# DaanVrancken/HubbardTN

Measured on AMD Instinct MI355X. Metric: DMRG sweep time (s) + GS energy/site, 1-band Hubbard L=64 chi=1024, lower is better.
Workload: dtype c128; 1 GPU; one-band Hubbard chain L=64 U/t=4, half filling, fZ2xSU(2)xU(1), two-site DMRG sweep (2L-3=125 bond updates) at chi=1024 (TensorKit dim units); model=one_band, L=64, chi=1024, krylovdim=30, parallelism=sector-parallel apply x1, backend=hip

## Files before the change

hubbardtn_amd/abi.py:

```python
from __future__ import annotations

import ctypes as C
import os

import numpy as np

HERE = os.path.dirname(os.path.abspath(__file__))
LIB_PATH = os.path.join(HERE, "csrc", "libhubbardtn_hip.so")

HTN_MAX_BUFS = 8
HTN_TILE = 32
OP_N, OP_T, OP_C = 0, 1, 2
SEG_GEMM, SEG_COPY = 0, 1

TILE_DT = np.dtype([("c_off", "<i8"), ("buf_c", "<i4"), ("ldc", "<i4"), ("m", "<i4"), ("n", "<i4"),
                    ("row0", "<i4"), ("col0", "<i4"), ("seg_begin", "<i4"), ("seg_count", "<i4"),
                    ("pad0", "<i4"), ("pad1", "<i4"), ("part", "<i4"), ("nparts", "<i4"), ("ws_slot", "<i4"),
                    ("ticket", "<i4")], align=False)
BUF_WS = 7
WS_TICKET_ELEMS = 4096
SEG_DT = np.dtype([("a_off", "<i8"), ("b_off", "<i8"), ("buf_a", "<i4"), ("buf_b", "<i4"),
                   ("lda", "<i4"), ("ldb", "<i4"), ("k", "<i4"), ("op_a", "<i4"), ("op_b", "<i4"),
                   ("type", "<i4"), ("alpha_re", "<f8"), ("alpha_im", "<f8")], align=False)
SVD_DT = np.dtype([("g_off", "<i8"), ("v_off", "<i8"), ("s_off", "<i8"), ("m", "<i4"), ("n", "<i4"),
                   ("flags", "<i4"), ("pad", "<i4")], align=False)
SVD_ACCUMULATE = 1
SVD_QRCP = 2
COPY_DT = np.dtype([("dst_off", "<i8"), ("src_off", "<i8"), ("idx_off", "<i8"), ("scl_off", "<i8"),
                    ("rows", "<i4"), ("cols", "<i4"), ("ldd", "<i4"), ("lds", "<i4"), ("op", "<i4"),
                    ("gather_dim", "<i4"), ("scale_dim", "<i4"), ("inv_norm", "<i4")], align=False)
QR_DT = np.dtype([("offset", "<i8"), ("m", "<i4"), ("n", "<i4"), ("ld", "<i4"), ("pad", "<i4"), ("r_offset", "<i8"),
                  ("ldr", "<i4"), ("trans", "<i4")], align=False)
QR_PANEL, QR_CHUNK, QR_MAX_M = 16, 512, 7664
assert TILE_DT.itemsize == 64 and SEG_DT.itemsize == 64 and SVD_DT.itemsize == 40 and COPY_DT.itemsize == 64
assert QR_DT.itemsize == 40
TRDOT_DT = np.dtype([("a_off", "<i8"), ("b_off", "<i8"), ("rows", "<i4"), ("cols", "<i4"), ("lda", "<i4"), ("ldb", "<i4"),
                     ("out", "<i4"), ("pad", "<i4", (3,)), ("w_re", "<f8"), ("w_im", "<f8")], align=False)
TRDOT_SLOTS = 16
assert TRDOT_DT.itemsize == 64

SYM_SU2_U1, SYM_U1_U1, SYM_SU2 = 0, 1, 2
MAX_SITE = 4
BACKEND_CPU, BACKEND_HIP = 0, 1
SITE_OP_DT = np.dtype([("k", "<i4"), ("dN", "<i4"), ("red", "<f8", (MAX_SITE * MAX_SITE,))], align=False)
MPO_ENTRY_DT = np.dtype([("wl", "<i4"), ("wr", "<i4"), ("op", "<i4"), ("pad", "<i4"), ("coef_re", "<f8"),
                         ("coef_im", "<f8")], align=False)
SUBBLOCK_DT = np.dtype([("lN", "<i4"), ("lj", "<i4"), ("s", "<i4"), ("rN", "<i4"), ("rj", "<i4"), ("ld", "<i4"),
                        ("off", "<i8")], align=False)
SECTOR_DT = np.dtype([("N", "<i4"), ("j", "<i4"), ("count", "<i4")], align=False)
ENV_BLOCK_DT = np.dtype([("aN", "<i4"), ("aj", "<i4"), ("w", "<i4"), ("bN", "<i4"), ("bj", "<i4"), ("rows", "<i4"),
                         ("cols", "<i4"), ("pad", "<i4"), ("off", "<i8")], align=False)
BOND_STATS_DT = np.dtype([("bond", "<i4"), ("direction", "<i4"), ("n_matvec", "<i4"), ("jacobi_sweeps", "<i4"),
                          ("chi_full", "<i4"), ("multiplets", "<i4"), ("n_tiles", "<i4"), ("n_segs", "<i4"),
                          ("theta_size", "<i8"), ("apply_flops", "<i8"), ("apply_bytes", "<i8"), ("svd_flops", "<i8"),
                          ("energy", "<f8"), ("residual", "<f8"), ("trunc_weight", "<f8"), ("t_plan", "<f8"),
                          ("t_lanczos", "<f8"), ("t_svd", "<f8"), ("t_env", "<f8"), ("t_total", "<f8"),
                          ("matvec_ms", "<f8")], align=False)
assert SITE_OP_DT.itemsize == 136 and MPO_ENTRY_DT.itemsize == 32 and SUBBLOCK_DT.itemsize == 32
assert SECTOR_DT.itemsize == 12 and ENV_BLOCK_DT.itemsize == 40 and BOND_STATS_DT.itemsize == 136


class Symmetry(C.Structure):
    _fields_ = [("kind", C.c_int32), ("n_site", C.c_int32), ("site_N", C.c_int32 * MAX_SITE),
                ("site_j", C.c_int32 * MAX_SITE)]


class SiteOp(C.Structure):
    _fields_ = [("k", C.c_int32), ("dN", C.c_int32), ("red", C.c_double * (MAX_SITE * MAX_SITE))]


class TrdotItem(C.Structure):
    _fields_ = [("a_off", C.c_int64), ("b_off", C.c_int64), ("rows", C.c_int32), ("cols", C.c_int32), ("lda", C.c_int32),
                ("ldb", C.c_int32), ("out", C.c_int32), ("pad", C.c_int32 * 3), ("w_re", C.c_double), ("w_im", C.c_double)]


class CorrChannel(C.Structure):
    _fields_ = [("open", SiteOp), ("pass_", SiteOp), ("close", SiteOp), ("onsite", SiteOp), ("has_onsite", C.c_int32),
                ("pad", C.c_int32)]


class SvdOpts(C.Structure):
    _fields_ = [("split_elems", C.c_int32), ("sweeps_hint", C.c_int32), ("rank_cut", C.c_double),
                ("sweeps_used", C.POINTER(C.c_int32))]


class SweepOpts(C.Structure):
    _fields_ = [("chi_full", C.c_int32), ("weighting", C.c_int32), ("cutoff", C.c_double), ("krylovdim", C.c_int32),
                ("maxrestart", C.c_int32), ("lanczos_tol", C.c_double), ("jacobi_tol", C.c_double),
                ("jacobi_max_sweeps", C.c_int32), ("svd_split_elems", C.c_int32), ("rank_cut", C.c_double),
                ("profile", C.c_int32), ("pad", C.c_int32)]


class IdmrgOpts(C.Structure):
    _fields_ = [("sweep", SweepOpts), ("cell_sites", C.c_int32), ("window_dN", C.c_int32), ("tol", C.c_double),
                ("min_steps", C.c_int32), ("maxiter", C.c_int32), ("sweeps_per_step", C.c_int32), ("warm_start", C.c_int32)]


class IdmrgStats(C.Structure):
    _fields_ = [("step", C.c_int32), ("sweeps", C.c_int32), ("converged", C.c_int32), ("finished", C.c_int32),
                ("needs_window", C.c_int32), ("chi_full", C.c_int32), ("energy", C.c_double),
                ("energy_per_site", C.c_double), ("delta", C.c_double)]


assert C.sizeof(SiteOp) == 136 and C.sizeof(TrdotItem) == 64 and C.sizeof(CorrChannel) == 4 * 136 + 8
assert C.sizeof(SweepOpts) == 64 and C.sizeof(IdmrgOpts) == 96 and C.sizeof(IdmrgStats) == 48

EXPORTS = ["htn_last_error", "htn_abi_version", "htn_device_init", "htn_grouped_gemm_z",
           "htn_dots_scratch_elems", "htn_dots_z", "htn_axpys_z", "htn_scale_inv_sqrt_z",
           "htn_jacobi_svd_z", "htn_batched_copy_z", "htn_lanczos_scratch_elems", "htn_lanczos_z", "htn_lanczos_orth_z",
           "htn_trdots_scratch_elems", "htn_block_trdots_z"]
ENGINE_EXPORTS = ["htn_ctx_create", "htn_ctx_destroy", "htn_ctx_backend", "htn_ctx_set_timing", "htn_comm_unique_id",
                  "htn_ctx_set_comm", "htn_ctx_set_exchange", "htn_mpo_create", "htn_mpo_destroy", "htn_mps_create",
                  "htn_mps_destroy", "htn_bond_update", "htn_dmrg2_sweep", "htn_mps_theta_size", "htn_heff2_apply",
                  "htn_mps_get_theta", "htn_mps_nsites", "htn_mps_bond", "htn_mps_spectrum", "htn_mps_site_size",
                  "htn_mps_get_site", "htn_mps_env_size", "htn_mps_get_env", "htn_mps_env_blocks", "htn_mps_env_bond",
                  "htn_plan_apply_dump", "htn_mps_cache_stats", "htn_balance_tiles",
                  "htn_idmrg_create", "htn_idmrg_destroy", "htn_idmrg_boundary", "htn_idmrg_step", "htn_idmrg_window",
                  "htn_mps_set_orthogonal", "htn_mps_orthogonal_count", "htn_mps_overlap",
                  "htn_site_update", "htn_dmrg1_sweep", "htn_mps_centre", "htn_mps_site_theta_size", "htn_heff1_apply",
                  "htn_qr_blocks_z", "htn_mps_correlator"]


class GemmLaunch(C.Structure):
    _fields_ = [("bufs", C.c_void_p * HTN_MAX_BUFS), ("tiles", C.c_void_p), ("segs", C.c_void_p),
                ("n_tiles", C.c_int32), ("pad", C.c_int32)]


EXCHANGE_FN = C.CFUNCTYPE(C.c_int, C.c_void_p, C.c_int64, C.c_void_p)

_lib = None


class HtnError(RuntimeError):
    pass


def load_library(path: str | None = None):
    global _lib
    if _lib is not None and path is None:
        return _lib
    p = path or LIB_PATH
    import torch
    if not os.path.exists(p):
        raise HtnError(f"{p} not found: build it with `python -m hubbardtn_amd.build` "
                       "(hipcc --offload-arch=gfx950); there is no CPU fallback")
    lib = C.CDLL(p)
    vp, i32, i64, f64 = C.c_void_p, C.c_int32, C.c_int64, C.c_double
    lib.htn_last_error.restype = C.c_char_p
    lib.htn_abi_version.restype = C.c_int
    lib.htn_device_init.argtypes = [C.c_int, C.c_char_p, C.POINTER(C.c_int)]
    lib.htn_grouped_gemm_z.argtypes = [C.POINTER(vp), vp, i32, vp, vp]
    lib.htn_dots_scratch_elems.argtypes = [i32]
    lib.htn_dots_scratch_elems.restype = i64
    lib.htn_dots_z.argtypes = [vp, i64, i32, vp, i64, vp, vp, vp]
    lib.htn_axpys_z.argtypes = [vp, vp, i64, i32, vp, f64, i64, vp]
    lib.htn_scale_inv_sqrt_z.argtypes = [vp, vp, vp, i64, vp]
    lib.htn_jacobi_svd_z.argtypes = [vp, vp, vp, vp, vp, i32, i32, i32, f64, vp, C.POINTER(SvdOpts), vp]
    lib.htn_batched_copy_z.argtypes = [vp, vp, vp, vp, vp, i32, f64, vp]
    lib.htn_lanczos_scratch_elems.argtypes = [i32]
    lib.htn_lanczos_scratch_elems.restype = i64
    lib.htn_lanczos_z.argtypes = [C.POINTER(GemmLaunch), i32, i32, i32, vp, i64, i32, f64, i32, vp, i32,
                                  EXCHANGE_FN, vp, C.POINTER(f64), C.POINTER(i32), C.POINTER(f64), C.POINTER(f64), vp]
    lib.htn_lanczos_orth_z.argtypes = [C.POINTER(GemmLaunch), i32, i32, i32, vp, i64, i32, f64, i32, vp, i32,
                                       EXCHANGE_FN, vp, C.POINTER(f64), C.POINTER(i32), C.POINTER(f64), C.POINTER(f64),
                                       vp, i32, vp]
    lib.htn_trdots_scratch_elems.argtypes = [i32]
    lib.htn_trdots_scratch_elems.restype = i64
    lib.htn_block_trdots_z.argtypes = [vp, vp, vp, i32, vp, i32, vp, vp]
    declare_engine(lib)
    for name in EXPORTS + ENGINE_EXPORTS:
        getattr(lib, name)
    if lib.htn_abi_version() != ABI_VERSION:
        raise HtnError("ABI version mismatch")
    if path is None:
        _lib = lib
    return lib


ABI_VERSION = 2


def declare_engine(lib):
    vp, i32, i64, f64 = C.c_void_p, C.c_int32, C.c_int64, C.c_double
    lib.htn_last_error.restype = C.c_char_p
    lib.htn_abi_version.restype = C.c_int
    lib.htn_ctx_create.argtypes = [i32, i32, vp, C.POINTER(vp)]
    lib.htn_ctx_destroy.argtypes = [vp]
    lib.htn_ctx_destroy.restype = None
    lib.htn_ctx_backend.argtypes = [vp]
    lib.htn_ctx_set_timing.argtypes = [vp, i32]
    lib.htn_comm_unique_id.argtypes = [vp]
    lib.htn_ctx_set_comm.argtypes = [vp, i32, i32, vp]
    lib.htn_ctx_set_exchange.argtypes = [vp, i32, i32, EXCHANGE_FN, vp]
    lib.htn_mpo_create.argtypes = [vp, C.POINTER(Symmetry), i32, vp, i32, vp, vp, vp, vp, C.POINTER(vp)]
    lib.htn_mpo_destroy.argtypes = [vp]
    lib.htn_mpo_destroy.restype = None
    lib.htn_mps_create.argtypes = [vp, vp, i32, vp, vp, vp, vp, vp, vp, vp, vp, C.POINTER(vp)]
    lib.htn_mps_destroy.argtypes = [vp]
    lib.htn_mps_destroy.restype = None
    lib.htn_bond_update.argtypes = [vp, i32, i32, i32, i32, C.POINTER(SweepOpts), vp]
    lib.htn_dmrg2_sweep.argtypes = [vp, C.POINTER(SweepOpts), vp, C.POINTER(f64)]
    lib.htn_mps_theta_size.argtypes = [vp, i32]
    lib.htn_mps_theta_size.restype = i64
    lib.htn_heff2_apply.argtypes = [vp, i32, vp, vp]
    lib.htn_mps_get_theta.argtypes = [vp, i32, vp]
    lib.htn_mps_nsites.argtypes = [vp]
    lib.htn_mps_bond.argtypes = [vp, i32, vp]
    lib.htn_mps_spectrum.argtypes = [vp, i32, vp, vp]
    lib.htn_mps_spectrum.restype = i64
    lib.htn_mps_site_size.argtypes = [vp, i32, C.POINTER(i32)]
    lib.htn_mps_site_size.restype = i64
    lib.htn_mps_get_site.argtypes = [vp, i32, vp, vp]
    lib.htn_mps_env_size.argtypes = [vp, i32, i32]
    lib.htn_mps_env_size.restype = i64
    lib.htn_mps_get_env.argtypes = [vp, i32, i32, vp]
    lib.htn_mps_env_blocks.argtypes = [vp, i32, i32, vp]
    lib.htn_mps_env_bond.argtypes = [vp, i32, i32, vp]
    lib.htn_plan_apply_dump.argtypes = [vp, i32, i32, C.POINTER(i32), vp, C.POINTER(i32), vp, C.POINTER(i64),
                                        C.POINTER(i64)]
    lib.htn_mps_cache_stats.argtypes = [vp, C.POINTER(i64), C.POINTER(i64)]
    lib.htn_balance_tiles.argtypes = [vp, i32, i32, vp, i32, C.POINTER(i32)]
    lib.htn_idmrg_create.argtypes = [vp, vp, C.POINTER(IdmrgOpts), C.POINTER(vp)]
    lib.htn_idmrg_destroy.argtypes = [vp]
    lib.htn_idmrg_destroy.restype = None
    lib.htn_idmrg_boundary.argtypes = [vp, i32, vp]
    lib.htn_idmrg_step.argtypes = [vp, vp, vp, vp, vp, vp, vp, C.POINTER(IdmrgStats)]
    lib.htn_idmrg_window.argtypes = [vp, C.POINTER(vp)]
    lib.htn_mps_set_orthogonal.argtypes = [vp, C.POINTER(vp), i32]
    lib.htn_mps_orthogonal_count.argtypes = [vp, C.POINTER(i32)]
    lib.htn_mps_overlap.argtypes = [vp, vp, C.POINTER(f64)]
    lib.htn_site_update.argtypes = [vp, i32, i32, i32, C.POINTER(SweepOpts), vp]
    lib.htn_dmrg1_sweep.argtypes = [vp, C.POINTER(SweepOpts), vp, C.POINTER(f64)]
    lib.htn_mps_centre.argtypes = [vp]
    lib.htn_mps_site_theta_size.argtypes = [vp, i32]
    lib.htn_mps_site_theta_size.restype = i64
    lib.htn_heff1_apply.argtypes = [vp, i32, vp, vp]
    lib.htn_qr_blocks_z.argtypes = [vp, vp, vp, vp, i32, vp]
    lib.htn_mps_correlator.argtypes = [vp, C.POINTER(CorrChannel), vp, C.POINTER(f64)]
    for name in ENGINE_EXPORTS:
        getattr(lib, name)


def check(lib, rc: int, what: str):
    if rc != 0:
        raise HtnError(f"{what}: {lib.htn_last_error().decode()}")
```

hubbardtn_amd/csrc/htn_backend_hip.hip:

```cpp
#include <dlfcn.h>

#include <map>
#include <mutex>

#include "htn_common.h"
#include "htn_core.h"

namespace {

__global__ __launch_bounds__(256) void k_scale_z(double2* __restrict__ x, int64_t n, double f) {
    for (int64_t j = (int64_t)blockIdx.x * blockDim.x + threadIdx.x; j < n; j += (int64_t)gridDim.x * blockDim.x) {
        const double2 v = x[j];
        x[j] = make_double2(v.x * f, v.y * f);
    }
}

__global__ __launch_bounds__(256) void k_copy_words(uint32_t* __restrict__ dst, const uint32_t* __restrict__ src, size_t n) {
    for (size_t j = (size_t)blockIdx.x * blockDim.x + threadIdx.x; j < n; j += (size_t)gridDim.x * blockDim.x) dst[j] = src[j];
    __threadfence_system();
}

struct Rccl {
    void* lib = nullptr;
    int (*GetUniqueId)(void*) = nullptr;
    void* CommInitRank = nullptr;
    int (*CommDestroy)(void*) = nullptr;
    int (*AllReduce)(const void*, void*, size_t, int, int, void*, hipStream_t) = nullptr;
    const char* (*GetErrorString)(int) = nullptr;
    bool ok = false;
};
struct NcclId {
    char internal[128];
};
Rccl& rccl() {
    static Rccl r;
    static std::once_flag once;
    std::call_once(once, [] {
        const char* names[] = {"librccl.so.1", "librccl.so", "/opt/rocm/lib/librccl.so.1", "/opt/rocm/lib/librccl.so"};
        for (const char* n : names) {
            r.lib = dlopen(n, RTLD_NOW | RTLD_GLOBAL);
            if (r.lib) break;
        }
        if (!r.lib) return;
        r.GetUniqueId = (int (*)(void*))dlsym(r.lib, "ncclGetUniqueId");
        r.CommInitRank = dlsym(r.lib, "ncclCommInitRank");
        r.CommDestroy = (int (*)(void*))dlsym(r.lib, "ncclCommDestroy");
        r.AllReduce = (int (*)(const void*, void*, size_t, int, int, void*, hipStream_t))dlsym(r.lib, "ncclAllReduce");
        r.GetErrorString = (const char* (*)(int))dlsym(r.lib, "ncclGetErrorString");
        r.ok = r.GetUniqueId && r.CommInitRank && r.CommDestroy && r.AllReduce;
    });
    return r;
}
typedef int (*nccl_init_fn)(void**, int, NcclId, int);

struct HipBackend : htn::Backend {
    int device = 0;
    hipStream_t st = nullptr;
    bool own_stream = false;
    std::multimap<size_t, void*> free_list;
    bool fork_open = false;
    std::map<void*, size_t> live;
    size_t pooled = 0;
    void* lan_scratch = nullptr;
    int64_t lan_scratch_elems = 0;
    void* trd_scratch = nullptr;
    int64_t trd_scratch_elems = 0;
    void* comm = nullptr;
    char* stage = nullptr;
    size_t stage_cap = (size_t)32 << 20, stage_pos = 0;
    char* land = nullptr;
    char* land_dev = nullptr;
    size_t land_cap = (size_t)4 << 20;

    ~HipBackend() override {
        (void)hipSetDevice(device);
        if (st) (void)hipStreamSynchronize(st);
        htn_krylov_release_stream(st);
        htn_svd_release_stream(st);
        if (comm && rccl().ok) rccl().CommDestroy(comm);
        for (auto& kv : free_list) (void)hipFree(kv.second);
        for (auto& kv : live) (void)hipFree(kv.first);
        if (lan_scratch) (void)hipFree(lan_scratch);
        if (trd_scratch) (void)hipFree(trd_scratch);
        if (stage) (void)hipHostFree(stage);
        if (land) (void)hipHostFree(land);
        if (own_stream && st) (void)hipStreamDestroy(st);
    }
    int kind() const override { return HTN_BACKEND_HIP; }
    int activate() override {
        HIP_TRY(hipSetDevice(device));
        return 0;
    }

    void* poisoned(void* p, size_t bytes) {
        if (p && htn_debug_poison() && hipMemsetAsync(p, 0xFF, bytes, st) != hipSuccess) {
            (void)hipGetLastError();
            htn::set_error("HTN_DEBUG_POISON: hipMemsetAsync failed");
            live.erase(p);
            (void)hipFree(p);
            return nullptr;
        }
        return p;
    }
    void* alloc(size_t bytes) override {
        if (fork_open) {
            htn::set_error("pool invariant violated: allocation while the SVD's forked stream is open");
            return nullptr;
        }
        bytes = (bytes + 255) / 256 * 256;
        auto it = free_list.lower_bound(bytes);
        if (it != free_list.end() && it->first <= bytes + bytes / 4 + 4096) {
            void* p = it->second;
            live[p] = it->first;
            pooled -= it->first;
            free_list.erase(it);
            return poisoned(p, live[p]);
        }
        void* p = nullptr;
        const size_t want = bytes + bytes / 8;
        if (hipMalloc(&p, want) != hipSuccess) {
            (void)hipGetLastError();
            (void)hipStreamSynchronize(st);
            for (auto& kv : free_list) (void)hipFree(kv.second);
            free_list.clear();
            pooled = 0;
            if (hipMalloc(&p, bytes) != hipSuccess) {
                (void)hipGetLastError();
                return nullptr;
            }
            live[p] = bytes;
            return poisoned(p, bytes);
        }
        live[p] = want;
        return poisoned(p, want);
    }
    void release(void* p) override {
        if (fork_open) {
            htn::set_error("pool invariant violated: release while the SVD's forked stream is open");
            abort();
        }
        auto it = live.find(p);
        if (it == live.end()) return;
        const size_t sz = it->second;
        live.erase(it);
        if (pooled + sz > ((size_t)64 << 30)) {
            (void)hipStreamSynchronize(st);
            (void)hipFree(p);
            return;
        }
        free_list.insert({sz, p});
        pooled += sz;
    }
    int upload(void* dst, const void* src, size_t bytes) override {
        if (!bytes) return 0;
        if (bytes > stage_cap / 2) {
            HIP_TRY(hipMemcpyAsync(dst, src, bytes, hipMemcpyHostToDevice, st));
            HIP_TRY(hipStreamSynchronize(st));
            stage_pos = 0;
            return 0;
        }
        if (!stage) HIP_TRY(hipHostMalloc((void**)&stage, stage_cap));
        const size_t need = (bytes + 255) & ~(size_t)255;
        if (stage_pos + need > stage_cap) {
            HIP_TRY(hipStreamSynchronize(st));
            stage_pos = 0;
        }
        memcpy(stage + stage_pos, src, bytes);
        HIP_TRY(hipMemcpyAsync(dst, stage + stage_pos, bytes, hipMemcpyHostToDevice, st));
        stage_pos += need;
        return 0;
    }
    int download(void* dst, const void* src, size_t bytes) override {
        if (!bytes) return 0;
        if (bytes > land_cap) {
            HIP_TRY(hipMemcpyAsync(dst, src, bytes, hipMemcpyDeviceToHost, st));
            HIP_TRY(hipStreamSynchronize(st));
            stage_pos = 0;
            return 0;
        }
        if (!land) {
            HIP_TRY(hipHostMalloc((void**)&land, land_cap, hipHostMallocMapped | hipHostMallocCoherent));
            HIP_TRY(hipHostGetDevicePointer((void**)&land_dev, land, 0));
        }
        if (bytes <= ((size_t)256 << 10) && ((uintptr_t)src & 3) == 0) {
            const size_t words = (bytes + 3) / 4;
            hipLaunchKernelGGL(k_copy_words, dim3((unsigned)std::min<size_t>((words + 255) / 256, 64)), dim3(256), 0, st,
                               (uint32_t*)land_dev, (const uint32_t*)src, words);
            HIP_TRY(hipGetLastError());
        } else
            HIP_TRY(hipMemcpyAsync(land, src, bytes, hipMemcpyDeviceToHost, st));
        HIP_TRY(htn_stream_spin(st));
        memcpy(dst, land, bytes);
        stage_pos = 0;
        return 0;
    }
    int zero(void* p, size_t bytes) override {
        if (!bytes) return 0;
        HIP_TRY(hipMemsetAsync(p, 0, bytes, st));
        return 0;
    }
    int sync() override {
        HIP_TRY(htn_stream_spin(st));
        stage_pos = 0;
        return 0;
    }
    int grouped_gemm(const void* const* bufs, const htn_tile* tiles, int32_t n_tiles, const htn_seg* segs) override {
        return htn_grouped_gemm_z(bufs, tiles, n_tiles, segs, st);
    }
    int lanczos(const htn_gemm_launch* stages, int n_stages, int x_slot, int y_slot, void* V, int64_t n, int krylovdim,
                double tol, int max_restart, int zero_y, htn_exchange2_fn exchange, void* user, double* eig, int* n_matvec,
                double* residual, double* matvec_ms) override {
        if (ensure_lan_scratch(htn_lanczos_scratch_elems(krylovdim))) return 1;
        int32_t nmv = 0;
        const int rc = htn_lanczos_z(stages, n_stages, x_slot, y_slot, V, n, krylovdim, tol, max_restart, lan_scratch, zero_y,
                                     exchange, user, eig, &nmv, residual, matvec_ms, st);
        *n_matvec = nmv;
        return rc;
    }
    int ensure_lan_scratch(int64_t need) {
        if (need > lan_scratch_elems) {
            if (lan_scratch) HIP_TRY(hipFree(lan_scratch));
            HIP_TRY(hipMalloc(&lan_scratch, sizeof(double2) * need));
            if (htn_debug_poison()) HIP_TRY(hipMemsetAsync(lan_scratch, 0xFF, sizeof(double2) * need, st));
            lan_scratch_elems = need;
        }
        return 0;
    }
    int lanczos_orth(const htn_gemm_launch* stages, int n_stages, int x_slot, int y_slot, void* V, int64_t n, int krylovdim,
                     double tol, int max_restart, int zero_y, htn_exchange2_fn exchange, void* user, const void* Q, int n_frozen,
                     double* eig, int* n_matvec, double* residual, double* matvec_ms) override {
        if (ensure_lan_scratch(htn_lanczos_scratch_elems(krylovdim + n_frozen))) return 1;
        int32_t nmv = 0;
        const int rc = htn_lanczos_orth_z(stages, n_stages, x_slot, y_slot, V, n, krylovdim, tol, max_restart, lan_scratch, zero_y,
                                          exchange, user, eig, &nmv, residual, matvec_ms, Q, n_frozen, st);
        *n_matvec = nmv;
        return rc;
    }
    int orthonormalise_rows(void* Pv, int64_t n, int nvec, double drop_tol, int* kept) override {
        if (nvec > 32) return htn::set_error("orthonormalise_rows: more than 32 rows");
        if (ensure_lan_scratch(htn_dots_scratch_elems(32) + 64)) return 1;
        double2* P = (double2*)Pv;
        double2* part = (double2*)lan_scratch;
        double2* coef = part + htn_dots_scratch_elems(32);
        double2* nrm = coef + 32;
        int k = 0;
        for (int r = 0; r < nvec; ++r) {
            double2* dst = P + (int64_t)k * n;
            if (r != k) HIP_TRY(hipMemcpyAsync(dst, P + (int64_t)r * n, sizeof(double2) * n, hipMemcpyDeviceToDevice, st));
            if (htn_dots_z(dst, n, 1, dst, n, nrm, part, st)) return 1;
            for (int pass = 0; pass < 2 && k > 0; ++pass) {
                if (htn_dots_z(P, n, k, dst, n, coef, part, st)) return 1;
                if (htn_axpys_z(dst, P, n, k, coef, -1.0, n, st)) return 1;
            }
            if (htn_dots_z(dst, n, 1, dst, n, nrm + 1, part, st)) return 1;
            double h[4];
            if (download(h, nrm, sizeof(h))) return 1;
            const double n0 = h[0], n1 = h[2];
            if (!(n0 > 0.0) || !(n1 > drop_tol * drop_tol * n0)) continue;
            if (htn_scale_inv_sqrt_z(dst, dst, nrm + 1, n, st)) return 1;
            ++k;
        }
        *kept = k;
        return 0;
    }
    int jacobi_svd(void* G, void* Vj, double* S, const htn_svd_block* desc_dev, const htn_svd_block* desc_host, int n_blocks,
                   int max_m, int max_sweeps, double tol, int32_t* info_dev, const htn_svd_opts* opts) override {
        fork_open = true;
        const int rc = htn_jacobi_svd_z(G, Vj, S, desc_dev, desc_host, n_blocks, max_m, max_sweeps, tol, info_dev, opts, st);
        fork_open = false;
        return rc;
    }
    int qr_blocks(void* A, void* R, const htn_qr_block* desc_dev, const htn_qr_block* desc_host, int n_blocks) override {
        return htn_qr_blocks_z(A, R, desc_dev, desc_host, n_blocks, st);
    }
    int block_trdots(const void* A, const void* B, const htn_trdot_item* items_dev, const htn_trdot_item* items_host, int n_items,
                     void* out, int n_out) override {
        (void)items_host;
        const int64_t need = htn_trdots_scratch_elems(n_items);
        if (need > trd_scratch_elems) {
            if (trd_scratch) HIP_TRY(hipFree(trd_scratch));
            trd_scratch = nullptr, trd_scratch_elems = 0;
            HIP_TRY(hipMalloc(&trd_scratch, sizeof(double2) * 2 * need));
            trd_scratch_elems = 2 * need;
            if (htn_debug_poison()) HIP_TRY(hipMemsetAsync(trd_scratch, 0xFF, sizeof(double2) * trd_scratch_elems, st));
        }
        return htn_block_trdots_z(A, B, items_dev, n_items, out, n_out, trd_scratch, st);
    }
    int batched_copy(void* dst, const void* src, const int32_t* idx, const double* scl, const htn_copy_item* items, int n_items,
                     double gscale) override {
        return htn_batched_copy_z(dst, src, idx, scl, items, n_items, gscale, st);
    }
    int scale(void* x, int64_t n, double f) override {
        if (n <= 0) return 0;
        const int grid = (int)std::min<int64_t>((n + 255) / 256, 2048);
        hipLaunchKernelGGL(k_scale_z, dim3(grid), dim3(256), 0, st, (double2*)x, n, f);
        HIP_TRY(hipGetLastError());
        return 0;
    }
    int set_comm(int rank, int world, const void* id) override {
        Rccl& r = rccl();
        if (!r.ok) return htn::set_error("htn_ctx_set_comm: librccl.so could not be loaded");
        if (comm) {
            r.CommDestroy(comm);
            comm = nullptr;
        }
        NcclId uid;
        memcpy(uid.internal, id, sizeof(uid.internal));
        const int rc = ((nccl_init_fn)r.CommInitRank)(&comm, world, uid, rank);
        if (rc != 0) return htn::set_error("ncclCommInitRank: %s", r.GetErrorString ? r.GetErrorString(rc) : "error");
        return 0;
    }
    bool has_comm() const override { return comm != nullptr; }
    int allreduce(void* y, int64_t n) override {
        if (!comm) return htn::set_error("allreduce: no communicator (htn_ctx_set_comm)");
        const int rc = rccl().AllReduce(y, y, (size_t)(2 * n), 8, 0, comm, st);
        if (rc != 0) return htn::set_error("ncclAllReduce: %s", rccl().GetErrorString ? rccl().GetErrorString(rc) : "error");
        return 0;
    }
};

}

char* htn_err_buf() { return htn::err_buf(); }

namespace htn {
Backend* make_backend(int backend, int device, void* stream) {
    if (backend != HTN_BACKEND_HIP) {
        set_error("libhubbardtn_hip.so has no CPU backend (backend %d requested): there is no CPU fallback", backend);
        return nullptr;
    }
    char name[256];
    int cus = 0;
    if (htn_device_init(device, name, &cus)) return nullptr;
    auto* b = new HipBackend();
    b->device = device;
    if (stream) b->st = (hipStream_t)stream;
    else {
        if (hipStreamCreateWithFlags(&b->st, hipStreamNonBlocking) != hipSuccess) {
            set_error("hipStreamCreate failed");
            delete b;
            return nullptr;
        }
        b->own_stream = true;
    }
    return b;
}
}

extern "C" int htn_comm_unique_id(void* id_host) {
    Rccl& r = rccl();
    if (!r.ok) return htn::set_error("htn_comm_unique_id: librccl.so could not be loaded");
    const int rc = r.GetUniqueId(id_host);
    if (rc != 0) return htn::set_error("ncclGetUniqueId: %s", r.GetErrorString ? r.GetErrorString(rc) : "error");
    return 0;
}
```

hubbardtn_amd/csrc/htn_common.h:

```cpp
#pragma once
#include <hip/hip_runtime.h>
#include <stdint.h>
#include <stdio.h>
#include <stdlib.h>
#include <string.h>

#include <map>
#include <memory>
#include <mutex>
#include <utility>

#include "hubbardtn_hip.h"

char* htn_err_buf();

static inline int htn_fail(const char* what, hipError_t e) {
    snprintf(htn_err_buf(), 512, "%s: %s", what, hipGetErrorString(e));
    return 1;
}
static inline int htn_fail_msg(const char* what) {
    snprintf(htn_err_buf(), 512, "%s", what);
    return 1;
}
#define fail htn_fail
#define fail_msg htn_fail_msg
#define HIP_TRY(x)                                       \
    do {                                                 \
        hipError_t _e = (x);                             \
        if (_e != hipSuccess) return htn_fail(#x, _e);   \
    } while (0)

typedef double d4 __attribute__((ext_vector_type(4)));

static inline hipError_t htn_event_spin(hipEvent_t ev) {
    hipError_t e;
    while ((e = hipEventQuery(ev)) == hipErrorNotReady) __builtin_ia32_pause();
    return e;
}
static inline hipError_t htn_stream_spin(hipStream_t st) {
    static thread_local hipEvent_t evs[64] = {};
    int dev = 0;
    hipError_t e = hipGetDevice(&dev);
    if (e != hipSuccess) return e;
    if (dev < 0 || dev >= 64) return hipStreamSynchronize(st);
    if (!evs[dev] && (e = hipEventCreateWithFlags(&evs[dev], hipEventDisableTiming)) != hipSuccess) return e;
    if ((e = hipEventRecord(evs[dev], st)) != hipSuccess) return e;
    return htn_event_spin(evs[dev]);
}


static inline bool htn_env_flag(const char* name) {
    const char* v = getenv(name);
    return v && v[0] && v[0] != '0';
}
static inline bool htn_debug_poison() {
    static const bool on = htn_env_flag("HTN_DEBUG_POISON");
    return on;
}
static inline bool htn_debug_event_waits() {
    static const bool on = htn_env_flag("HTN_DEBUG_EVENT_WAITS");
    return on;
}

struct LanRecord {
    unsigned long long w[4];
};
__host__ __device__ __forceinline__ unsigned long long lan_rotl(unsigned long long x, int r) { return (x << r) | (x >> (64 - r)); }
__host__ __device__ __forceinline__ unsigned long long lan_check(unsigned long long w0, unsigned long long w1, unsigned long long w2,
                                                                 unsigned long long serial) {
    return serial ^ lan_rotl(w0, 13) ^ lan_rotl(w1, 29) ^ lan_rotl(w2, 47) ^ 0x9E3779B97F4A7C15ull;
}
#define HTN_DOT_BLOCKS 256
struct HtnGemmPublish {
    const double* norm_partial;
    const double2* c1;
    const double2* c2;
    LanRecord* rec_out;
    unsigned long long serial;
};
int htn_grouped_gemm_launch(const void* const* bufs_host, const htn_tile* tiles, int32_t n_tiles, const htn_seg* segs,
                            const HtnGemmPublish* pub, hipStream_t stream);

enum HtnBufKind {
    HTN_BUF_DEVICE,
    HTN_BUF_PINNED,
    HTN_BUF_MAPPED
};
struct HtnBuf {
    const HtnBufKind kind;
    const bool poison;
    void* p = nullptr;
    void* dev = nullptr;
    size_t cap = 0;
    explicit HtnBuf(HtnBufKind k, bool poison_new = true) : kind(k), poison(poison_new) {}
    HtnBuf(const HtnBuf&) = delete;
    ~HtnBuf() { (void)release(); }
    hipError_t release() {
        const hipError_t e = !p ? hipSuccess : (kind == HTN_BUF_DEVICE ? hipFree(p) : hipHostFree(p));
        p = dev = nullptr, cap = 0;
        return e;
    }
    int reserve(size_t bytes) {
        if (bytes <= cap) return 0;
        HIP_TRY(release());
        const size_t want = bytes * 2;
        if (kind == HTN_BUF_DEVICE) {
            HIP_TRY(hipMalloc(&p, want));
            dev = p;
            if (poison && htn_debug_poison()) HIP_TRY(hipMemset(p, 0xFF, want));
        } else if (kind == HTN_BUF_PINNED) {
            HIP_TRY(hipHostMalloc(&p, want, hipHostMallocDefault));
        } else {
            HIP_TRY(hipHostMalloc(&p, want, hipHostMallocMapped | hipHostMallocCoherent));
            HIP_TRY(hipHostGetDevicePointer(&dev, p, 0));
        }
        cap = want;
        return 0;
    }
};

template <class T>
class HtnStreamRegistry {
    std::mutex mu;
    std::map<std::pair<int, hipStream_t>, std::unique_ptr<T>> entries;

public:
    template <class Init>
    int get(hipStream_t st, T** out, Init init) {
        int dev = 0;
        HIP_TRY(hipGetDevice(&dev));
        std::lock_guard<std::mutex> lk(mu);
        auto it = entries.find({dev, st});
        if (it == entries.end()) {
            auto r = std::make_unique<T>();
            r->device = dev;
            if (init(*r)) return 1;
            it = entries.emplace(std::make_pair(dev, st), std::move(r)).first;
        }
        *out = it->second.get();
        return 0;
    }
    void release(hipStream_t st) {
        int dev = 0;
        if (hipGetDevice(&dev) != hipSuccess) return;
        std::lock_guard<std::mutex> lk(mu);
        entries.erase({dev, st});
    }
};
void htn_krylov_release_stream(hipStream_t st);
void htn_svd_release_stream(hipStream_t st);

template <int CTRL>
__device__ __forceinline__ double dpp_f64(double v) {
    const int lo = __builtin_amdgcn_update_dpp(0, __double2loint(v), CTRL, 0xF, 0xF, true);
    const int hi = __builtin_amdgcn_update_dpp(0, __double2hiint(v), CTRL, 0xF, 0xF, true);
    return __hiloint2double(hi, lo);
}

__device__ __forceinline__ double row_sum16(double v) {
    v += dpp_f64<0xB1>(v);
    v += dpp_f64<0x4E>(v);
    v += dpp_f64<0x141>(v);
    v += dpp_f64<0x140>(v);
    return v;
}

template <int L>
__device__ __forceinline__ double lane_bcast(double v) {
    const int lo = __builtin_amdgcn_readlane(__double2loint(v), L);
    const int hi = __builtin_amdgcn_readlane(__double2hiint(v), L);
    return __hiloint2double(hi, lo);
}

__device__ __forceinline__ double wave_sum(double v) {
    v = row_sum16(v);
    const double a = lane_bcast<0>(v) + lane_bcast<16>(v);
    const double b = lane_bcast<32>(v) + lane_bcast<48>(v);
    return a + b;
}

template <int CTRL>
__device__ __forceinline__ unsigned long long dpp_u64(unsigned long long v) {
    const unsigned lo = (unsigned)__builtin_amdgcn_update_dpp(0, (int)(unsigned)v, CTRL, 0xF, 0xF, true);
    const unsigned hi = (unsigned)__builtin_amdgcn_update_dpp(0, (int)(unsigned)(v >> 32), CTRL, 0xF, 0xF, true);
    return ((unsigned long long)hi << 32) | lo;
}
__device__ __forceinline__ unsigned long long umax64(unsigned long long a, unsigned long long b) { return a > b ? a : b; }
__device__ __forceinline__ unsigned long long row_max16_u64(unsigned long long v) {
    v = umax64(v, dpp_u64<0xB1>(v));
    v = umax64(v, dpp_u64<0x4E>(v));
    v = umax64(v, dpp_u64<0x141>(v));
    v = umax64(v, dpp_u64<0x140>(v));
    return v;
}
template <int L>
__device__ __forceinline__ unsigned long long lane_bcast_u64(unsigned long long v) {
    const unsigned lo = (unsigned)__builtin_amdgcn_readlane((int)(unsigned)v, L);
    const unsigned hi = (unsigned)__builtin_amdgcn_readlane((int)(unsigned)(v >> 32), L);
    return ((unsigned long long)hi << 32) | lo;
}
__device__ __forceinline__ unsigned long long wave_max_u64(unsigned long long v) {
    v = row_max16_u64(v);
    return umax64(umax64(lane_bcast_u64<0>(v), lane_bcast_u64<16>(v)),
                  umax64(lane_bcast_u64<32>(v), lane_bcast_u64<48>(v)));
}

__device__ __forceinline__ double fast_rcp(double a) {
    double x = __builtin_amdgcn_rcp(a);
    x = fma(fma(-a, x, 1.0), x, x);
    x = fma(fma(-a, x, 1.0), x, x);
    return x;
}
__device__ __forceinline__ double fast_rsq(double a) {
    double y = __builtin_amdgcn_rsq(a);
    const double h = 0.5 * a;
    y = y * fma(-h * y, y, 1.5);
    y = y * fma(-h * y, y, 1.5);
    return y;
}
```

hubbardtn_amd/csrc/htn_core.h:

```cpp
#pragma once
#include <stdint.h>
#include <string.h>

#include <array>
#include <complex>
#include <memory>
#include <string>
#include <unordered_map>
#include <utility>
#include <vector>

#include "hubbardtn_hip.h"

namespace htn {

typedef std::complex<double> cplx;

enum { BUF_X = 0, BUF_Y, BUF_L, BUF_R, BUF_Z, BUF_S1, BUF_S2, BUF_AUX };

struct Sec {
    int32_t N, j;
};
inline bool operator<(const Sec& a, const Sec& b) { return a.N < b.N || (a.N == b.N && a.j < b.j); }
inline bool operator==(const Sec& a, const Sec& b) { return a.N == b.N && a.j == b.j; }
inline bool operator!=(const Sec& a, const Sec& b) { return !(a == b); }
inline uint64_t skey(Sec s) { return ((uint64_t)(uint32_t)s.N << 32) | (uint32_t)s.j; }

struct Sym {
    int kind = HTN_SYM_SU2_U1;
    int n_site = 3;
    Sec site[HTN_MAX_SITE] = {{0, 0}, {1, 1}, {2, 0}, {0, 0}};
    bool su2() const { return kind != HTN_SYM_U1_U1; }
    int wrapN(int N) const { return kind == HTN_SYM_SU2 ? (N & 1) : N; }
    int qdim(Sec c) const { return su2() ? c.j + 1 : 1; }
    int jeff(int j) const { return su2() ? j : 0; }
    bool triangle(int a, int b, int c) const;
    bool connects(Sec ket, int dN, int k, Sec bra) const { return bra.N == wrapN(ket.N + dN) && triangle(ket.j, k, bra.j); }
    void fuse(Sec sec, int s, std::vector<Sec>& out) const;
    void split(Sec sec, int s, std::vector<Sec>& out) const;
};

double wigner6j(int j1, int j2, int j3, int j4, int j5, int j6);
double wigner9j(int j1, int j2, int j3, int j4, int j5, int j6, int j7, int j8, int j9);
double coef_left(int jbp, int k, int jb, int jsp, int js, int kop, int jap, int kp, int ja);
double coef_right(int jcp, int k, int jc, int jsp, int js, int kop, int jbp, int kp, int jb);
double coef_apply(int ja, int jap, int k, int js1, int js1p, int kop1, int km, int jc, int jcp, int js2, int js2p,
                  int kop2, int kp, int jb, int jbp);

typedef std::array<int32_t, 12> Key;
struct KeyHash {
    size_t operator()(const Key& k) const {
        uint64_t h = 1469598103934665603ull;
        for (int32_t v : k) {
            h ^= (uint32_t)v;
            h *= 1099511628211ull;
        }
        return (size_t)h;
    }
};
typedef std::unordered_map<Key, int, KeyHash> KeyMap;
inline Key mk(int32_t a = -9, int32_t b = -9, int32_t c = -9, int32_t d = -9, int32_t e = -9, int32_t f = -9, int32_t g = -9,
              int32_t h = -9, int32_t i = -9, int32_t j = -9, int32_t k = -9, int32_t l = -9) {
    return Key{a, b, c, d, e, f, g, h, i, j, k, l};
}

struct Bond {
    std::vector<Sec> secs;
    std::vector<int32_t> dims;
    std::unordered_map<uint64_t, int> index;
    std::string key;
    std::string seckey;
    Bond() {}
    explicit Bond(std::vector<std::pair<Sec, int>> items);
    int find(Sec s) const {
        auto it = index.find(skey(s));
        return it == index.end() ? -1 : it->second;
    }
    bool has(Sec s) const { return index.count(skey(s)) != 0; }
    int dim(Sec s) const {
        const int i = find(s);
        return i < 0 ? 0 : dims[i];
    }
    int64_t dim_full(const Sym& sym) const;
    int multiplets() const;
};
typedef std::shared_ptr<const Bond> BondP;

struct BlockRec {
    int64_t off;
    int32_t m, n, ld;
};
struct Grp {
    Sec sec;
    int s;
};

struct SiteLayout {
    char kind;
    BondP bl, br;
    std::vector<Key> bkeys;
    std::vector<BlockRec> blocks;
    KeyMap bidx;
    struct Mat {
        Sec c;
        int64_t off;
        int32_t rows, cols;
        std::vector<Grp> groups;
    };
    std::vector<Mat> mats;
    std::unordered_map<uint64_t, int> midx;
    int64_t size = 0;
    int block(Sec l, int s, Sec r) const {
        auto it = bidx.find(mk(l.N, l.j, s, r.N, r.j));
        return it == bidx.end() ? -1 : it->second;
    }
    int mat(Sec c) const {
        auto it = midx.find(skey(c));
        return it == midx.end() ? -1 : it->second;
    }
};
typedef std::shared_ptr<const SiteLayout> SiteLayoutP;
SiteLayoutP build_site_layout(const Sym& sym, char kind, BondP bl, BondP br);

struct ThetaLayout {
    BondP bl, br;
    struct Mat {
        Sec c;
        int64_t off;
        int32_t rows, cols;
        std::vector<Grp> rows_g, cols_g;
        std::vector<int32_t> roffs, coffs;
    };
    std::vector<Mat> mats;
    std::unordered_map<uint64_t, int> midx;
    std::vector<Key> bkeys;
    std::vector<BlockRec> blocks;
    KeyMap bidx;
    int64_t size = 0;
    int block(Sec a, int s1, Sec c, int s2, Sec b) const {
        auto it = bidx.find(mk(a.N, a.j, s1, c.N, c.j, s2, b.N, b.j));
        return it == bidx.end() ? -1 : it->second;
    }
};
typedef std::shared_ptr<const ThetaLayout> ThetaLayoutP;
ThetaLayoutP build_theta_layout(const Sym& sym, BondP bl, BondP br);

struct Lvl {
    int32_t dN, k;
};
struct EnvLayout {
    char side;
    BondP bond;
    std::vector<Lvl> levels;
    int ident;
    std::vector<Key> bkeys;
    struct Blk {
        int64_t off;
        int32_t m, n;
    };
    std::vector<Blk> blocks;
    KeyMap bidx;
    std::unordered_map<Key, std::vector<Sec>, KeyHash> by_ket;
    int64_t size = 0;
    int block(Sec x, int w, Sec y) const {
        auto it = bidx.find(mk(x.N, x.j, w, y.N, y.j));
        return it == bidx.end() ? -1 : it->second;
    }
    const std::vector<Sec>* kets(int w, Sec ket) const {
        auto it = by_ket.find(mk(w, ket.N, ket.j));
        return it == by_ket.end() ? nullptr : &it->second;
    }
};
typedef std::shared_ptr<const EnvLayout> EnvLayoutP;
EnvLayoutP build_env_layout(const Sym& sym, char side, BondP bond, const std::vector<Lvl>& levels);

struct MpoEntry {
    int32_t wl, wr, op;
    cplx coef;
};
struct MpoSite {
    std::vector<Lvl> left, right;
    std::vector<MpoEntry> entries;
    std::string key;
};
struct SiteOp {
    int k, dN;
    double red[HTN_MAX_SITE][HTN_MAX_SITE];
};
struct Mpo {
    Sym sym;
    std::vector<SiteOp> ops;
    std::vector<MpoSite> sites;
};

struct Tasks {
    std::vector<htn_tile> tiles;
    int32_t ntiles = 0;
    std::vector<htn_seg> segs;
    int32_t nsegs = 0;
    int64_t flops = 0;
    std::vector<int64_t> group_bounds;
};

int balance_tiles(Tasks& t, int n_cus);

struct ApplyPlan {
    Tasks tz, ty;
    bool has_z = false;
    int64_t zsize = 0;
    int64_t nterms = 0;
};
void plan_apply(const Mpo& mpo, const ThetaLayout& tl, const EnvLayout& Ll, const EnvLayout& Rl, const MpoSite& W1,
                const MpoSite& W2, ApplyPlan& out);
void plan_apply1(const Mpo& mpo, const SiteLayout& lay, const EnvLayout& Ll, const EnvLayout& Rl, const MpoSite& W, ApplyPlan& out);
void plan_gauge1(const SiteLayout& cen, const SiteLayout& nb, std::vector<htn_qr_block>& desc, int64_t& rsize, Tasks& out);
void plan_theta(const char* mode, const SiteLayout& lay1, const SiteLayout& lay2, const ThetaLayout& tl, Tasks& out);
struct EnvPlan {
    Tasks t1, t2;
    int64_t zsize = 0;
};
void plan_left_env(const Mpo& mpo, const EnvLayout& Ll, const SiteLayout& lay, const MpoSite& W, const EnvLayout& Lnew,
                   EnvPlan& out);
void plan_right_env(const Mpo& mpo, const EnvLayout& Rl, const SiteLayout& lay, const MpoSite& W, const EnvLayout& Rnew,
                    EnvPlan& out);

struct OvlLayout {
    BondP rows, cols;
    std::vector<Sec> secs;
    std::vector<int64_t> off;
    std::vector<int32_t> m, n;
    std::unordered_map<uint64_t, int> index;
    int64_t size = 0;
    int find(Sec s) const {
        auto it = index.find(skey(s));
        return it == index.end() ? -1 : it->second;
    }
};
typedef std::shared_ptr<const OvlLayout> OvlLayoutP;
OvlLayoutP build_ovl_layout(BondP rows, BondP cols);
struct OvlPlan {
    Tasks t1, t2;
    int64_t zsize = 0;
};
void plan_ovl_left(const OvlLayout& Ol, const SiteLayout& bra, const SiteLayout& ket, const OvlLayout& Onew, OvlPlan& out);
void plan_ovl_right(const OvlLayout& Or, const SiteLayout& bra, const SiteLayout& ket, const OvlLayout& Onew, OvlPlan& out);
void plan_ovl_project(const OvlLayout& Ol, const OvlLayout& Or, const SiteLayout& k1, const SiteLayout& k2, const ThetaLayout& tl,
                      OvlPlan& out);

struct SvdPlan {
    std::vector<htn_svd_block> desc;
    std::vector<htn_copy_item> stage;
    std::vector<Sec> mids;
    std::vector<char> transposed, accumulate;
    int64_t g_size = 0, v_size = 0, s_size = 0;
    int32_t max_m = 0;
    int64_t flops = 0;
    bool any_accumulate = false;
};
int plan_svd(const ThetaLayout& tl, bool right, SvdPlan& out);

void truncate(const std::vector<double>& vals, const std::vector<int>& lens, const std::vector<int>& qdims, int chi_full,
              double cutoff, int weighting, std::vector<int>& counts, double& trunc_weight, double& kept_norm);

struct FinalizePlan {
    std::vector<htn_copy_item> iso_g, cen_g, iso_v;
    Tasks cen;
    bool has_cen = false;
    int64_t n_idx = 0;
};
void plan_finalize(const ThetaLayout& tl, const SvdPlan& sp, const std::vector<int>& keep, const SiteLayout& layA,
                   const SiteLayout& layB, bool right, int64_t offA, int64_t offB, FinalizePlan& out);

struct Backend {
    virtual ~Backend() {}
    virtual int kind() const = 0;
    virtual int activate() { return 0; }
    virtual void* alloc(size_t bytes) = 0;
    virtual void release(void* p) = 0;
    virtual int upload(void* dst, const void* src_host, size_t bytes) = 0;
    virtual int download(void* dst_host, const void* src, size_t bytes) = 0;
    virtual int zero(void* p, size_t bytes) = 0;
    virtual int sync() = 0;
    virtual int grouped_gemm(const void* const* bufs, const htn_tile* tiles, int32_t n_tiles, const htn_seg* segs) = 0;
    virtual int lanczos(const htn_gemm_launch* stages, int n_stages, int x_slot, int y_slot, void* V, int64_t n,
                        int krylovdim, double tol, int max_restart, int zero_y, htn_exchange2_fn exchange, void* user,
                        double* eig, int* n_matvec, double* residual, double* matvec_ms) = 0;
    virtual int lanczos_orth(const htn_gemm_launch* stages, int n_stages, int x_slot, int y_slot, void* V, int64_t n,
                             int krylovdim, double tol, int max_restart, int zero_y, htn_exchange2_fn exchange, void* user,
                             const void* Q, int n_frozen, double* eig, int* n_matvec, double* residual, double* matvec_ms);
    virtual int orthonormalise_rows(void* P, int64_t n, int nvec, double drop_tol, int* kept);
    virtual int qr_blocks(void* A, void* R, const htn_qr_block* desc_dev, const htn_qr_block* desc_host, int n_blocks);
    virtual int block_trdots(const void* A, const void* B, const htn_trdot_item* items_dev, const htn_trdot_item* items_host,
                             int n_items, void* out, int n_out);
    virtual int jacobi_svd(void* G, void* Vj, double* S, const htn_svd_block* desc_dev, const htn_svd_block* desc_host,
                           int n_blocks, int max_m, int max_sweeps, double tol, int32_t* info_dev,
                           const htn_svd_opts* opts) = 0;
    virtual int batched_copy(void* dst, const void* src, const int32_t* idx, const double* scl,
                             const htn_copy_item* items_dev, int n_items, double gscale) = 0;
    virtual int scale(void* x, int64_t n, double f) = 0;
    virtual int set_comm(int rank, int world, const void* id) { return 1; }
    virtual bool has_comm() const { return false; }
    virtual int allreduce(void* y, int64_t n) { return 1; }
    bool timing = false;
};

void qr_blocks_host(cplx* A, cplx* R, const htn_qr_block* desc, int n_blocks);

int set_error(const char* fmt, ...);
char* err_buf();

}
```

hubbardtn_amd/csrc/htn_engine.cpp:

```cpp
#include <math.h>
#include <stdio.h>
#include <stdlib.h>

#include <algorithm>
#include <atomic>
#include <chrono>
#include <map>

#include "htn_core.h"

namespace htn {
Backend* make_backend(int backend, int device, void* stream);
}
using namespace htn;

namespace {
void tridiag_lowest_host(const std::vector<double>& alpha, const std::vector<double>& beta, double* eig, std::vector<double>& vec) {
    const int k = (int)alpha.size();
    auto count = [&](double x) {
        int cnt = 0;
        double d = 1.0;
        for (int i = 0; i < k; ++i) {
            d = (alpha[i] - x) - (i ? beta[i - 1] * beta[i - 1] / d : 0.0);
            if (d == 0.0) d = 1e-300;
// ... 597 lines not shown
        (left ? plan_left_env : plan_right_env)(*mpo, *elay[from], lay, W, *e->lay, p);
        return compile2(e, p);
    });
    if (!c) return 1;
    DView z = zalloc(c->zsize, false), out = zalloc(c->lay->size, false);
    if (!z.base || !out.base) return set_error("device allocation failed (%s environment)", left ? "left" : "right");
    if (gemm(c->d1, {{left ? BUF_L : BUF_R, ebuf[from].ptr()}, {BUF_S1, site_buf[i].ptr()}, {BUF_Z, z.ptr()}})) return 1;
    if (gemm(c->d2, {{BUF_S1, site_buf[i].ptr()}, {BUF_Z, z.ptr()}, {BUF_Y, out.ptr()}})) return 1;
    elay[to] = c->lay;
    ebuf[to] = out;
    return 0;
}

int htn_mps::ovl_boundary(const htn_mps* ket, int b, OvlLayoutP* outl, DView* out) {
    OvlLayoutP lay = b == 0 ? build_ovl_layout(bonds[0], ket->bonds[0]) : build_ovl_layout(ket->bonds[L], bonds[L]);
    if (lay->size != 1) return set_error("overlap: the end bonds of the two states are not one common sector of dimension 1");
    DView v = zalloc(1, false);
    const cplx one(1.0, 0.0);
    if (!v.base || be->upload(v.ptr(), &one, sizeof(one))) return set_error("overlap: device allocation failed");
    *outl = lay;
    *out = v;
    return 0;
}

int htn_mps::ovl_step(char side, const htn_mps* ket, int i, const OvlLayoutP& inl, const DView& in, OvlLayoutP* outl, DView* out) {
    const bool left = side == 'L';
    const SiteLayout &lb = *site_lay[i], &lk = *ket->site_lay[i];
    auto c = cached<OvlC>(std::string(left ? "ovlL" : "ovlR") + lb.kind + lk.kind + bonds[i]->key + "|" + bonds[i + 1]->key + "|" +
                              ket->bonds[i]->key + "|" + ket->bonds[i + 1]->key,
                          [&]() -> std::shared_ptr<OvlC> {
                              auto e = std::make_shared<OvlC>();
                              e->lay = left ? build_ovl_layout(bonds[i + 1], ket->bonds[i + 1]) : build_ovl_layout(ket->bonds[i], bonds[i]);
                              OvlPlan p;
                              (left ? plan_ovl_left : plan_ovl_right)(*inl, lb, lk, *e->lay, p);
                              return compile2(e, p);
                          });
    if (!c) return 1;
    DView z = zalloc(c->zsize, false), o = zalloc(c->lay->size, true);
    if (!z.base || !o.base) return set_error("device allocation failed (overlap environment)");
    if (gemm(c->d1, {{left ? BUF_L : BUF_R, in.ptr()}, {BUF_S2, ket->site_buf[i].ptr()}, {BUF_Z, z.ptr()}})) return 1;
    if (gemm(c->d2, {{BUF_S1, site_buf[i].ptr()}, {BUF_Z, z.ptr()}, {BUF_Y, o.ptr()}})) return 1;
    *outl = c->lay;
    *out = o;
    return 0;
}

int htn_mps::ovl_project(const OrthState& os, int i, const ThetaLayout& tl, cplx* dst) {
    const htn_mps* ket = os.phi;
    const SiteLayout &k1 = *ket->site_lay[i], &k2 = *ket->site_lay[i + 1];
    auto c = cached<OvlC>(std::string("ovlP") + k1.kind + k2.kind + bonds[i]->key + "|" + bonds[i + 2]->key + "|" + ket->bonds[i]->key + "|" +
                              ket->bonds[i + 1]->key + "|" + ket->bonds[i + 2]->key,
                          [&]() -> std::shared_ptr<OvlC> {
                              OvlPlan p;
                              plan_ovl_project(*os.Llay[i], *os.Rlay[i + 2], k1, k2, tl, p);
                              return compile2(std::make_shared<OvlC>(), p);
                          });
    if (!c) return 1;
    DView z = zalloc(c->zsize, false);
    if (!z.base) return set_error("device allocation failed (projector row)");
    if (gemm(c->d1, {{BUF_L, os.Lbuf[i].ptr()}, {BUF_R, os.Rbuf[i + 2].ptr()}, {BUF_S1, ket->site_buf[i].ptr()},
                     {BUF_S2, ket->site_buf[i + 1].ptr()}, {BUF_Z, z.ptr()}}))
        return 1;
    return gemm(c->d2, {{BUF_Z, z.ptr()}, {BUF_Y, dst}});
}

void htn_mps::orth_detach() {
    for (auto& os : orth) htn_mps_destroy(os.phi);
    orth.clear();
    orth_dropped = 0;
}

int htn_mps::orth_attach(htn_mps* const* others, int n) {
    std::vector<OrthState> fresh((size_t)n);
    for (int k = 0; k < n; ++k) {
        OrthState& os = fresh[k];
        os.phi = others[k];
        os.Llay.resize(L + 1);
        os.Rlay.resize(L + 1);
        os.Lbuf.resize(L + 1);
        os.Rbuf.resize(L + 1);
        if (ovl_boundary(os.phi, 0, &os.Llay[0], &os.Lbuf[0]) || ovl_boundary(os.phi, L, &os.Rlay[L], &os.Rbuf[L])) return 1;
        for (int i = 0; i < L; ++i)
            if (ovl_step('L', os.phi, i, os.Llay[i], os.Lbuf[i], &os.Llay[i + 1], &os.Lbuf[i + 1])) return 1;
        for (int i = L - 1; i >= 0; --i)
            if (ovl_step('R', os.phi, i, os.Rlay[i + 1], os.Rbuf[i + 1], &os.Rlay[i], &os.Rbuf[i])) return 1;
    }
    if (be->sync()) return 1;
    for (int k = 0; k < n; ++k) ++others[k]->refs;
    orth_detach();
    orth.swap(fresh);
    return 0;
}

std::shared_ptr<ApplyC> htn_mps::compile_apply(ApplyPlan& p, bool deal_y) {
    auto a = std::make_shared<ApplyC>();
    a->has_z = p.has_z;
    a->zsize = p.zsize;
    a->flops = p.ty.flops + (p.has_z ? p.tz.flops : 0);
    a->ntiles = p.ty.ntiles + (p.has_z ? p.tz.ntiles : 0);
    a->nsegs = p.ty.nsegs + (p.has_z ? p.tz.nsegs : 0);
    if (deal_y && ctx->world > 1) {
        std::vector<htn_tile> sel;
        for (int t = ctx->rank; t < p.ty.ntiles; t += ctx->world) sel.push_back(p.ty.tiles[t]);
        p.ty.ntiles = (int32_t)sel.size();
        if (sel.empty()) sel.push_back(p.ty.tiles[0]);
        p.ty.tiles.swap(sel);
    }
    if (p.has_z && upload_tasks(p.tz, a->dz)) return nullptr;
    if (upload_tasks(p.ty, a->dy)) return nullptr;
    return a;
}

std::shared_ptr<ApplyC> htn_mps::make_apply(int i, const ThetaLayout& tl) {
    return cached<ApplyC>(ikey("apply", i) + bonds[i]->key + "|" + bonds[i + 2]->key, [&]() -> std::shared_ptr<ApplyC> {
        ApplyPlan p;
        plan_apply(*mpo, tl, *Llay[i], *Rlay[i + 2], mpo->sites[i], mpo->sites[i + 1], p);
        return compile_apply(p, true);
    });
}
std::shared_ptr<ApplyC> htn_mps::make_apply1(int i, const SiteLayout& lay) {
    return cached<ApplyC>(ikey("apply1", i) + lay.kind + bonds[i]->key + "|" + bonds[i + 1]->key, [&]() -> std::shared_ptr<ApplyC> {
        ApplyPlan p;
        plan_apply1(*mpo, lay, *Llay[i], *Rlay[i + 1], mpo->sites[i], p);
        return compile_apply(p, false);
    });
}

int htn_mps::apply_stages(const ApplyC& ap, const DView& L, const DView& R, const DView& z, htn_gemm_launch* stages) {
    if (ensure_ws(std::max(ap.dy.ws_slots, ap.has_z ? ap.dz.ws_slots : 0))) return -1;
    memset(stages, 0, 2 * sizeof(htn_gemm_launch));
    stages[0].bufs[HTN_BUF_WS] = stages[1].bufs[HTN_BUF_WS] = ws.ptr();
    int ns = 0;
    if (ap.has_z) {
        stages[ns].bufs[BUF_L] = L.ptr();
        stages[ns].bufs[BUF_Z] = z.ptr();
        stages[ns].tiles = ap.dz.tiles, stages[ns].segs = ap.dz.segs, stages[ns].n_tiles = ap.dz.ntiles;
        ++ns;
    }
    stages[ns].bufs[BUF_L] = L.ptr();
    stages[ns].bufs[BUF_R] = R.ptr();
    stages[ns].bufs[BUF_Z] = z.ptr();
    stages[ns].tiles = ap.dy.tiles, stages[ns].segs = ap.dy.segs, stages[ns].n_tiles = ap.dy.ntiles;
    return ns + 1;
}

int htn_mps::theta_into(int i, const ThetaLayout& tl, cplx* dst) {
    const SiteLayout &l1 = *site_lay[i], &l2 = *site_lay[i + 1];
    const char mode[3] = {l1.kind, l2.kind, 0};
    if (strcmp(mode, "RR") && strcmp(mode, "LL") && strcmp(mode, "LR")) return set_error("theta: centre is not on sites (%d, %d)", i, i + 1);
    auto d = cached<DevTasks>(std::string("theta") + mode + bonds[i]->key + "|" + bonds[i + 1]->key + "|" + bonds[i + 2]->key,
                              [&]() -> std::shared_ptr<DevTasks> {
                                  Tasks t;
                                  plan_theta(mode, l1, l2, tl, t);
                                  auto dt = std::make_shared<DevTasks>();
                                  if (upload_tasks(t, *dt)) return nullptr;
                                  return dt;
                              });
    if (!d) return 1;
    return gemm(*d, {{BUF_S1, site_buf[i].ptr()}, {BUF_S2, site_buf[i + 1].ptr()}, {BUF_Y, dst}});
}

static int exchange_tramp(void* y, int64_t n, void* user) {
    htn_ctx* ctx = (htn_ctx*)user;
    if (ctx->exch) return ctx->exch(y, n, ctx->exch_user);
    return ctx->be->allreduce(y, n);
}

int htn_mps::apply_once(const ApplyC& ap, const DView& L, const DView& R, int64_t n, const void* x_host, void* y_host, bool exchange) {
    DView x = zalloc(n, false), y = zalloc(n, true), z = zalloc(ap.zsize, false);
    if (!x.base || !y.base || !z.base) return set_error("device allocation failed");
    if (be->upload(x.ptr(), x_host, sizeof(cplx) * n)) return 1;
    if (ap.has_z && gemm(ap.dz, {{BUF_X, x.ptr()}, {BUF_L, L.ptr()}, {BUF_Z, z.ptr()}})) return 1;
    if (gemm(ap.dy, {{BUF_X, x.ptr()}, {BUF_Y, y.ptr()}, {BUF_L, L.ptr()}, {BUF_R, R.ptr()}, {BUF_Z, z.ptr()}})) return 1;
    if (exchange && exchange_tramp(y.ptr(), n, ctx)) return set_error("htn_heff2_apply: exchange failed");
    return be->download(y_host, y.ptr(), sizeof(cplx) * n);
}

void htn_mps::fill_stats(htn_bond_stats* st, int bond, int direction, const Solve& sol, int64_t env_elems, int jacobi_sweeps,
                         int64_t svd_flops, double trunc_weight, const StageClock& clk) {
    memset(st, 0, sizeof(*st));
    st->bond = bond, st->direction = direction;
    st->n_matvec = sol.nmv, st->jacobi_sweeps = jacobi_sweeps;
    st->chi_full = (int32_t)bonds[bond]->dim_full(mpo->sym), st->multiplets = bonds[bond]->multiplets();
    st->n_tiles = sol.ap->ntiles, st->n_segs = sol.ap->nsegs;
    st->theta_size = sol.n;
    st->apply_flops = sol.ap->flops, st->apply_bytes = 16 * (2 * sol.n + env_elems), st->svd_flops = svd_flops;
    st->energy = sol.E, st->residual = sol.res, st->trunc_weight = trunc_weight;
    st->t_plan = clk.plan, st->t_lanczos = clk.lanczos, st->t_env = clk.env;
    st->t_total = now() - clk.t0;
    st->t_svd = clk.svd >= 0.0 ? clk.svd : st->t_total - clk.plan - clk.lanczos - clk.env;
    st->matvec_ms = sol.mv_ms > 0.0 ? sol.mv_ms : 0.0;
}

int htn_mps::bond_solve(int i, bool optimise, const htn_sweep_opts& o, StageClock& clk, BondWork& w) {
    w.tl = theta_layout(bonds[i], bonds[i + 2]);
    const ThetaLayout& tl = *w.tl;
    Solve& s = w.sol;
    const int64_t n = s.n = tl.size;
    const int kd = o.krylovdim;
    if (n <= 0) return set_error("htn_bond_update: empty two-site tensor on bond %d", i);
    w.V = zalloc((int64_t)(kd + 2) * n, false);
    if (!w.V.base) return set_error("device allocation of the Krylov basis failed (%lld elements)", (long long)((kd + 2) * n));
    if (theta_into(i, tl, w.V.ptr())) return 1;
    s.ap = make_apply(i, tl);
    if (!s.ap) return 1;
    w.z = zalloc(s.ap->zsize, false);
    htn_gemm_launch stages[2];
    const int ns = apply_stages(*s.ap, Lbuf[i], Rbuf[i + 2], w.z, stages);
    if (ns < 0) return 1;
    clk.plan = clk.lap();
    const bool shard = ctx->shard;
    int n_frozen = 0;
    if (!orth.empty() && optimise) {
        const int na = (int)orth.size();
        if (kd + na > 31)
            return set_error("htn_bond_update: krylovdim + attached states = %d + %d > 31 (row limit of the projected Lanczos step)", kd, na);
        w.Qb = zalloc((int64_t)na * n, false);
        if (!w.Qb.base) return set_error("device allocation of the projector rows failed");
        for (int k = 0; k < na; ++k)
            if (ovl_project(orth[k], i, tl, w.Qb.ptr() + (int64_t)k * n)) return 1;
        if (be->orthonormalise_rows(w.Qb.ptr(), n, na, 1e-12, &n_frozen)) return 1;
        orth_dropped = na - n_frozen;
    }
    if (n_frozen > 0) {
        if (be->lanczos_orth(stages, ns, BUF_X, BUF_Y, w.V.ptr(), n, kd, o.lanczos_tol, o.maxrestart, shard ? 1 : 0,
                             shard ? exchange_tramp : nullptr, ctx, w.Qb.ptr(), n_frozen, &s.E, &s.nmv, &s.res,
                             be->timing ? &s.mv_ms : nullptr))
            return 1;
    } else if (be->lanczos(stages, ns, BUF_X, BUF_Y, w.V.ptr(), n, kd, optimise ? o.lanczos_tol : 1e300, o.maxrestart, shard ? 1 : 0,
                           shard ? exchange_tramp : nullptr, ctx, &s.E, &s.nmv, &s.res, be->timing ? &s.mv_ms : nullptr))
        return 1;
    clk.lanczos = clk.lap();
    return 0;
}

std::shared_ptr<SvdC> htn_mps::make_svd(int i, const ThetaLayout& tl, bool right) {
    return cached<SvdC>(std::string(right ? "svdR" : "svdL") + bonds[i]->key + "|" + bonds[i + 2]->key, [&]() -> std::shared_ptr<SvdC> {
        auto s = std::make_shared<SvdC>();
        if (plan_svd(tl, right, s->sp)) return nullptr;
        if (!(s->stage = upload_vec(be, s->sp.stage)) || !(s->desc = upload_vec(be, s->sp.desc))) return nullptr;
        if (ctx->world > 1) {
            const int nbk = (int)s->sp.mids.size();
            std::vector<int> ord(nbk);
            for (int b = 0; b < nbk; ++b) ord[b] = b;
            auto cost = [&](int b) { return (double)s->sp.desc[b].m * s->sp.desc[b].n * s->sp.desc[b].n; };
            std::stable_sort(ord.begin(), ord.end(), [&](int a, int b) { return cost(a) > cost(b); });
            std::vector<double> load(ctx->world, 0.0);
            std::vector<htn_copy_item> st_own;
            for (int b : ord) {
                int r = 0;
                for (int q = 1; q < ctx->world; ++q)
                    if (load[q] < load[r]) r = q;
                load[r] += cost(b);
                if (r == ctx->rank) {
                    s->own_desc.push_back(s->sp.desc[b]);
                    st_own.push_back(s->sp.stage[b]);
                }
            }
            s->n_own = (int)s->own_desc.size();
            if (s->n_own && (!(s->own_stage = upload_vec(be, st_own)) || !(s->own_desc_dev = upload_vec(be, s->own_desc)))) return nullptr;
        }
        return s;
    });
}

int htn_mps::bond_svd(int i, bool right, const htn_sweep_opts& o, BondWork& w) {
    w.sc = make_svd(i, *w.tl, right);
    if (!w.sc) return 1;
    const SvdC& sc = *w.sc;
    const SvdPlan& sp = sc.sp;
    const int nb = (int)sp.mids.size();
    w.G = zalloc(sp.g_size, false), w.Vj = zalloc(sp.v_size, false);
    w.s_elems = ((size_t)std::max<int64_t>(sp.s_size, 1) + 1) & ~(size_t)1;
    const size_t s_elems = w.s_elems, i_elems = (size_t)std::max(nb, 1);
    const size_t s_bytes = sizeof(double) * s_elems + sizeof(int32_t) * i_elems;
    w.S = dalloc(s_bytes);
    if (!w.G.base || !w.Vj.base || !w.S) return set_error("device allocation failed (SVD workspace)");
    int32_t* info_dev = (int32_t*)((double*)w.S->p + s_elems);
    const bool svd_shard = ctx->world > 1 && ctx->shard;
    const DBufP& stage = svd_shard ? sc.own_stage : sc.stage;
    const DBufP& desc_dev = svd_shard ? sc.own_desc_dev : sc.desc;
    const htn_svd_block* desc_host = svd_shard ? sc.own_desc.data() : sp.desc.data();
    const int n_run = svd_shard ? sc.n_own : nb;
    const bool run = n_run > 0 || !svd_shard;
    if (svd_shard) {
        if (be->zero(w.G.ptr(), sizeof(cplx) * (size_t)std::max<int64_t>(sp.g_size, 1))) return 1;
        if (be->zero(w.S->p, s_bytes)) return 1;
        if (sp.any_accumulate && be->zero(w.Vj.ptr(), sizeof(cplx) * (size_t)std::max<int64_t>(sp.v_size, 1))) return 1;
    }
    if (run && be->batched_copy(w.G.ptr(), w.V.ptr(), nullptr, nullptr, (const htn_copy_item*)stage->p, n_run, 1.0)) return 1;
    int32_t jac_used = 0;
    htn_svd_opts so = {o.svd_split_elems, 0, 0.0, &jac_used};
    {
        auto h = sweeps_hint.find(i + 1);
        if (h != sweeps_hint.end()) so.sweeps_hint = h->second;
    }
    if (o.rank_cut > 0.0) {
        double cut = 0.0;
        auto h = cut_hint.find(i + 1);
        if (h != cut_hint.end() && h->second.first.first == o.chi_full && h->second.first.second == o.cutoff)
            cut = o.rank_cut * h->second.second;
        so.rank_cut = std::max(cut, o.rank_cut * o.cutoff);
    }
    if (run && be->jacobi_svd(w.G.ptr(), w.Vj.ptr(), (double*)w.S->p, (const htn_svd_block*)desc_dev->p, desc_host, n_run, sp.max_m,
                              o.jacobi_max_sweeps, o.jacobi_tol, info_dev, &so))
        return 1;
    if (svd_shard) {
        if (exchange_tramp(w.G.ptr(), std::max<int64_t>(sp.g_size, 1), ctx)) return set_error("sharded SVD: exchange of the blocks failed");
        if (exchange_tramp(w.S->p, (int64_t)(s_elems / 2), ctx)) return set_error("sharded SVD: exchange of the singular values failed");
        if (sp.any_accumulate && exchange_tramp(w.Vj.ptr(), std::max<int64_t>(sp.v_size, 1), ctx)) return 1;
    }
    if (jac_used > 0) sweeps_hint[i + 1] = jac_used;
    w.tA = now();
    w.s_host.resize(s_elems + (i_elems + 1) / 2);
    if (be->download(w.s_host.data(), w.S->p, s_bytes)) return 1;
    w.tB = now();
    const int32_t* info_h = (const int32_t*)(w.s_host.data() + s_elems);
    for (int b = 0; b < n_run; ++b) {
        if (info_h[b] < 0) return set_error("Jacobi SVD did not converge (bond %d, block %d, %d sweeps)", i + 1, b, -info_h[b]);
        w.jac_sweeps = std::max(w.jac_sweeps, (int)info_h[b]);
    }
    return 0;
}

int htn_mps::bond_truncate(int i, const htn_sweep_opts& o, BondWork& w) {
    const SvdPlan& sp = w.sc->sp;
    const int nb = (int)sp.mids.size();
    w.lens.resize(nb), w.qd.resize(nb), w.order.resize(nb);
    w.vals.reserve((size_t)sp.s_size);
    std::vector<std::pair<double, int>> tmp;
    for (int b = 0; b < nb; ++b) {
        const int len = sp.desc[b].n;
        const double* sv = w.s_host.data() + sp.desc[b].s_off;
        w.lens[b] = len;
        w.qd[b] = mpo->sym.qdim(sp.mids[b]);
        tmp.resize(len);
        for (int k = 0; k < len; ++k) tmp[k] = {sv[k], k};
        std::sort(tmp.begin(), tmp.end(), [](const std::pair<double, int>& a, const std::pair<double, int>& c) {
            return a.first != c.first ? a.first > c.first : a.second < c.second;
        });
        w.order[b].resize(len);
        for (int k = 0; k < len; ++k) {
            w.order[b][k] = tmp[k].second;
            w.vals.push_back(tmp[k].first);
        }
    }
    truncate(w.vals, w.lens, w.qd, o.chi_full, o.cutoff, o.weighting, w.counts, w.tw, w.nrm);
    std::vector<std::pair<Sec, int>> mid_items;
    int64_t kept_tot = 0, positive = 0;
    for (int b = 0; b < nb; ++b) {
        if (w.counts[b] > 0) mid_items.push_back({sp.mids[b], w.counts[b]});
        kept_tot += w.counts[b];
    }
    for (double v : w.vals) positive += v > 0.0;
    if (kept_tot == 0 || !(w.nrm > 0.0)) return set_error("htn_bond_update: nothing kept by the truncation on bond %d", i + 1);
    w.mid = std::make_shared<Bond>(mid_items);
    w.tC = now();
    if (o.chi_full > 0 && w.tw > 0.0 && kept_tot < positive) {
        double smin = 1e300;
        size_t p = 0;
        for (int b = 0; b < nb; ++b) {
            if (w.counts[b] > 0) smin = std::min(smin, w.vals[p + w.counts[b] - 1]);
            p += w.lens[b];
        }
        cut_hint[i + 1] = {{o.chi_full, o.cutoff}, smin};
    } else
        cut_hint.erase(i + 1);
    return 0;
}

int htn_mps::bond_finalise(int i, bool right, BondWork& w) {
    const ThetaLayout& tl = *w.tl;
    const SvdPlan& sp = w.sc->sp;
    const std::vector<int>& counts = w.counts;
    const BondP bl = bonds[i], br = bonds[i + 2], mid = w.mid;
    std::string ckey((const char*)counts.data(), sizeof(int) * counts.size());
    auto fc = cached<FinC>(std::string(right ? "finR" : "finL") + bl->key + "|" + br->key + "|" + ckey, [&]() -> std::shared_ptr<FinC> {
        auto f = std::make_shared<FinC>();
        f->layA = site_layout('L', bl, mid);
        f->layB = site_layout('R', mid, br);
        FinalizePlan fp;
        plan_finalize(tl, sp, counts, *f->layA, *f->layB, right, 0, f->layA->size, fp);
        f->n_ig = (int)fp.iso_g.size(), f->n_cg = (int)fp.cen_g.size(), f->n_iv = (int)fp.iso_v.size();
        if (f->n_ig + f->n_cg + f->n_iv) {
            std::vector<htn_copy_item> all;
            all.insert(all.end(), fp.iso_g.begin(), fp.iso_g.end());
            all.insert(all.end(), fp.cen_g.begin(), fp.cen_g.end());
            all.insert(all.end(), fp.iso_v.begin(), fp.iso_v.end());
            if (!(f->items = upload_vec(be, all))) return nullptr;
            f->ig = (const htn_copy_item*)f->items->p;
            f->cg = f->ig + f->n_ig;
            f->iv = f->cg + f->n_cg;
        }
        f->has_cen = fp.has_cen;
        if (fp.has_cen && upload_tasks(fp.cen, f->cen)) return nullptr;
        return f;
    });
    if (!fc) return 1;
    w.tD = now();
    idx_host.clear();
    for (size_t b = 0; b < counts.size(); ++b)
        for (int k = 0; k < counts[b]; ++k) idx_host.push_back(w.order[b][k]);
    w.idx = upload_vec(be, idx_host);
    const int64_t sizeA = fc->layA->size, sizeB = fc->layB->size;
    DView out = zalloc(sizeA + sizeB, true);
    if (!w.idx || !out.base) return set_error("device allocation failed (site tensors)");
    const int32_t* idxp = (const int32_t*)w.idx->p;
    const double* Sp = (const double*)w.S->p;
    cplx* x = w.V.ptr();
    const int64_t n = tl.size;
    if (fc->n_ig && be->batched_copy(out.ptr(), w.G.ptr(), idxp, Sp, fc->ig, fc->n_ig, 1.0)) return 1;
    if (fc->n_cg && be->batched_copy(out.ptr(), w.G.ptr(), idxp, Sp, fc->cg, fc->n_cg, 1.0 / w.nrm)) return 1;
    if (fc->n_iv && be->batched_copy(out.ptr(), w.Vj.ptr(), idxp, Sp, fc->iv, fc->n_iv, 1.0)) return 1;
    if (fc->has_cen) {
        if (be->scale(x, n, 1.0 / w.nrm)) return 1;
        if (gemm(fc->cen, {{BUF_X, x}, {BUF_S1, out.ptr()}, {BUF_Y, out.ptr()}})) return 1;
    }
    bonds[i + 1] = mid;
    site_lay[i] = fc->layA;
    site_buf[i] = DView{out.base, out.off};
    site_lay[i + 1] = fc->layB;
    site_buf[i + 1] = DView{out.base, out.off + sizeA};
    return 0;
}

int htn_mps::bond_advance(int i, bool right) {
    if (right ? left_env(i) : right_env(i + 1)) return 1;
    for (auto& os : orth)
        if (right ? ovl_step('L', os.phi, i, os.Llay[i], os.Lbuf[i], &os.Llay[i + 1], &os.Lbuf[i + 1])
                  : ovl_step('R', os.phi, i + 1, os.Rlay[i + 2], os.Rbuf[i + 2], &os.Rlay[i + 1], &os.Rbuf[i + 1]))
            return 1;
    return 0;
}

void htn_mps::bond_spectrum(int i, const BondWork& w) {
    const SvdPlan& sp = w.sc->sp;
    Spectrum spec;
    size_t p = 0;
    for (size_t b = 0; b < w.counts.size(); ++b) {
        if (w.counts[b] > 0) {
            spec.secs.push_back(sp.mids[b]);
            std::vector<double> v(w.counts[b]);
            const double f = 1.0 / w.nrm / sqrt((double)w.qd[b]);
            for (int k = 0; k < w.counts[b]; ++k) v[k] = w.vals[p + k] * f;
            spec.vals.push_back(std::move(v));
        }
        p += w.lens[b];
    }
    spectra[i + 1] = std::move(spec);
}

int htn_mps::update_bond(int i, int direction, bool right, bool optimise, const htn_sweep_opts& o, htn_bond_stats* st) {
    if (i < 0 || i + 1 >= L) return set_error("htn_bond_update: bond index %d out of range", i);
    StageClock clk(be, o.profile);
    BondWork w;
    if (bond_solve(i, optimise, o, clk, w)) return 1;
    const double t_svd0 = clk.last;
    if (bond_svd(i, right, o, w)) return 1;
    if (bond_truncate(i, o, w)) return 1;
    if (bond_finalise(i, right, w)) return 1;
    static const bool dbg_timers = getenv("HTN_DEBUG_HOST_TIMERS") != nullptr;
    if (dbg_timers)
        fprintf(stderr, "bond %d: svd call %.1f us, download %.1f, sort+truncate %.1f, finalize plan %.1f, enqueue %.1f  misses %lld hits %lld nvals %zu\n", i + 1,
                (w.tA - t_svd0) * 1e6, (w.tB - w.tA) * 1e6, (w.tC - w.tB) * 1e6, (w.tD - w.tC) * 1e6, (now() - w.tD) * 1e6, (long long)misses, (long long)hits, w.vals.size());
    clk.svd = clk.lap();
    if (bond_advance(i, right)) return 1;
    clk.env = clk.lap();
    energy = w.sol.E;
    centre = right ? i + 1 : i;
    bond_spectrum(i, w);
    if (st) fill_stats(st, i + 1, direction, w.sol, Llay[i]->size + Rlay[i + 2]->size, w.jac_sweeps, w.sc->sp.flops, w.tw, clk);
    return 0;
}

int htn_mps::sweep(const htn_sweep_opts& o, htn_bond_stats* st, double* E) {
    int k = 0;
    for (int i = 0; i < L - 1; ++i, ++k)
        if (update_bond(i, +1, i < L - 2, true, o, st ? st + k : nullptr)) return 1;
    for (int i = L - 3; i >= 0; --i, ++k)
        if (update_bond(i, -1, false, true, o, st ? st + k : nullptr)) return 1;
    if (E) *E = energy;
    return 0;
}

int htn_mps::relay(const SiteLayout& from, const cplx* src, const SiteLayout& to, cplx* dst) {
    auto rc = cached<RelayC>(std::string("relay") + from.kind + to.kind + from.bl->key + "|" + from.br->key, [&]() -> std::shared_ptr<RelayC> {
        std::vector<htn_copy_item> items;
        for (size_t q = 0; q < to.blocks.size(); ++q) {
            const Key& k = to.bkeys[q];
            const int sq = from.block({k[0], k[1]}, k[2], {k[3], k[4]});
            if (sq < 0) continue;
            const BlockRec &D = to.blocks[q], &S = from.blocks[sq];
            items.push_back(copy_item(D.off, D.ld, S.off, S.ld, D.m, D.n));
        }
        auto r = std::make_shared<RelayC>();
        r->n = (int)items.size();
        if (!(r->items = upload_vec(be, items))) return nullptr;
        return r;
    });
    if (!rc) return 1;
    return rc->n ? be->batched_copy(dst, src, nullptr, nullptr, (const htn_copy_item*)rc->items->p, rc->n, 1.0) : 0;
}

static int site1_checks(const htn_mps* m, int i, const char* who) {
    if (i < 0 || i >= m->L) return set_error("%s: site %d out of range", who, i);
    if (m->centre != i) return set_error("%s: the centre is on site %d, not on site %d", who, m->centre, i);
    if (!m->orth.empty()) return set_error("%s: one-site updates of a state with attached orthogonal states are not supported", who);
    if (m->ctx->world > 1 || m->ctx->shard || m->be->has_comm())
        return set_error("%s: one-site updates on a context with a communicator are not supported", who);
    if (!m->Llay[i] || !m->Rlay[i + 1] || m->Llay[i]->bond->key != m->bonds[i]->key || m->Rlay[i + 1]->bond->key != m->bonds[i + 1]->key)
        return set_error("%s: the environments of site %d were built on other bond tables: run a two-site sweep first", who, i);
    return 0;
}

int htn_mps::update_site(int i, int direction, bool optimise, const htn_sweep_opts& o, htn_bond_stats* st) {
    if (site1_checks(this, i, "htn_site_update")) return 1;
    if (direction < -1 || direction > 1) return set_error("htn_site_update: direction %d (must be -1, 0 or +1)", direction);
    if ((direction > 0 && i + 1 >= L) || (direction < 0 && i == 0))
        return set_error("htn_site_update: site %d has no neighbour in direction %d", i, direction);
    StageClock clk(be, o.profile);
    const SiteLayoutP cur = site_lay[i];
    const SiteLayoutP lay = direction == 0 ? cur : site_layout(direction > 0 ? 'L' : 'R', bonds[i], bonds[i + 1]);
    Solve s;
    const int64_t n = s.n = lay->size;
    if (n <= 0) return set_error("htn_site_update: empty site tensor on site %d", i);
    for (const auto& M : lay->mats)
        if (direction != 0 && (lay->kind == 'L' ? M.rows < M.cols : M.cols < M.rows))
            return set_error("htn_site_update: sector (%d, %d) of site %d is a %d x %d block, its bond is wider than the rest of the "
                             "site supports: run a two-site sweep first", M.c.N, M.c.j, i, M.rows, M.cols);
    if (direction != 0 && site_lay[i + direction]->kind != (direction > 0 ? 'R' : 'L'))
        return set_error("htn_site_update: site %d is not in %s layout", i + direction, direction > 0 ? "right" : "left");
    const int kd = o.krylovdim;
    DView V = zalloc((int64_t)(kd + 2) * n, false);
    if (!V.base) return set_error("device allocation of the Krylov basis failed (%lld elements)", (long long)((kd + 2) * n));
    if (relay(*cur, site_buf[i].ptr(), *lay, V.ptr())) return 1;
    s.ap = make_apply1(i, *lay);
    if (!s.ap) return 1;
    DView z = zalloc(s.ap->zsize, false);
    if (!z.base) return set_error("device allocation failed (one-site apply)");
    htn_gemm_launch stages[2];
    const int ns = apply_stages(*s.ap, Lbuf[i], Rbuf[i + 1], z, stages);
    if (ns < 0) return 1;
    clk.plan = clk.lap();
    if (be->lanczos(stages, ns, BUF_X, BUF_Y, V.ptr(), n, kd, optimise ? o.lanczos_tol : 1e300, o.maxrestart, 0, nullptr, ctx, &s.E, &s.nmv,
                    &s.res, be->timing ? &s.mv_ms : nullptr))
        return 1;
    clk.lanczos = clk.lap();
    DView out = zalloc(n, false);
    if (!out.base) return set_error("device allocation failed (site tensor)");
    if (relay(*lay, V.ptr(), *lay, out.ptr())) return 1;
    const int crossed = direction > 0 ? i + 1 : i;
    if (direction != 0) {
        const int j = i + direction;
        const SiteLayoutP nl = site_lay[j];
        auto gc = cached<Gauge1C>(std::string(direction > 0 ? "gauge1R" : "gauge1L") + lay->bl->key + "|" + lay->br->key + "|" +
                                      (direction > 0 ? nl->br->key : nl->bl->key),
                                  [&]() -> std::shared_ptr<Gauge1C> {
                                      auto g = std::make_shared<Gauge1C>();
                                      Tasks t;
                                      plan_gauge1(*lay, *nl, g->desc, g->rsize, t);
                                      if (!(g->desc_dev = upload_vec(be, g->desc)) || upload_tasks(t, g->absorb)) return nullptr;
                                      return g;
                                  });
        if (!gc) return 1;
        DView Rf = zalloc(gc->rsize, false), nb_out = zalloc(nl->size, false);
        if (!Rf.base || !nb_out.base) return set_error("device allocation failed (gauge move)");
        if (be->qr_blocks(out.ptr(), Rf.ptr(), (const htn_qr_block*)gc->desc_dev->p, gc->desc.data(), (int)gc->desc.size())) return 1;
        if (gemm(gc->absorb, {{BUF_S1, Rf.ptr()}, {BUF_S2, site_buf[j].ptr()}, {BUF_Y, nb_out.ptr()}})) return 1;
        site_lay[i] = lay;
        site_buf[i] = out;
        site_buf[j] = nb_out;
        centre = j;
        clk.lap();
        if (direction > 0 ? left_env(i) : right_env(i)) return 1;
        clk.env = clk.lap();
    } else {
        site_lay[i] = lay;
        site_buf[i] = out;
    }
    energy = s.E;
    if (st) fill_stats(st, crossed, direction, s, Llay[i]->size + Rlay[i + 1]->size, 0, 0, 0.0, clk);
    return 0;
}

int htn_mps::sweep1(const htn_sweep_opts& o, htn_bond_stats* st, double* E) {
    if (L < 2) return set_error("htn_dmrg1_sweep: a chain of %d site(s) has no bond to sweep over", L);
    if (centre != 0) return set_error("htn_dmrg1_sweep: the centre is on site %d, not on site 0", centre);
    int k = 0;
    for (int i = 0; i < L - 1; ++i, ++k)
        if (update_site(i, +1, true, o, st ? st + k : nullptr)) return 1;
    for (int i = L - 1; i >= 1; --i, ++k)
        if (update_site(i, -1, true, o, st ? st + k : nullptr)) return 1;
    if (E) *E = energy;
    return 0;
}

int htn_mps::correlator(const htn_corr_channel& ch, cplx* out_host, double* norm_host) {
    const Sym& sym = mpo->sym;
    const char* who = "htn_mps_correlator";
    if (ctx->world > 1 || ctx->shard || ctx->exch || be->has_comm())
        return set_error("%s: not available on a context with a communicator or an exchange hook", who);
    if (ch.open.dN + ch.close.dN != 0 || (sym.su2() ? ch.open.k != ch.close.k : ch.open.k + ch.close.k != 0))
        return set_error("%s: the charges of open (dN %d, k %d) and close (dN %d, k %d) do not add up to zero", who, ch.open.dN, ch.open.k,
                         ch.close.dN, ch.close.k);
    if (ch.pass.dN != 0 || ch.pass.k != 0) return set_error("%s: the pass operator carries a charge (dN %d, k %d)", who, ch.pass.dN, ch.pass.k);
    if (ch.has_onsite && (ch.onsite.dN != 0 || ch.onsite.k != 0))
        return set_error("%s: the onsite operator carries a charge (dN %d, k %d)", who, ch.onsite.dN, ch.onsite.k);
    if (Llay[0]->size != 0 || Rlay[L]->size != 0 || bonds[0]->multiplets() != 1 || bonds[L]->multiplets() != 1)
        return set_error("%s: needs a finite chain with open ends (end bonds of one sector, dimension 1)", who);

    Mpo pm;
    pm.sym = sym;
    auto add_op = [&](const htn_site_op& o) {
        SiteOp r;
        r.k = o.k, r.dN = o.dN;
        for (int a = 0; a < HTN_MAX_SITE; ++a)
            for (int b = 0; b < HTN_MAX_SITE; ++b) r.red[a][b] = o.red[a * HTN_MAX_SITE + b];
        pm.ops.push_back(r);
// ... 1173 lines not shown
```

hubbardtn_amd/csrc/htn_krylov.hip:

```cpp
#include <math.h>

#include <chrono>
#include <vector>

#include "htn_common.h"

#define DOT_BLOCKS HTN_DOT_BLOCKS
#define DOT_THREADS 256
#define DOT_CHUNK 32

#define HTN_CH_DISPATCH(nvec, per, LAUNCH)          \
    do {                                            \
        if ((nvec) <= 4) LAUNCH(4, 256);            \
        else if ((nvec) <= 8) LAUNCH(8, 256);       \
        else if ((nvec) <= 12) LAUNCH(12, 256);     \
        else if ((nvec) <= 16) LAUNCH(16, 256);     \
        else if ((nvec) <= 20) LAUNCH(20, 256);     \
        else if ((nvec) <= 24) LAUNCH(24, 256);     \
        else if ((nvec) <= 28) LAUNCH(28, 256);     \
        else LAUNCH(32, 256);                       \
    } while (0)
static inline int64_t dot_slice(int64_t n) { return (n + DOT_BLOCKS - 1) / DOT_BLOCKS; }

template <bool FZ>
// ... 73 lines not shown
    HTN_CH_DISPATCH(nvec, dot_slice(n), HTN_DP);
#undef HTN_DP
}
static void launch_dots_partial_fz(const double2* V, int64_t ldv, int nvec, const double2* w, int64_t n, double2* partial,
                                   const double2* Q, int nf, int upd0, hipStream_t st) {
#define HTN_DP(CHV, THV)                                                                                                    \
    hipLaunchKernelGGL((k_dots_partial<CHV, THV, true>), dim3(DOT_BLOCKS), dim3(THV), 0, st, V, ldv, nvec, w, n, partial, Q, \
                       nf, upd0)
    HTN_CH_DISPATCH(nvec, dot_slice(n), HTN_DP);
#undef HTN_DP
}

__global__ void k_dots_reduce(const double2* __restrict__ partial, int nvec, double2* __restrict__ out) {
    const int i = blockIdx.x;
    const double2 r = reduce_partials(partial + (int64_t)i * DOT_BLOCKS, threadIdx.x);
    if (threadIdx.x == 0) out[i] = r;
}

template <int CH, int TH, bool FZ>
__global__ __launch_bounds__(TH) void k_axpy_norm(double2* __restrict__ w, const double2* __restrict__ V,
                                                           int64_t ldv, int nvec,
                                                           const double2* __restrict__ partial,
                                                           double2* __restrict__ c_out, int c_index, double sign,
                                                           int64_t n, double* __restrict__ norm_partial,
                                                           const double2* __restrict__ Q, int nf) {
    __shared__ double cs[64][2];
    __shared__ double red[TH / 64];
    const int tid = threadIdx.x, lane = tid & 63, wave = tid >> 6;
    for (int i = wave; i < nvec; i += TH / 64) {
        const double2 r = reduce_partials(partial + (int64_t)i * DOT_BLOCKS, lane);
        if (lane == 0) {
            cs[i][0] = r.x;
            cs[i][1] = r.y;
            if (blockIdx.x == 0 && i == c_index) *c_out = r;
        }
    }
    if (tid >= nvec && tid < 64) cs[tid][0] = cs[tid][1] = 0.0;
    __syncthreads();
    const int64_t per = (n + DOT_BLOCKS - 1) / DOT_BLOCKS;
    const int64_t lo = (int64_t)blockIdx.x * per;
    const int64_t hi = lo + per < n ? lo + per : n;
    double nn = 0.0;
    for (int64_t j = lo + tid; j < hi; j += TH) {
        double2 v[CH];
#pragma unroll
        for (int c = 0; c < CH; ++c) {
            const int i = c < nvec ? c : nvec - 1;
            v[c] = lan_row<FZ>(V, Q, ldv, nf, i)[j];
        }
        double2 x = w[j];
        double sr = 0.0, si = 0.0;
#pragma unroll
        for (int c = 0; c < CH; ++c) {
            sr += cs[c][0] * v[c].x - cs[c][1] * v[c].y;
            si += cs[c][0] * v[c].y + cs[c][1] * v[c].x;
        }
        x.x += sign * sr;
        x.y += sign * si;
        w[j] = x;
        nn += x.x * x.x + x.y * x.y;
    }
    nn = wave_sum(nn);
    if (lane == 0) red[wave] = nn;
    __syncthreads();
    if (tid == 0) {
        double t = 0.0;
#pragma unroll
        for (int q = 0; q < TH / 64; ++q) t += red[q];
        norm_partial[blockIdx.x] = t;
    }
}

static void launch_axpy_norm(double2* w, const double2* V, int64_t ldv, int nvec, const double2* partial, double2* c_out, int c_index,
                             double sign, int64_t n, double* norm_partial, hipStream_t st) {
#define HTN_AN(CHV, THV)                                                                                                    \
    hipLaunchKernelGGL((k_axpy_norm<CHV, THV, false>), dim3(DOT_BLOCKS), dim3(THV), 0, st, w, V, ldv, nvec, partial, c_out, \
                       c_index, sign, n, norm_partial, (const double2*)nullptr, 0)
    HTN_CH_DISPATCH(nvec, dot_slice(n), HTN_AN);
#undef HTN_AN
}
static void launch_axpy_norm_fz(double2* w, const double2* V, int64_t ldv, int nvec, const double2* partial, double2* c_out,
                                int c_index, double sign, int64_t n, double* norm_partial, const double2* Q, int nf,
                                hipStream_t st) {
#define HTN_AN(CHV, THV)                                                                                                   \
    hipLaunchKernelGGL((k_axpy_norm<CHV, THV, true>), dim3(DOT_BLOCKS), dim3(THV), 0, st, w, V, ldv, nvec, partial, c_out, \
                       c_index, sign, n, norm_partial, Q, nf)
    HTN_CH_DISPATCH(nvec, dot_slice(n), HTN_AN);
#undef HTN_AN
}

template <int CH, int TH, bool FZ>
__global__ __launch_bounds__(TH) void k_axpy_dots(double2* __restrict__ w, double2* __restrict__ V,
                                                           int64_t ldv, int nvec,
                                                           const double2* __restrict__ partial_in,
                                                           double2* __restrict__ c_out, int c_index, double sign,
                                                           int64_t n, double2* __restrict__ partial_out,
                                                           const double* __restrict__ norm_prev, int upd0,
                                                           const double2* __restrict__ Q, int nf) {
    __shared__ double cs[64][2];
    __shared__ double red[TH / 64][CH][2];
    __shared__ double s_scale;
    const int tid = threadIdx.x, lane = tid & 63, wave = tid >> 6;
    const int last = nvec - 1;
    if (tid < 64) {
        double t = 1.0;
        if (norm_prev) {
            t = 0.0;
#pragma unroll
            for (int b = 0; b < DOT_BLOCKS / 64; ++b) t += norm_prev[tid + 64 * b];
            t = wave_sum(t);
            t = t > 0.0 ? 1.0 / sqrt(t) : 0.0;
        }
        if (tid == 0) s_scale = t;
    }
    __syncthreads();
    const double s = s_scale;
    const int skip = FZ ? upd0 - nf : upd0;
    for (int p = (FZ ? 0 : upd0) + wave; p < (FZ ? nvec - skip : nvec); p += TH / 64) {
        const int i = FZ && p >= nf ? p + skip : p;
        double2 r = reduce_partials(partial_in + (int64_t)(FZ ? p : i - upd0) * DOT_BLOCKS, lane);
        const bool raw_row = norm_prev && i == last;
        const double f = raw_row ? s * s : s;
        r.x *= f;
        r.y *= f;
        if (lane == 0) {
            cs[i][0] = raw_row ? r.x * s : r.x;
            cs[i][1] = raw_row ? r.y * s : r.y;
            if (blockIdx.x == 0 && i == c_index) *c_out = r;
        }
    }
    if ((tid >= nvec || (tid < upd0 && !(FZ && tid < nf))) && tid < 64) cs[tid][0] = cs[tid][1] = 0.0;
    __syncthreads();
    const bool fix = norm_prev != nullptr;
    double2* const vlast = V + (int64_t)(FZ ? last - nf : last) * ldv;
    const int64_t per = (n + DOT_BLOCKS - 1) / DOT_BLOCKS;
    const int64_t lo = (int64_t)blockIdx.x * per;
    const int64_t hi = lo + per < n ? lo + per : n;
    double ar[CH], ai[CH];
#pragma unroll
    for (int c = 0; c < CH; ++c) ar[c] = ai[c] = 0.0;
    for (int64_t j = lo + tid; j < hi; j += TH) {
        double2 v[CH];
#pragma unroll
        for (int c = 0; c < CH; ++c) {
            const int i = c < nvec ? c : nvec - 1;
            v[c] = lan_row<FZ>(V, Q, ldv, nf, i)[j];
        }
        if (fix) {
            const double2 vl = vlast[j];
            vlast[j] = make_double2(vl.x * s, vl.y * s);
        }
        double sr = 0.0, si = 0.0;
#pragma unroll
        for (int c = 0; c < CH; ++c) {
            sr += cs[c][0] * v[c].x - cs[c][1] * v[c].y;
            si += cs[c][0] * v[c].y + cs[c][1] * v[c].x;
        }
        double2 x = w[j];
        x.x = fma(x.x, s, sign * sr);
        x.y = fma(x.y, s, sign * si);
        w[j] = x;
#pragma unroll
        for (int c = 0; c < CH; ++c) {
            ar[c] += v[c].x * x.x + v[c].y * x.y;
            ai[c] += v[c].x * x.y - v[c].y * x.x;
        }
    }
#pragma unroll
    for (int c = 0; c < CH; ++c) {
        const double r = wave_sum(ar[c]);
        const double m = wave_sum(ai[c]);
        if (lane == 0) {
            red[wave][c][0] = r;
            red[wave][c][1] = m;
        }
    }
    __syncthreads();
    if (tid < CH && tid < nvec) {
        double r = 0.0, m = 0.0;
#pragma unroll
        for (int q = 0; q < TH / 64; ++q) {
            r += red[q][tid][0];
            m += red[q][tid][1];
        }
        if (fix && tid == last) {
            r *= s;
            m *= s;
        }
        partial_out[(int64_t)tid * DOT_BLOCKS + blockIdx.x] = make_double2(r, m);
    }
}

static void launch_axpy_dots(double2* w, double2* V, int64_t ldv, int nvec, const double2* partial_in, double2* c_out,
                             int c_index, double sign, int64_t n, double2* partial_out, const double* norm_prev, int upd0,
                             hipStream_t st) {
#define HTN_AD(CHV, THV)                                                                                                  \
    hipLaunchKernelGGL((k_axpy_dots<CHV, THV, false>), dim3(DOT_BLOCKS), dim3(THV), 0, st, w, V, ldv, nvec, partial_in, c_out, \
                       c_index, sign, n, partial_out, norm_prev, upd0, (const double2*)nullptr, 0)
    HTN_CH_DISPATCH(nvec, dot_slice(n), HTN_AD);
#undef HTN_AD
}
static void launch_axpy_dots_fz(double2* w, double2* V, int64_t ldv, int nvec, const double2* partial_in, double2* c_out,
                                int c_index, double sign, int64_t n, double2* partial_out, const double* norm_prev, int upd0,
                                const double2* Q, int nf, hipStream_t st) {
#define HTN_AD(CHV, THV)                                                                                                 \
    hipLaunchKernelGGL((k_axpy_dots<CHV, THV, true>), dim3(DOT_BLOCKS), dim3(THV), 0, st, w, V, ldv, nvec, partial_in, c_out, \
                       c_index, sign, n, partial_out, norm_prev, upd0, Q, nf)
    HTN_CH_DISPATCH(nvec, dot_slice(n), HTN_AD);
#undef HTN_AD
}

__global__ __launch_bounds__(DOT_THREADS) void k_scale_by_norm(double2* __restrict__ dst, const double2* __restrict__ src,
                                                               const double* __restrict__ norm_partial, int64_t n,
                                                               LanRecord* __restrict__ rec_out,
                                                               const double2* __restrict__ c1, const double2* __restrict__ c2,
                                                               unsigned long long serial) {
    __shared__ double s_inv;
    const int tid = threadIdx.x;
    if (tid < 64) {
        double t = 0.0;
#pragma unroll
        for (int b = 0; b < DOT_BLOCKS / 64; ++b) t += norm_partial[tid + 64 * b];
        t = wave_sum(t);
        if (tid == 0) {
            s_inv = t > 0.0 ? 1.0 / sqrt(t) : 0.0;
            if (blockIdx.x == 0 && rec_out) {
                const unsigned long long w0 = (unsigned long long)__double_as_longlong(c1[0].x);
                const unsigned long long w1 = (unsigned long long)__double_as_longlong(c2[0].x);
                const unsigned long long w2 = (unsigned long long)__double_as_longlong(t);
                ulonglong2* out = (ulonglong2*)rec_out;
                out[0] = make_ulonglong2(w0, w1);
                out[1] = make_ulonglong2(w2, lan_check(w0, w1, w2, serial));
                __threadfence_system();
            }
        }
    }
    __syncthreads();
    const double s = s_inv;
    for (int64_t j = (int64_t)blockIdx.x * DOT_THREADS + tid; j < n; j += (int64_t)gridDim.x * DOT_THREADS) {
        const double2 v = src[j];
        dst[j] = make_double2(v.x * s, v.y * s);
    }
}

__global__ __launch_bounds__(64) void k_publish_record(const double* __restrict__ norm_partial, const double2* __restrict__ c1,
                                                       const double2* __restrict__ c2, LanRecord* __restrict__ rec_out,
                                                       unsigned long long serial) {
    const int tid = threadIdx.x;
    double t = 0.0;
#pragma unroll
    for (int b = 0; b < DOT_BLOCKS / 64; ++b) t += norm_partial[tid + 64 * b];
    t = wave_sum(t);
    if (tid == 0) {
        const unsigned long long w0 = (unsigned long long)__double_as_longlong(c1[0].x);
        const unsigned long long w1 = (unsigned long long)__double_as_longlong(c2[0].x);
        const unsigned long long w2 = (unsigned long long)__double_as_longlong(t);
        ulonglong2* out = (ulonglong2*)rec_out;
        out[0] = make_ulonglong2(w0, w1);
        out[1] = make_ulonglong2(w2, lan_check(w0, w1, w2, serial));
        __threadfence_system();
    }
}

__global__ __launch_bounds__(DOT_THREADS) void k_norm_partial(const double2* __restrict__ w, int64_t n,
                                                              double* __restrict__ norm_partial) {
    __shared__ double red[DOT_THREADS / 64];
    const int tid = threadIdx.x;
    const int64_t per = (n + DOT_BLOCKS - 1) / DOT_BLOCKS;
    const int64_t lo = (int64_t)blockIdx.x * per;
    const int64_t hi = lo + per < n ? lo + per : n;
    double nn = 0.0;
    for (int64_t j = lo + tid; j < hi; j += DOT_THREADS) {
        const double2 x = w[j];
        nn += x.x * x.x + x.y * x.y;
    }
    nn = wave_sum(nn);
    if ((tid & 63) == 0) red[tid >> 6] = nn;
    __syncthreads();
    if (tid == 0) {
        double t = 0.0;
        for (int q = 0; q < DOT_THREADS / 64; ++q) t += red[q];
        norm_partial[blockIdx.x] = t;
    }
}

__global__ __launch_bounds__(256) void k_axpys(double2* __restrict__ w, const double2* __restrict__ V,
                                               int64_t ldv, int nvec, const double2* __restrict__ coef,
                                               double sign, int64_t n) {
    for (int64_t j = (int64_t)blockIdx.x * blockDim.x + threadIdx.x; j < n; j += (int64_t)gridDim.x * blockDim.x) {
        double sr = 0.0, si = 0.0;
        for (int i = 0; i < nvec; ++i) {
            const double2 c = coef[i];
            const double2 v = V[(int64_t)i * ldv + j];
            sr += c.x * v.x - c.y * v.y;
            si += c.x * v.y + c.y * v.x;
        }
        double2 x = w[j];
        x.x += sign * sr;
        x.y += sign * si;
        w[j] = x;
    }
}

__global__ __launch_bounds__(256) void k_scale_inv_sqrt(double2* __restrict__ dst, const double2* __restrict__ src,
                                                        const double2* __restrict__ nrm2, int64_t n) {
    const double s = 1.0 / sqrt(nrm2[0].x);
    for (int64_t j = (int64_t)blockIdx.x * blockDim.x + threadIdx.x; j < n; j += (int64_t)gridDim.x * blockDim.x) {
        const double2 v = src[j];
        dst[j] = make_double2(v.x * s, v.y * s);
    }
}

static inline int grid_for(int64_t n) {
    int64_t b = (n + 255) / 256;
    return (int)(b > 1024 ? 1024 : (b < 1 ? 1 : b));
}

extern "C" int64_t htn_dots_scratch_elems(int32_t nvec) { return (int64_t)nvec * DOT_BLOCKS; }

extern "C" int htn_dots_z(const void* V, int64_t ldv, int32_t nvec, const void* w, int64_t n, void* out,
                          void* scratch, void* stream) {
    if (nvec <= 0) return 0;
    if (nvec > 64) return fail_msg("htn_dots_z: nvec > 64");
    launch_dots_partial((const double2*)V, ldv, nvec, (const double2*)w, n, (double2*)scratch, (hipStream_t)stream);
    hipLaunchKernelGGL(k_dots_reduce, dim3(nvec), dim3(64), 0, (hipStream_t)stream, (const double2*)scratch,
                       nvec, (double2*)out);
    HIP_TRY(hipGetLastError());
    return 0;
}

extern "C" int htn_axpys_z(void* w, const void* V, int64_t ldv, int32_t nvec, const void* coef, double sign,
                           int64_t n, void* stream) {
    if (nvec <= 0 || n <= 0) return 0;
    hipLaunchKernelGGL(k_axpys, dim3(grid_for(n)), dim3(256), 0, (hipStream_t)stream, (double2*)w, (const double2*)V,
                       ldv, nvec, (const double2*)coef, sign, n);
    HIP_TRY(hipGetLastError());
    return 0;
}

extern "C" int htn_scale_inv_sqrt_z(void* dst, const void* src, const void* nrm2, int64_t n, void* stream) {
    if (n <= 0) return 0;
    hipLaunchKernelGGL(k_scale_inv_sqrt, dim3(grid_for(n)), dim3(256), 0, (hipStream_t)stream, (double2*)dst,
                       (const double2*)src, (const double2*)nrm2, n);
    HIP_TRY(hipGetLastError());
    return 0;
}

static int sturm_count(const std::vector<double>& a, const std::vector<double>& b, double x) {
    int cnt = 0;
    double d = 1.0;
    const int k = (int)a.size();
    for (int i = 0; i < k; ++i) {
        const double off = i ? b[i - 1] * b[i - 1] : 0.0;
        d = (a[i] - x) - (i ? off / d : 0.0);
        if (d == 0.0) d = 1e-300;
        if (d < 0.0) ++cnt;
    }
    return cnt;
}

static void tridiag_lowest(const std::vector<double>& alpha, const std::vector<double>& beta, double* eig,
                           std::vector<double>& vec) {
    const int k = (int)alpha.size();
    double lo = alpha[0], hi = alpha[0];
    for (int i = 0; i < k; ++i) {
        const double r = (i ? fabs(beta[i - 1]) : 0.0) + (i + 1 < k ? fabs(beta[i]) : 0.0);
        lo = fmin(lo, alpha[i] - r);
        hi = fmax(hi, alpha[i] + r);
    }
    const double scale = fmax(fabs(lo), fabs(hi)) + 1e-300;
    hi = hi + 1e-12 * scale;
    for (int it = 0; it < 200 && hi - lo > 4e-16 * scale; ++it) {
        const double mid = 0.5 * (lo + hi);
        if (sturm_count(alpha, beta, mid) >= 1) hi = mid;
        else lo = mid;
    }
    const double lam = 0.5 * (lo + hi);
    *eig = lam;
    vec.assign(k, 1.0 / sqrt((double)k));
    if (k == 1) {
        vec[0] = 1.0;
        return;
    }
    const double mu = lam - 1e-10 * scale;
    std::vector<double> d(k), l(k), z(k);
    d[0] = alpha[0] - mu;
    for (int i = 1; i < k; ++i) {
        l[i] = beta[i - 1] / d[i - 1];
        d[i] = (alpha[i] - mu) - l[i] * beta[i - 1];
        if (d[i] == 0.0) d[i] = 1e-300;
    }
    for (int i = 0; i < k; ++i) vec[i] = (i & 1) ? -0.7 : 1.0;
    for (int iter = 0; iter < 4; ++iter) {
        z[0] = vec[0];
        for (int i = 1; i < k; ++i) z[i] = vec[i] - l[i] * z[i - 1];
        z[k - 1] /= d[k - 1];
        for (int i = k - 2; i >= 0; --i) z[i] = z[i] / d[i] - l[i + 1] * z[i + 1];
        double nn = 0.0;
        for (int i = 0; i < k; ++i) nn += z[i] * z[i];
        nn = 1.0 / sqrt(nn);
        for (int i = 0; i < k; ++i) vec[i] = z[i] * nn;
    }
    if (vec[0] < 0.0)
        for (int i = 0; i < k; ++i) vec[i] = -vec[i];
}

extern "C" int64_t htn_lanczos_scratch_elems(int32_t krylovdim) {
    return 2 * (int64_t)(krylovdim + 1) * DOT_BLOCKS + 3 * (krylovdim + 1) + DOT_BLOCKS + 8;
}

#define LAN_SLOTS 64
namespace {
struct LanRes {
    int device = -1;
    LanRecord* h_rec = nullptr;
    LanRecord* d_rec = nullptr;
    double2* h_y = nullptr;
    hipEvent_t ev_done[LAN_SLOTS], ev_mv0[LAN_SLOTS], ev_mv1[LAN_SLOTS];
    bool have_events = false;
    unsigned long long serial = 0;
    unsigned sample = 0;
    ~LanRes() {
        if (device >= 0) (void)hipSetDevice(device);
        if (h_rec) (void)hipHostFree(h_rec);
        if (h_y) (void)hipHostFree(h_y);
        if (have_events)
            for (int i = 0; i < LAN_SLOTS; ++i) {
                (void)hipEventDestroy(ev_done[i]);
                (void)hipEventDestroy(ev_mv0[i]);
                (void)hipEventDestroy(ev_mv1[i]);
            }
    }
};
HtnStreamRegistry<LanRes> g_lan_res;

int lan_res_get(hipStream_t st, LanRes** out) {
    return g_lan_res.get(st, out, [](LanRes& r) -> int {
        HIP_TRY(hipHostMalloc((void**)&r.h_rec, sizeof(LanRecord) * LAN_SLOTS, hipHostMallocMapped | hipHostMallocCoherent));
        memset(r.h_rec, 0, sizeof(LanRecord) * LAN_SLOTS);
        HIP_TRY(hipHostGetDevicePointer((void**)&r.d_rec, r.h_rec, 0));
        HIP_TRY(hipHostMalloc((void**)&r.h_y, sizeof(double2) * LAN_SLOTS, hipHostMallocDefault));
        for (int i = 0; i < LAN_SLOTS; ++i) {
            HIP_TRY(hipEventCreateWithFlags(&r.ev_done[i], hipEventDisableTiming));
            HIP_TRY(hipEventCreate(&r.ev_mv0[i]));
            HIP_TRY(hipEventCreate(&r.ev_mv1[i]));
        }
        r.have_events = true;
        return 0;
    });
}
}

void htn_krylov_release_stream(hipStream_t st) { g_lan_res.release(st); }

static int lanczos_run(const htn_gemm_launch* stages, int32_t n_stages, int32_t x_slot, int32_t y_slot,
                       void* Vv, int64_t n, int32_t krylovdim, double tol, int32_t max_restart,
                       void* scratch, int32_t zero_y, htn_exchange2_fn exchange, void* user,
                       double* eig_host, int32_t* n_matvec_host, double* residual_host,
                       double* matvec_ms_host, void* stream_v, const double2* Q, int nf) {
    hipStream_t st = (hipStream_t)stream_v;
    const int kd = krylovdim;
    const int kt = kd + nf;
    double2* V = (double2*)Vv;
    double2* partial = (double2*)scratch;
    double2* partial2 = partial + (int64_t)(kt + 1) * DOT_BLOCKS;
    double2* c1 = partial2 + (int64_t)(kt + 1) * DOT_BLOCKS;
    double2* c2 = c1 + (kt + 1);
    double2* ycoef = c2 + (kt + 1);
    double* norm_partial = (double*)(ycoef + (kt + 1));

    LanRes* R = nullptr;
    if (lan_res_get(st, &R)) return 1;
    const bool event_waits = htn_debug_event_waits();
    static const bool full_first_pass = htn_env_flag("HTN_LANCZOS_FULL_FIRST_PASS");

    bool timed_step[LAN_SLOTS] = {false};
    unsigned long long step_serial[LAN_SLOTS] = {0};
    auto matvec = [&](double2* x, double2* y, const HtnGemmPublish* pub) -> int {
        if (zero_y) HIP_TRY(hipMemsetAsync(y, 0, sizeof(double2) * n, st));
        bool published = pub == nullptr;
        for (int s = 0; s < n_stages; ++s) {
            const void* bufs[HTN_MAX_BUFS];
            for (int b = 0; b < HTN_MAX_BUFS; ++b) bufs[b] = stages[s].bufs[b];
            bufs[x_slot] = x;
            bufs[y_slot] = y;
            const bool here = !published && stages[s].n_tiles > 0;
            if (htn_grouped_gemm_launch(bufs, stages[s].tiles, stages[s].n_tiles, stages[s].segs, here ? pub : nullptr, st)) return 1;
            published |= here;
        }
        if (!published)
            hipLaunchKernelGGL(k_publish_record, dim3(1), dim3(64), 0, st, pub->norm_partial, pub->c1, pub->c2, pub->rec_out, pub->serial);
        if (exchange && exchange(y, n, user)) return fail_msg("htn_lanczos_z: the exchange hook reported a failure");
        return 0;
    };
    auto enqueue_step = [&](int j, bool first) -> int {
        double2* vj = V + (int64_t)j * n;
        double2* w = V + (int64_t)(j + 1) * n;
        const bool timed = matvec_ms_host && (R->sample % 8) == 0;
        timed_step[j] = timed;
        ++R->sample;
        step_serial[j] = ++R->serial;
        HtnGemmPublish pub = {nullptr, nullptr, nullptr, nullptr, 0ull};
        if (!first) pub = {norm_partial, (const double2*)(c1 + (j - 1)), (const double2*)(c2 + (j - 1)), R->d_rec + (j - 1), step_serial[j - 1]};
        if (timed) HIP_TRY(hipEventRecord(R->ev_mv0[j], st));
        if (matvec(vj, w, first ? nullptr : &pub)) return 1;
        if (timed) HIP_TRY(hipEventRecord(R->ev_mv1[j], st));
        if (!first && event_waits) HIP_TRY(hipEventRecord(R->ev_done[j - 1], st));
        const int upd0 = full_first_pass || j < 2 ? 0 : j - 1;
        if (nf == 0) {
            launch_dots_partial(V + (int64_t)upd0 * n, n, j + 1 - upd0, w, n, partial, st);
            launch_axpy_dots(w, V, n, j + 1, partial, c1 + j, j, -1.0, n, partial2, first ? (const double*)nullptr : norm_partial, upd0, st);
            launch_axpy_norm(w, V, n, j + 1, partial2, c2 + j, j, -1.0, n, norm_partial, st);
        } else {
            launch_dots_partial_fz(V, n, nf + j + 1 - upd0, w, n, partial, Q, nf, upd0, st);
            launch_axpy_dots_fz(w, V, n, nf + j + 1, partial, c1 + j, nf + j, -1.0, n, partial2,
                                first ? (const double*)nullptr : norm_partial, nf + upd0, Q, nf, st);
            launch_axpy_norm_fz(w, V, n, nf + j + 1, partial2, c2 + j, nf + j, -1.0, n, norm_partial, Q, nf, st);
        }
        if (j == kd - 1) {
            hipLaunchKernelGGL(k_publish_record, dim3(1), dim3(64), 0, st, (const double*)norm_partial, (const double2*)(c1 + j),
                               (const double2*)(c2 + j), R->d_rec + j, step_serial[j]);
            if (event_waits) HIP_TRY(hipEventRecord(R->ev_done[j], st));
        }
        return 0;
    };
    auto read_record = [&](int j, double* a1, double* a2, double* nn) -> bool {
        const volatile unsigned long long* p = R->h_rec[j].w;
        const unsigned long long w0 = p[0], w1 = p[1], w2 = p[2], w3 = p[3];
        if (w3 != lan_check(w0, w1, w2, step_serial[j])) return false;
        memcpy(a1, &w0, 8);
        memcpy(a2, &w1, 8);
        memcpy(nn, &w2, 8);
        return true;
    };
    auto wait_step = [&](int j, double* a1, double* a2, double* nn) -> int {
        if (event_waits) {
            HIP_TRY(hipEventSynchronize(R->ev_done[j]));
            if (!read_record(j, a1, a2, nn)) return fail_msg("htn_lanczos_z: the step's event completed but its record does not validate");
            return 0;
        }
        for (unsigned spins = 1;; ++spins) {
            if (read_record(j, a1, a2, nn)) return 0;
            __builtin_ia32_pause();
            if ((spins & 0xffff) == 0) {
                const hipError_t q = hipStreamQuery(st);
                if (q == hipSuccess)
                    return read_record(j, a1, a2, nn) ? 0 : fail_msg("htn_lanczos_z: the stream drained without producing the step's record");
                if (q != hipErrorNotReady) return fail("hipStreamQuery", q);
            }
        }
    };

    auto project_out = [&](double2* w) {
        for (int pass = 0; pass < 2; ++pass) {
            launch_dots_partial(Q, n, nf, w, n, partial, st);
            launch_axpy_norm(w, Q, n, nf, partial, c1, -1, -1.0, n, norm_partial, st);
        }
    };
    if (nf > 0) project_out(V);
    else
    hipLaunchKernelGGL(k_norm_partial, dim3(DOT_BLOCKS), dim3(DOT_THREADS), 0, st, V, n, norm_partial);
    hipLaunchKernelGGL(k_scale_by_norm, dim3(grid_for(n)), dim3(DOT_THREADS), 0, st, V, V, norm_partial, n,
                       (LanRecord*)nullptr, (const double2*)nullptr, (const double2*)nullptr, 0ull);
    double mv_ms = 0.0;
    int nmv = 0, n_timed = 0;
    static const bool dbg_timers = getenv("HTN_DEBUG_HOST_TIMERS") != nullptr;
    auto now_us = [] { return std::chrono::duration<double, std::micro>(std::chrono::steady_clock::now().time_since_epoch()).count(); };
    double t_enq = 0.0, t_wait = 0.0, t_host = 0.0;
    const double t_begin = now_us();
    double theta = 0.0, res = 0.0, beta = 0.0, amax = 0.0;
    std::vector<double> y;
    for (int restart = 0; restart <= max_restart; ++restart) {
        std::vector<double> alphas, betas;
        double tq = now_us();
        if (enqueue_step(0, true)) return 1;
        t_enq += now_us() - tq;
        ++nmv;
        for (int j = 0; j < kd; ++j) {
            if (j + 1 < kd) {
                tq = now_us();
                if (enqueue_step(j + 1, false)) return 1;
                t_enq += now_us() - tq;
                ++nmv;
            }
            double a1 = 0.0, a2 = 0.0, nn = 0.0;
            tq = now_us();
            if (wait_step(j, &a1, &a2, &nn)) return 1;
            t_wait += now_us() - tq;
            tq = now_us();
            if (timed_step[j]) {
                float ms = 0.f;
                HIP_TRY(htn_event_spin(R->ev_mv1[j]));
                HIP_TRY(hipEventElapsedTime(&ms, R->ev_mv0[j], R->ev_mv1[j]));
                mv_ms += ms;
                ++n_timed;
            }
            const double alpha = a1 + a2;
            if (!(alpha == alpha) || !(nn == nn)) return fail_msg("htn_lanczos_z: NaN in the tridiagonal coefficients (operator or start vector not finite)");
            beta = sqrt(nn > 0.0 ? nn : 0.0);
            alphas.push_back(alpha);
            tridiag_lowest(alphas, betas, &theta, y);
            res = fabs(beta * y.back());
            amax = std::max(amax, std::max(fabs(alpha), beta));
            t_host += now_us() - tq;
            if (res < tol || beta < 1e-14 * std::max(amax, 1e-300) || j == kd - 1) break;
            betas.push_back(beta);
        }
        HIP_TRY(htn_stream_spin(st));
        const int k = (int)y.size();
        for (int i = 0; i < k; ++i) R->h_y[i] = make_double2(y[i], 0.0);
        HIP_TRY(hipMemcpyAsync(ycoef, R->h_y, sizeof(double2) * k, hipMemcpyHostToDevice, st));
        double2* xrow = V + (int64_t)(kd + 1) * n;
        HIP_TRY(hipMemsetAsync(xrow, 0, sizeof(double2) * n, st));
        hipLaunchKernelGGL(k_axpys, dim3(grid_for(n)), dim3(256), 0, st, xrow, V, n, k, ycoef, 1.0, n);
        if (nf > 0) project_out(xrow);
        else
        hipLaunchKernelGGL(k_norm_partial, dim3(DOT_BLOCKS), dim3(DOT_THREADS), 0, st, xrow, n, norm_partial);
        hipLaunchKernelGGL(k_scale_by_norm, dim3(grid_for(n)), dim3(DOT_THREADS), 0, st, V, xrow, norm_partial, n,
                           (LanRecord*)nullptr, (const double2*)nullptr, (const double2*)nullptr, 0ull);
        HIP_TRY(htn_stream_spin(st));
        if (res < tol || beta < 1e-14 * std::max(amax, 1e-300)) break;
    }
    HIP_TRY(hipGetLastError());
    if (dbg_timers)
        fprintf(stderr, "lanczos n=%lld: %d matvecs in %.1f us: enqueue %.1f, waiting for records %.1f, tridiagonal %.1f\n", (long long)n, nmv,
                now_us() - t_begin, t_enq, t_wait, t_host);
    *eig_host = theta;
    *n_matvec_host = nmv;
    *residual_host = res;
    if (matvec_ms_host) *matvec_ms_host = n_timed ? mv_ms * nmv / n_timed : -1.0;
    return 0;
}

extern "C" int htn_lanczos_z(const htn_gemm_launch* stages, int32_t n_stages, int32_t x_slot, int32_t y_slot,
                             void* Vv, int64_t n, int32_t krylovdim, double tol, int32_t max_restart,
                             void* scratch, int32_t zero_y, htn_exchange2_fn exchange, void* user,
                             double* eig_host, int32_t* n_matvec_host, double* residual_host,
                             double* matvec_ms_host, void* stream_v) {
    if (krylovdim < 2 || krylovdim + 1 > DOT_CHUNK) return fail_msg("htn_lanczos_z: krylovdim must be in 2..31");
    return lanczos_run(stages, n_stages, x_slot, y_slot, Vv, n, krylovdim, tol, max_restart, scratch, zero_y, exchange, user,
                       eig_host, n_matvec_host, residual_host, matvec_ms_host, stream_v, nullptr, 0);
}

extern "C" int htn_lanczos_orth_z(const htn_gemm_launch* stages, int32_t n_stages, int32_t x_slot, int32_t y_slot,
                                  void* Vv, int64_t n, int32_t krylovdim, double tol, int32_t max_restart,
                                  void* scratch, int32_t zero_y, htn_exchange2_fn exchange, void* user,
                                  double* eig_host, int32_t* n_matvec_host, double* residual_host,
                                  double* matvec_ms_host, const void* Q, int32_t n_frozen, void* stream_v) {
    if (n_frozen < 0 || (n_frozen > 0 && !Q)) return fail_msg("htn_lanczos_orth_z: n_frozen rows need a device pointer Q");
    if (krylovdim < 2 || krylovdim + n_frozen + 1 > DOT_CHUNK)
        return fail_msg("htn_lanczos_orth_z: krylovdim >= 2 and krylovdim + n_frozen <= 31 required");
    return lanczos_run(stages, n_stages, x_slot, y_slot, Vv, n, krylovdim, tol, max_restart, scratch, zero_y, exchange, user,
                       eig_host, n_matvec_host, residual_host, matvec_ms_host, stream_v, (const double2*)Q, n_frozen);
}
```

hubbardtn_amd/csrc/htn_svd.hip:

```cpp
#include <algorithm>
#include <utility>
#include <vector>

#include "htn_common.h"

#define JAC_THREADS 1024
#define JAC_MAXEL 8

template <int GS>
__device__ __forceinline__ double group_sum(double v) {
    v = row_sum16(v);
    if (GS == 16) return v;
    const double a = lane_bcast<0>(v) + lane_bcast<16>(v);
    const double b = lane_bcast<32>(v) + lane_bcast<48>(v);
    if (GS == 32) return (threadIdx.x & 32) ? b : a;
    return a + b;
}

template <int GS>
__device__ __forceinline__ double jacobi_pair(double2* ga, double2* gb, double2* __restrict__ va,
                                              double2* __restrict__ vb, int m, int n, int sub, double tol,
                                              bool accumulate, double zero2) {
    double2 a[JAC_MAXEL], b[JAC_MAXEL];
    double aa = 0.0, bb = 0.0, gr = 0.0, gi = 0.0;
// ... 2090 lines not shown
#else
#define RING_T(var)
#define RING_ACC(slot, a, b)
#endif
struct RingArgs {
    double2* Vj;
    double2* G;
    double* S;
    const htn_svd_block* desc;
    const int* large_ids;
    const RingItem* items;
    const int* perm;
    const double* zero2;
    double2* mbox;
    unsigned* sync;
    int arrive_off, fail_off, conv_off;
    int xcc_off;
    int max_sweeps;
    int two_partner;
    int staged_send;
    double tol;
    int* info;
    int* sweeps_out;
};

template <int GS, int E>
__device__ __forceinline__ void ring_run(const RingArgs A, const RingItem it, const htn_svd_block D, double2* lds, int* s_top, int* s_bot,
                         unsigned long long* s_rbits, int* s_ok, double* s_bnorm, int* s_local, unsigned* s_arr) {
    constexpr int mp = GS * E;
    const int tid = threadIdx.x, lane = tid & 63, wave = tid >> 6;
    const int P = it.P, k = it.k, w = it.w, n = it.n, m = D.m;
    double2* __restrict__ X = A.Vj + D.v_off;
    const int slot_elems = w * mp;
    double2* bufT = lds;
    double2* bufB = lds + slot_elems;
    unsigned* flags = A.sync;
    unsigned* fail = A.sync + A.fail_off;
    const double zero2 = A.zero2[it.li];
    const double tol2 = A.tol * A.tol, thr = fmax(tol2, 0.1 * A.tol);
    auto ncols = [&](int q) {
        const int c = n - q * w;
        return c < 0 ? 0 : (c > w ? w : c);
    };
    if (tid < P) {
        s_top[tid] = 2 * tid;
        s_bot[tid] = 2 * tid + 1;
    }
    if (tid == 0) {
        *s_ok = 1;
        s_arr[0] = s_arr[1] = 0u;
        int local = 0;
        if (P > 1 && A.xcc_off >= 0) {
            unsigned xcc;
            asm volatile("s_getreg_b32 %0, hwreg(HW_REG_XCC_ID)" : "=s"(xcc));
            xcc = (xcc & 0xfu) + 1u;
            unsigned* xw = A.sync + A.xcc_off + it.g0;
            __hip_atomic_store(xw + k, xcc, __ATOMIC_RELAXED, __HIP_MEMORY_SCOPE_AGENT);
            local = 1;
            for (int q = 0; q < P && local >= 0; ++q) {
                if (!ring_wait_ge(xw + q, 1u, fail)) local = -1;
                else if (__hip_atomic_load(xw + q, __ATOMIC_RELAXED, __HIP_MEMORY_SCOPE_AGENT) != xcc) local = local > 0 ? 0 : local;
            }
            if (local < 0) *s_ok = 0;
        }
        *s_local = local > 0 ? 1 : 0;
    }
    __syncthreads();
    const bool local = *s_local != 0;
    {
        const int gsx = m <= 16 * JAC_MAXEL ? 16 : (m <= 32 * JAC_MAXEL ? 32 : 64);
        const int ldx = gsx * ((m + gsx - 1) / gsx);
        for (int side = 0; side < 2; ++side) {
            const int q = side ? s_bot[k] : s_top[k];
            double2* buf = side ? bufB : bufT;
            const int cnt = ncols(q) * mp;
            for (int idx = tid; idx < cnt; idx += RING_THREADS) {
                const int c = idx / mp, i = idx - c * mp;
                buf[idx] = i < m ? X[(int64_t)(q * w + c) * ldx + i] : make_double2(0.0, 0.0);
            }
        }
    }
    __syncthreads();
#ifdef HTN_RING_PROF
    long long prof[16] = {0, 0, 0, 0, 0, 0, 0, 0, 0, 0, 0, 0, 0, 0, 0, 0};
    const long long prof_t0 = wall_clock64();
    long long prof_c0;
    asm volatile("s_memtime %0\n\ts_waitcnt lgkmcnt(0)" : "=s"(prof_c0)::"memory");
#endif
    long long* split = nullptr;
#ifdef HTN_RING_STEP_PROF
    split = prof + 8;
#endif
    int sweeps = 0;
    bool done = n < 2, ok = *s_ok != 0;
    const int rounds = 2 * P - 1;
    const bool direct = A.staged_send == 0;
    double* const s_bscale = s_bnorm + RING_THREADS / 16;
    double* const s_tnorm = s_bnorm + 2 * (RING_THREADS / 16);
    while (!done && ok && sweeps < A.max_sweeps) {
        double ratio = 0.0;
        for (int r = 0; r < rounds && ok; ++r) {
            const unsigned epoch = (unsigned)(sweeps * rounds + r + 1);
            const int par = (int)(epoch & 1u);
            const int nt = ncols(s_top[k]), nb = ncols(s_bot[k]);
            RING_T(p0);
            double2* box = A.mbox + it.mbox;
            double2* const to_t = box + (int64_t)(((k + 1) * 2 + 0) * 2 + par) * slot_elems;
            double2* const to_b = k == 0 ? box + (int64_t)((1 * 2 + 0) * 2 + par) * slot_elems
                                         : box + (int64_t)(((k - 1) * 2 + 1) * 2 + par) * slot_elems;
            const bool send_t = k > 0 && k < P - 1;
            const bool have_t = direct && r > 0 && k > 0, have_b = direct && r > 0 && k < P - 1;
            const bool reg_send = direct && !(GS == 16 && A.two_partner) && P > 1 && nt > 0 && nb > 0;
            RingOut out;
            out.slot_t = __builtin_amdgcn_make_buffer_rsrc((void*)to_t, 0, (reg_send && send_t) ? nt * mp * 16 : 0, 0x00020000);
            out.slot_b = __builtin_amdgcn_make_buffer_rsrc((void*)to_b, 0, reg_send ? nb * mp * 16 : 0, 0x00020000);
            out.send_t = send_t, out.keep_t = !send_t, out.local = local;
            double rr = 0.0;
            if (reg_send) rr = ring_cross<GS, E, false, true>(bufT, bufB, nt, nb, tid, tol2, zero2, s_bnorm, s_bscale, s_tnorm, have_t, have_b, out, split);
            else if (GS == 16 && A.two_partner) {
                if constexpr (GS == 16)
                    rr = ring_cross<GS, E, true, false>(bufT, bufB, nt, nb, tid, tol2, zero2, s_bnorm, s_bscale, s_tnorm, have_t, have_b, out, split);
            } else rr = ring_cross<GS, E, false, false>(bufT, bufB, nt, nb, tid, tol2, zero2, s_bnorm, s_bscale, s_tnorm, have_t, have_b, out, split);
            ratio = rr > ratio ? rr : ratio;
            RING_T(p1);
            RING_ACC(0, p0, p1);
            if (P < 2) continue;
            if (!reg_send) {
                if (send_t) ring_send(bufT, to_t, nt * mp, tid, local);
                ring_send(bufB, to_b, nb * mp, tid, local);
            }
            const int in_top = k == 0 ? s_top[0] : (k == 1 ? s_bot[0] : s_top[k - 1]);
            const int in_bot = k < P - 1 ? s_bot[k + 1] : s_top[P - 1];
            asm volatile("s_waitcnt vmcnt(0)" ::: "memory");
            __syncthreads();
            RING_T(p2);
            RING_ACC(1, p1, p2);
            const int half = k == 0 ? 1 : (k == P - 1 ? 0 : wave >> 2);
            const bool both = k > 0 && k < P - 1;
            if (tid == 0) {
                if (k == 0) ring_flag(flags + (it.g0 + 1) * 2 + 0, epoch, local);
                else {
                    if (k < P - 1) ring_flag(flags + (it.g0 + k + 1) * 2 + 0, epoch, local);
                    ring_flag(flags + (it.g0 + k - 1) * 2 + 1, epoch, local);
                }
                const int t_last = s_top[P - 1], b0 = s_bot[0];
                for (int q = P - 1; q >= 2; --q) s_top[q] = s_top[q - 1];
                s_top[1] = b0;
                for (int q = 0; q + 1 < P; ++q) s_bot[q] = s_bot[q + 1];
                s_bot[P - 1] = t_last;
                if (!direct) {
                    bool good = true;
                    if (k > 0) good = ring_wait_ge(flags + (it.g0 + k) * 2 + 0, epoch, fail);
                    if (good && k < P - 1) good = ring_wait_ge(flags + (it.g0 + k) * 2 + 1, epoch, fail);
                    if (!good) *s_ok = 0;
                }
            }
            if (k == P - 1) {
                double2* t = bufT;
                bufT = bufB;
                bufB = t;
            }
            if (!direct) {
                __syncthreads();
                RING_T(p3);
                RING_ACC(2, p2, p3);
                ok = *s_ok != 0;
                if (ok) {
                    const double2* mine = box + (int64_t)(k * 4) * slot_elems;
                    if (k > 0) ring_recv(bufT, mine + (int64_t)(0 * 2 + par) * slot_elems, ncols(s_top[k]) * mp, tid);
                    if (k < P - 1) ring_recv(bufB, mine + (int64_t)(1 * 2 + par) * slot_elems, ncols(s_bot[k]) * mp, tid);
                }
                __syncthreads();
                RING_T(p4);
                RING_ACC(3, p3, p4);
            } else {
                if (tid == (both ? half * (RING_THREADS / 2) : 0)) {
                    const bool good = ring_wait_ge(flags + (it.g0 + k) * 2 + half, epoch, fail);
                    if (!good) *s_ok = 0;
                    __hip_atomic_store(s_arr + half, good ? epoch : ~0u, __ATOMIC_RELEASE, __HIP_MEMORY_SCOPE_WORKGROUP);
                }
                unsigned seen;
                while ((seen = __hip_atomic_load(s_arr + half, __ATOMIC_ACQUIRE, __HIP_MEMORY_SCOPE_WORKGROUP)) < epoch)
                    __builtin_amdgcn_s_sleep(1);
                RING_T(p3);
                RING_ACC(2, p2, p3);
                if (seen != ~0u) {
                    const double2* mine = box + (int64_t)(k * 4 + half * 2 + par) * slot_elems;
                    const int ngt = RING_THREADS / GS, ng = both ? ngt / 2 : ngt, grp = tid / GS;
                    ring_recv_cols<GS, E>(half ? bufB : bufT, mine, ncols(half ? in_bot : in_top), both ? grp % ng : grp, ng, tid % GS,
                                          half ? s_bnorm : s_tnorm, half ? s_bscale : nullptr);
                }
                __syncthreads();
                RING_T(p4);
                RING_ACC(3, p3, p4);
                ok = *s_ok != 0;
            }
        }
        if (!ok) break;
        RING_T(p5);
        {
            const double rr = ring_intra<GS, E>(bufT, ncols(s_top[k]), bufB, ncols(s_bot[k]), tid, tol2, zero2);
            ratio = rr > ratio ? rr : ratio;
        }
        RING_T(p6);
        RING_ACC(4, p5, p6);
        if (tid == 0) *s_rbits = 0ull;
        __syncthreads();
        {
            const unsigned long long key = wave_max_u64((unsigned long long)__double_as_longlong(ratio));
            if (lane == 0 && key) atomicMax(s_rbits, key);
        }
        __syncthreads();
        if (tid == 0) {
            unsigned long long* conv = (unsigned long long*)(A.sync + A.conv_off) + (int64_t)it.li * A.max_sweeps + sweeps;
            unsigned* arrive = A.sync + A.arrive_off + it.li * A.max_sweeps + sweeps;
            unsigned long long mx = *s_rbits;
            if (P > 1) {
                const unsigned long long old = __hip_atomic_fetch_max(conv, mx, __ATOMIC_RELAXED, __HIP_MEMORY_SCOPE_AGENT);
                asm volatile("s_waitcnt vmcnt(0)" ::: "memory");
                (void)old;
                __hip_atomic_fetch_add(arrive, 1u, __ATOMIC_RELAXED, __HIP_MEMORY_SCOPE_AGENT);
                if (ring_wait_ge(arrive, (unsigned)P, fail)) mx = __hip_atomic_load(conv, __ATOMIC_RELAXED, __HIP_MEMORY_SCOPE_AGENT);
                else *s_ok = 0;
            }
            *s_rbits = mx;
        }
        __syncthreads();
        ok = *s_ok != 0;
        ++sweeps;
        done = __longlong_as_double((long long)*s_rbits) <= thr;
        __syncthreads();
        RING_T(p7);
        RING_ACC(5, p6, p7);
    }
#ifdef HTN_RING_PROF
    if (tid == 0 && blockIdx.x < 256) {
        prof[6] = wall_clock64() - prof_t0;
        prof[7] = (local ? 1000000 : 0) + sweeps * 1000 + P;
        long long prof_c1;
        asm volatile("s_memtime %0\n\ts_waitcnt lgkmcnt(0)" : "=s"(prof_c1)::"memory");
        prof[15] = prof_c1 - prof_c0;
        for (int q = 0; q < 16; ++q) g_ring_prof[blockIdx.x * 16 + q] = prof[q];
    }
#endif
    double2* __restrict__ g = A.G + D.g_off;
    const int* __restrict__ pc = A.perm + it.li * 64 * JAC_MAXEL;
    for (int side = 0; side < 2; ++side) {
        const double2* buf = side ? bufB : bufT;
        const int q = side ? s_bot[k] : s_top[k];
        const int nc = ncols(q);
        for (int c = wave; c < nc; c += RING_THREADS / 64) {
            const int col = q * w + c;
            double sn = 0.0;
            for (int i = lane; i < m; i += 64) {
                const double2 x = buf[c * mp + i];
                sn += x.x * x.x + x.y * x.y;
                g[(int64_t)col * m + pc[i]] = x;
            }
            sn = wave_sum(sn);
            if (lane == 0) A.S[D.s_off + col] = sqrt(sn);
        }
    }
    for (int col = n + k * (RING_THREADS / 64) + wave; col < D.n; col += P * (RING_THREADS / 64)) {
        for (int i = lane; i < m; i += 64) g[(int64_t)col * m + i] = make_double2(0.0, 0.0);
        if (lane == 0) A.S[D.s_off + col] = 0.0;
    }
    if (k == 0 && tid == 0) {
        A.info[A.large_ids[it.li]] = (done && ok) ? sweeps : -(sweeps > 0 ? sweeps : 1);
        A.sweeps_out[it.li] = ok ? sweeps + ((local || P == 1) ? 1000 : 0) : 0;
        __threadfence_system();
    }
}

__global__ __launch_bounds__(RING_THREADS) void k_jacobi_ring(RingArgs A) {
    extern __shared__ double2 g_lds[];
    __shared__ int s_top[RING_MAX_P], s_bot[RING_MAX_P];
    __shared__ unsigned long long s_rbits;
    __shared__ int s_ok, s_local;
    __shared__ double s_bnorm[3 * (RING_THREADS / 16)];
    __shared__ unsigned s_arr[2];
    const RingItem it = A.items[blockIdx.x];
    if (it.P <= 0) return;
    const htn_svd_block D = A.desc[A.large_ids[it.li]];
    const int m = D.m;
    const int gs = ring_gs(m), E = ring_e(m);
#define RING_CASE(GSV, EV) \
    case EV: ring_run<GSV, EV>(A, it, D, g_lds, s_top, s_bot, &s_rbits, &s_ok, s_bnorm, &s_local, s_arr); break;
    if (gs == 16) {
        switch (E) {
            RING_CASE(16, 1) RING_CASE(16, 2) RING_CASE(16, 3) RING_CASE(16, 4) RING_CASE(16, 5) RING_CASE(16, 6) RING_CASE(16, 7)
            RING_CASE(16, 8) RING_CASE(16, 9) RING_CASE(16, 10) RING_CASE(16, 11) RING_CASE(16, 12) RING_CASE(16, 13)
            RING_CASE(16, 14) RING_CASE(16, 15)
            default: ring_run<16, 16>(A, it, D, g_lds, s_top, s_bot, &s_rbits, &s_ok, s_bnorm, &s_local, s_arr);
        }
    } else {
        switch (E) {
            RING_CASE(64, 5) RING_CASE(64, 6) RING_CASE(64, 7)
            default: ring_run<64, 8>(A, it, D, g_lds, s_top, s_bot, &s_rbits, &s_ok, s_bnorm, &s_local, s_arr);
        }
    }
#undef RING_CASE
}

struct JacScratch {
    int device = -1;
    int cu_count = 0;
    int xcd_local = 0;
    HtnBuf dev{HTN_BUF_DEVICE};
    HtnBuf pinned{HTN_BUF_PINNED};
    HtnBuf flags{HTN_BUF_MAPPED};
    HtnBuf ring_sync{HTN_BUF_DEVICE, false};
    HtnBuf ring_items{HTN_BUF_DEVICE, false};
    HtnBuf ring_items_h{HTN_BUF_PINNED};
    HtnBuf ring_mbox{HTN_BUF_DEVICE};
    HtnBuf qr_box{HTN_BUF_DEVICE};
    HtnBuf tall_dev{HTN_BUF_DEVICE};
    HtnBuf tall_pin{HTN_BUF_PINNED};
    HtnBuf tall_flags{HTN_BUF_MAPPED};
    hipStream_t aux = nullptr;
    hipEvent_t ev_fork = nullptr, ev_join = nullptr, ev_sweep[2] = {nullptr, nullptr};
    ~JacScratch() {
        if (device >= 0) (void)hipSetDevice(device);
        if (aux) {
            (void)hipStreamSynchronize(aux);
            (void)hipStreamDestroy(aux);
        }
        for (hipEvent_t ev : {ev_fork, ev_join, ev_sweep[0], ev_sweep[1]})
            if (ev) (void)hipEventDestroy(ev);
    }
};
static HtnStreamRegistry<JacScratch> g_js_res;

void htn_svd_release_stream(hipStream_t st) { g_js_res.release(st); }

static int js_get(hipStream_t st, JacScratch** out) {
    return g_js_res.get(st, out, [](JacScratch& js) -> int {
        HIP_TRY(hipDeviceGetAttribute(&js.cu_count, hipDeviceAttributeMultiprocessorCount, js.device));
        HIP_TRY(hipStreamCreateWithFlags(&js.aux, hipStreamNonBlocking));
        HIP_TRY(hipEventCreateWithFlags(&js.ev_fork, hipEventDisableTiming));
        HIP_TRY(hipEventCreateWithFlags(&js.ev_join, hipEventDisableTiming));
        HIP_TRY(hipEventCreateWithFlags(&js.ev_sweep[0], hipEventDisableTiming));
        HIP_TRY(hipEventCreateWithFlags(&js.ev_sweep[1], hipEventDisableTiming));
        return 0;
    });
}

struct JacTournament {
    std::vector<JacPairItem> items;
    std::vector<size_t> off;
    int n_rounds() const { return (int)off.size() - 1; }
    unsigned round_size(int r) const { return (unsigned)(off[r + 1] - off[r]); }
};
static JacTournament jacobi_tournament(const int* n_cols, int n_blk) {
    const int w = JAC_PANEL;
    std::vector<std::vector<JacPairItem>> rounds;
    std::vector<JacPairItem> intra;
    for (int li = 0; li < n_blk; ++li) {
        const int n = n_cols[li];
        if (n < 1) continue;
        const int nb = (n + w - 1) / w;
        const int nbp = nb + (nb & 1);
        if ((int)rounds.size() < nbp - 1) rounds.resize(nbp - 1);
        for (int r = 0; r < nbp - 1; ++r)
            for (int p = 0; p < nbp / 2; ++p) {
                int a = p == 0 ? nbp - 1 : (r + p) % (nbp - 1);
                int c = p == 0 ? r : (r + nbp - 1 - p) % (nbp - 1);
                if (a >= nb || c >= nb) continue;
                if (a > c) std::swap(a, c);
                JacPairItem it = {li, a * w, std::min(w, n - a * w), c * w, std::min(w, n - c * w), {0, 0, 0}};
                rounds[r].push_back(it);
            }
        for (int a = 0; a < nb; a += 2) {
            const int c = a + 1;
            JacPairItem it = {li, a * w, std::min(w, n - a * w), c < nb ? c * w : 0,
                              c < nb ? std::min(w, n - c * w) : 0, {1, 0, 0}};
            intra.push_back(it);
        }
    }
    rounds.push_back(intra);
    JacTournament T;
    for (auto& rl : rounds) {
        T.off.push_back(T.items.size());
        T.items.insert(T.items.end(), rl.begin(), rl.end());
    }
    T.off.push_back(T.items.size());
    return T;
}
static int upload_tournament(const JacTournament& T, JacPairItem* h_items, JacPairItem* d_items, hipStream_t st) {
    if (T.items.empty()) return 0;
    memcpy(h_items, T.items.data(), sizeof(JacPairItem) * T.items.size());
    HIP_TRY(hipMemcpyAsync(d_items, h_items, sizeof(JacPairItem) * T.items.size(), hipMemcpyHostToDevice, st));
    return 0;
}

template <class Enqueue>
static int jacobi_sweep_pipeline(int max_sweeps, int hint, hipEvent_t* ev_sweep, const volatile int* h_active,
                                 hipStream_t st, Enqueue enqueue) {
    hipError_t err = hipSuccess;
    int enq = 0, used = 0;
    auto enqueue_next = [&]() {
        enqueue(enq);
        err = hipEventRecord(ev_sweep[enq & 1], st);
        ++enq;
    };
    if (max_sweeps > 0) enqueue_next();
    for (int sweep = 0; sweep < max_sweeps && err == hipSuccess; ++sweep) {
        const bool expect_last = hint > 0 && sweep + 1 >= hint;
        if (sweep + 1 < max_sweeps && !expect_last && enq == sweep + 1) enqueue_next();
        if (err == hipSuccess) err = htn_event_spin(ev_sweep[sweep & 1]);
        if (err != hipSuccess) break;
        used = sweep + 1;
        if (h_active[sweep] == 0) break;
        if (sweep + 1 < max_sweeps && enq == sweep + 1) enqueue_next();
    }
    return err == hipSuccess ? used : -htn_fail("jacobi_sweep_pipeline", err);
}

struct JacCall {
    double2 *G, *Vj;
    double* S;
    const htn_svd_block *desc, *desc_host;
    int n_blocks, max_sweeps;
    double tol, cut2;
    int split;
    int32_t* info_dev;
    hipStream_t st;
    std::vector<int> large;
    std::vector<int> n_eff;
    int nl() const { return (int)large.size(); }
};
static int jac_padded_rows(int m) {
    const int gsx = m <= 16 * JAC_MAXEL ? 16 : (m <= 32 * JAC_MAXEL ? 32 : 64);
    return gsx * ((m + gsx - 1) / gsx);
}
static const int JAC_LDS_ELEMS = 9216;

static int jac_set_kernel_attributes() {
    static std::mutex attr_mu;
    static bool attr_set[64] = {};
    int dev = 0;
    HIP_TRY(hipGetDevice(&dev));
    std::lock_guard<std::mutex> lk(attr_mu);
    if (dev >= 0 && dev < 64 && !attr_set[dev]) {
        HIP_TRY(hipFuncSetAttribute((const void*)k_jacobi_svd, hipFuncAttributeMaxDynamicSharedMemorySize,
                                    JAC_LDS_ELEMS * (int)sizeof(double2)));
        HIP_TRY(hipFuncSetAttribute((const void*)k_qr_large, hipFuncAttributeMaxDynamicSharedMemorySize,
                                    16 * (64 * JAC_MAXEL + 1) * (int)sizeof(double2)));
        HIP_TRY(hipFuncSetAttribute((const void*)k_jacobi_pairs_gram, hipFuncAttributeMaxDynamicSharedMemorySize,
                                    (16 * (64 * JAC_MAXEL + 1) + JG_GU_ELEMS) * (int)sizeof(double2)));
        HIP_TRY(hipFuncSetAttribute((const void*)k_jacobi_ring, hipFuncAttributeMaxDynamicSharedMemorySize,
                                    2 * RING_PANEL_ELEMS * (int)sizeof(double2)));
        attr_set[dev] = true;
    }
    return 0;
}

static std::vector<int> classify_large(const htn_svd_block* desc_host, int n_blocks, int split) {
    const int large_min = split > 0 ? std::min(split, JAC_LDS_ELEMS) : JAC_LDS_ELEMS;
    std::vector<int> large;
    if (desc_host)
        for (int b = 0; b < n_blocks; ++b) {
            const htn_svd_block& D = desc_host[b];
            if (!(D.flags & HTN_SVD_QRCP) || D.n < 2) continue;
            if ((int64_t)jac_padded_rows(D.m) * D.n > large_min) large.push_back(b);
        }
    return large;
}

struct JacCoreBufs {
    int *d_ids, *d_slot, *d_perm;
    double* d_zero;
    unsigned long long* d_ratio;
    int *d_done, *d_sw;
    unsigned* d_qsync;
    JacPairItem* d_items;
    JacPairItem* h_items;
    int *h_ids, *h_slot;
    volatile int *h_active, *h_rank, *h_ring_sw;
    int *d_active, *d_rank, *d_ring_sw;
};
static int carve_core_scratch(JacScratch& js, int nl, int n_blocks, int max_sweeps, size_t n_items_max, JacCoreBufs* B) {
    const size_t off_ids = 0, off_slot = off_ids + sizeof(int) * nl, off_perm = off_slot + sizeof(int) * n_blocks;
    const size_t off_zero = off_perm + sizeof(int) * nl * 64 * JAC_MAXEL;
    const size_t off_ratio = (off_zero + sizeof(double) * nl + 7) / 8 * 8, off_done = off_ratio + 8 * nl;
    const size_t off_sw = off_done + sizeof(int) * nl, off_qsync = off_sw + sizeof(int) * nl;
    const size_t off_items = (off_qsync + sizeof(unsigned) * (QR_SYNC_WORDS * (size_t)nl + 8) + 31) / 32 * 32;
    if (js.dev.reserve(off_items + sizeof(JacPairItem) * n_items_max)) return 1;
    if (js.pinned.reserve(sizeof(JacPairItem) * n_items_max + 4 * (size_t)(nl + n_blocks) + 128)) return 1;
    if (js.flags.reserve(sizeof(int) * ((size_t)(max_sweeps + 1) + 2 * (size_t)nl + 16))) return 1;
    char* d = (char*)js.dev.p;
    B->d_ids = (int*)(d + off_ids);
    B->d_slot = (int*)(d + off_slot);
    B->d_perm = (int*)(d + off_perm);
    B->d_zero = (double*)(d + off_zero);
    B->d_ratio = (unsigned long long*)(d + off_ratio);
    B->d_done = (int*)(d + off_done);
    B->d_sw = (int*)(d + off_sw);
    B->d_qsync = (unsigned*)(d + off_qsync);
    B->d_items = (JacPairItem*)(d + off_items);
    char* h = (char*)js.pinned.p;
    B->h_items = (JacPairItem*)h;
    B->h_ids = (int*)(h + sizeof(JacPairItem) * n_items_max);
    B->h_slot = B->h_ids + nl;
    B->h_active = (volatile int*)js.flags.p;
    B->h_rank = B->h_active + (max_sweeps + 1);
    B->h_ring_sw = B->h_rank + nl;
    B->d_active = (int*)js.flags.dev;
    B->d_rank = B->d_active + (max_sweeps + 1);
    B->d_ring_sw = B->d_rank + nl;
    return 0;
}

struct RingPlan {
    std::vector<RingItem> items;
    std::vector<std::pair<int, int>> batches;
    int wgs = 0;
    int64_t mbox_elems = 0;
};
static bool plan_ring(const JacCall& c, int n_xcd, int ring_cap, RingPlan* plan) {
    *plan = RingPlan();
    struct Blk {
        int li, P, w, mp;
    };
    std::vector<Blk> blks;
    for (int li = 0; li < c.nl(); ++li) {
        const htn_svd_block& D = c.desc_host[c.large[li]];
        const int gsx = ring_gs(D.m);
        const int mp = gsx * ring_e(D.m);
        int wcap = std::min(RING_THREADS / gsx, RING_PANEL_ELEMS / mp);
        if (gsx == 16 && wcap > 16 && wcap < 32) wcap = 16;
        if (c.split > 0) wcap = std::min(wcap, 3);
        const int n = std::max(c.n_eff[li], 1);
        const int P = std::max(1, (n + 2 * wcap - 1) / (2 * wcap));
        if (wcap < 1 || P > RING_MAX_P || P > ring_cap) return false;
        blks.push_back({li, P, (n + 2 * P - 1) / (2 * P), mp});
    }
    std::stable_sort(blks.begin(), blks.end(), [](const Blk& a, const Blk& b) { return a.P > b.P; });
    std::vector<char> placed(blks.size(), 0);
    size_t left = blks.size();
    int nx = n_xcd;
    for (const Blk& B : blks)
        if (B.P > ring_cap / nx) nx = 1;
    const int lane_cap = ring_cap / nx;
    while (left) {
        const int first = (int)plan->items.size();
        std::vector<int> lane_used((size_t)nx, 0);
        struct Put {
            int q, x, s0;
        };
        std::vector<Put> puts;
        for (size_t q = 0; q < blks.size(); ++q) {
            if (placed[q]) continue;
            int x = 0;
            for (int y = 1; y < nx; ++y)
                if (lane_used[y] < lane_used[x]) x = y;
            if (lane_used[x] + blks[q].P > lane_cap) continue;
            puts.push_back({(int)q, x, lane_used[x]});
            lane_used[x] += blks[q].P;
            placed[q] = 1;
            --left;
        }
        int depth = 0;
        for (int y = 0; y < nx; ++y) depth = std::max(depth, lane_used[y]);
        const int grid = depth * nx;
        plan->items.resize((size_t)first + grid, RingItem{0, 0, 0, 0, 0, 0, 0});
        for (const Put& pt : puts) {
            const Blk& B = blks[pt.q];
            for (int k = 0; k < B.P; ++k)
                plan->items[(size_t)first + (size_t)(pt.s0 + k) * nx + pt.x] = {B.li, k, B.P, B.w, c.n_eff[B.li], plan->wgs,
                                                                                 plan->mbox_elems};
            plan->mbox_elems += (int64_t)B.P * 4 * B.w * B.mp;
            plan->wgs += B.P;
        }
        plan->batches.push_back({first, grid});
    }
    return true;
}

static int launch_qr_large(const JacCall& c, JacScratch& js, const JacCoreBufs& B, int n_xcd) {
    const int nl = c.nl();
    int max_m0 = 0, min_m0 = 1 << 30, max_n0 = 0;
    for (int b : c.large) {
        max_m0 = std::max(max_m0, (int)c.desc_host[b].pad);
        min_m0 = std::min(min_m0, (int)c.desc_host[b].pad);
        max_n0 = std::max(max_n0, (int)c.desc_host[b].m);
    }
    const size_t qr_panel_elems = (size_t)16 * (((max_m0 + 15) & ~15) + 1);
    const bool coop = ((min_m0 + 15) & ~15) <= 256 && qr_panel_elems * sizeof(double2) + 65536 + 30720 <= 163840;
    const size_t qr_lds = qr_panel_elems * sizeof(double2) + (coop ? 65536 : 0);
    static const bool qr_single = htn_env_flag("HTN_QR_SINGLE");
    static const int env_nw = getenv("HTN_QR_NW") ? atoi(getenv("HTN_QR_NW")) : 0;
    int NW = qr_single ? 1 : ((max_n0 >= 160 || js.xcd_local) ? 4 : 1);
    if (env_nw > 0 && !qr_single) NW = std::min(env_nw, 4);
    const int cus = std::max(1, std::min(js.cu_count > 0 ? js.cu_count : 256, 256));
    const int qnx = (NW > 1 && n_xcd > 1) ? n_xcd : 1;
    const int nl_pad = (nl + qnx - 1) / qnx * qnx;
    NW = std::max(1, std::min(NW, cus / std::max(nl_pad, 1)));
    if (NW > 1 && js.qr_box.reserve((size_t)nl * QR_BOX_BYTES)) return 1;
    const int qgrid_nx = NW > 1 ? qnx : 1;
    hipLaunchKernelGGL(k_qr_large, dim3((NW > 1 ? nl_pad : nl) * NW), dim3(JAC_THREADS), qr_lds, c.st, c.G, c.Vj, c.desc, B.d_ids,
                       B.d_perm, B.d_zero, c.cut2, B.d_rank, NW, (char*)js.qr_box.p, B.d_qsync, nl, qgrid_nx,
                       coop ? (int)qr_panel_elems : 0);
    return 0;
}

static int run_ring(const JacCall& c, JacScratch& js, const JacCoreBufs& B, const RingPlan& plan, int n_xcd, bool two_partner,
                    bool staged_send, int32_t* sweeps_used) {
    const int nl = c.nl(), n_wg = plan.wgs, n_items = (int)plan.items.size();
    const int arrive_off = 2 * n_wg, fail_off = arrive_off + nl * c.max_sweeps, xcc_off = fail_off + 1;
    const int conv_off = (xcc_off + n_wg + 3) & ~3;
    const size_t sync_bytes = ((size_t)conv_off * 4 + (size_t)nl * c.max_sweeps * 8 + 15) & ~(size_t)15;
    if (js.ring_sync.reserve(sync_bytes)) return 1;
    if (js.ring_mbox.reserve(sizeof(double2) * (size_t)std::max<int64_t>(plan.mbox_elems, 1))) return 1;
    if (js.ring_items.reserve(sizeof(RingItem) * n_items) || js.ring_items_h.reserve(sizeof(RingItem) * n_items)) return 1;
    memcpy(js.ring_items_h.p, plan.items.data(), sizeof(RingItem) * n_items);
    for (int li = 0; li < nl; ++li) B.h_ring_sw[li] = 0;
    HIP_TRY(hipMemcpyAsync(js.ring_items.p, js.ring_items_h.p, sizeof(RingItem) * n_items, hipMemcpyHostToDevice, c.st));
    HIP_TRY(hipMemsetAsync(js.ring_sync.p, 0, sync_bytes, c.st));
    RingArgs ra;
    ra.Vj = c.Vj, ra.G = c.G, ra.S = c.S, ra.desc = c.desc, ra.large_ids = B.d_ids;
    ra.perm = B.d_perm, ra.zero2 = B.d_zero, ra.mbox = (double2*)js.ring_mbox.p, ra.sync = (unsigned*)js.ring_sync.p;
    ra.arrive_off = arrive_off, ra.fail_off = fail_off, ra.conv_off = conv_off, ra.max_sweeps = c.max_sweeps, ra.tol = c.tol;
    ra.xcc_off = xcc_off;
    ra.two_partner = two_partner ? 1 : 0;
    ra.staged_send = staged_send ? 1 : 0;
    ra.info = c.info_dev, ra.sweeps_out = B.d_ring_sw;
    for (auto& bt : plan.batches) {
        ra.items = (const RingItem*)js.ring_items.p + bt.first;
        hipLaunchKernelGGL(k_jacobi_ring, dim3((unsigned)bt.second), dim3(RING_THREADS), 2 * RING_PANEL_ELEMS * sizeof(double2),
                           c.st, ra);
    }
    HIP_TRY(hipGetLastError());
    HIP_TRY(hipStreamWaitEvent(c.st, js.ev_join, 0));
    HIP_TRY(htn_stream_spin(c.st));
    int used = 0;
    for (int li = 0; li < nl; ++li) {
        if (B.h_rank[li] < 0) return fail_msg("htn_jacobi_svd_z: a hand-off of the multi-workgroup QR timed out");
        if (B.h_ring_sw[li] <= 0 && c.n_eff[li] >= 2)
            return fail_msg("htn_jacobi_svd_z: a hand-off of the ring Jacobi kernel timed out");
        used = std::max(used, (int)B.h_ring_sw[li] % 1000);
    }
    int all_local = n_xcd > 1 ? 1 : 0;
    for (int li = 0; li < nl; ++li)
        if (c.n_eff[li] >= 2 && B.h_ring_sw[li] < 1000) all_local = 0;
    js.xcd_local = all_local;
    if (sweeps_used) *sweeps_used = used;
    return 0;
}

static int run_pair_visits(const JacCall& c, JacScratch& js, const JacCoreBufs& B, const JacTournament& T, int hint,
                           int32_t* sweeps_used) {
    const int nl = c.nl();
    int max_mp = 0;
    for (int b : c.large) max_mp = std::max(max_mp, jac_padded_rows(c.desc_host[b].m));
    const size_t gram_lds_bytes = (size_t)(16 * (max_mp + 1) + JG_GU_ELEMS) * sizeof(double2);
    const double thr = std::max(c.tol * c.tol, 0.1 * c.tol);
    const int used = jacobi_sweep_pipeline(c.max_sweeps, hint, js.ev_sweep, B.h_active, c.st, [&](int sweep) {
        for (int r = 0; r < T.n_rounds(); ++r)
            if (T.round_size(r))
                hipLaunchKernelGGL(k_jacobi_pairs_gram, dim3(T.round_size(r)), dim3(256), gram_lds_bytes, c.st, c.Vj, c.desc,
                                   B.d_ids, B.d_items + T.off[r], B.d_zero, B.d_ratio, B.d_done, c.tol, 1);
        hipLaunchKernelGGL(k_jacobi_check, dim3(1), dim3(64), 0, c.st, B.d_ratio, B.d_done, B.d_sw, nl, thr, B.d_active + sweep);
    });
    if (used < 0) return 1;
    if (sweeps_used) *sweeps_used = used;
    HIP_TRY(hipStreamWaitEvent(c.st, js.ev_join, 0));
    hipLaunchKernelGGL(k_jacobi_finish, dim3(nl), dim3(JAC_THREADS), 0, c.st, c.G, (const double2*)c.Vj, c.S, c.desc, B.d_ids,
                       B.d_perm, B.d_sw, B.d_done, c.info_dev);
    HIP_TRY(hipGetLastError());
    HIP_TRY(htn_stream_spin(c.st));
    return 0;
}

static int jacobi_svd_core(void* G, void* Vj, double* S, const htn_svd_block* desc, const htn_svd_block* desc_host,
                           int32_t n_blocks, int32_t max_m_host, int32_t max_sweeps, double tol, int32_t* info_dev,
                           const htn_svd_opts* opts, void* stream, const int* skip_dev, const unsigned char* skip_host) {
    if (n_blocks <= 0) return 0;
    if (max_m_host > 64 * JAC_MAXEL) return fail_msg("htn_jacobi_svd_z: block taller than 512 rows");
    const double rank_cut = opts && opts->rank_cut > 0.0 ? opts->rank_cut : 0.0;
    JacCall c = {(double2*)G, (double2*)Vj, S, desc, desc_host, n_blocks, max_sweeps, tol, rank_cut * rank_cut,
                 opts && opts->split_elems > 0 ? opts->split_elems : 0, info_dev, (hipStream_t)stream, {}, {}};
    int32_t* sweeps_used = opts ? opts->sweeps_used : nullptr;
    if (jac_set_kernel_attributes()) return 1;
    c.large = classify_large(desc_host, n_blocks, c.split);
    if (sweeps_used) *sweeps_used = 0;
    if (c.large.empty()) {
        hipLaunchKernelGGL(k_jacobi_svd, dim3(n_blocks), dim3(JAC_THREADS), JAC_LDS_ELEMS * sizeof(double2), c.st, c.G, c.Vj, S,
                           desc, max_sweeps, tol, info_dev, JAC_LDS_ELEMS, skip_dev, c.cut2);
        HIP_TRY(hipGetLastError());
        return 0;
    }
    const int nl = c.nl();
    size_t n_items_max = 0;
    for (int b : c.large) {
        const int nb = (desc_host[b].n + JAC_PANEL - 1) / JAC_PANEL, nbp = nb + (nb & 1);
        n_items_max += (size_t)(nbp - 1) * (nbp / 2) + (nb + 1) / 2;
        c.n_eff.push_back(desc_host[b].n);
    }
    JacScratch* jsp = nullptr;
    JacCoreBufs B;
    if (js_get(c.st, &jsp) || carve_core_scratch(*jsp, nl, n_blocks, max_sweeps, n_items_max, &B)) return 1;
    JacScratch& js = *jsp;
    for (int b = 0; b < n_blocks; ++b) B.h_slot[b] = skip_host && skip_host[b] ? nl : -1;
    for (int li = 0; li < nl; ++li) B.h_slot[c.large[li]] = li;
    for (int li = 0; li < nl; ++li) B.h_ids[li] = c.large[li];
    for (int k = 0; k <= max_sweeps; ++k) B.h_active[k] = 1;
    HIP_TRY(hipMemcpyAsync(B.d_ids, B.h_ids, sizeof(int) * (nl + n_blocks), hipMemcpyHostToDevice, c.st));
    HIP_TRY(hipMemsetAsync(B.d_ratio, 0, 16 * (size_t)nl + sizeof(unsigned) * (QR_SYNC_WORDS * (size_t)nl + 8), c.st));
    static const bool force_pairs = htn_env_flag("HTN_SVD_PAIRS");
    static const bool no_xcd = htn_env_flag("HTN_RING_NO_XCD");
    static const bool ring_staged = htn_env_flag("HTN_RING_STAGED_SEND");
    const bool ring_two_partner = htn_env_flag("HTN_RING_TWO_PARTNER");
    const int n_xcd = (!no_xcd && js.cu_count > 0 && js.cu_count % 8 == 0) ? 8 : 1;
    const int ring_cap = std::max(1, std::min(js.cu_count > 0 ? js.cu_count : 256, 256));
    RingPlan plan;
    JacTournament T;
    bool use_ring = !force_pairs && plan_ring(c, n_xcd, ring_cap, &plan);
    if (c.cut2 <= 0.0 && !use_ring) {
        T = jacobi_tournament(c.n_eff.data(), nl);
        if (upload_tournament(T, B.h_items, B.d_items, c.st)) return 1;
    }
    HIP_TRY(hipEventRecord(js.ev_fork, c.st));
    HIP_TRY(hipStreamWaitEvent(js.aux, js.ev_fork, 0));
    hipLaunchKernelGGL(k_jacobi_svd, dim3(n_blocks), dim3(JAC_THREADS), JAC_LDS_ELEMS * sizeof(double2), js.aux, c.G, c.Vj, S,
                       desc, max_sweeps, tol, info_dev, JAC_LDS_ELEMS, (const int*)B.d_slot, c.cut2);
    HIP_TRY(hipEventRecord(js.ev_join, js.aux));
    if (launch_qr_large(c, js, B, n_xcd)) return 1;
    if (c.cut2 > 0.0) {
        HIP_TRY(hipEventRecord(js.ev_sweep[0], c.st));
        HIP_TRY(htn_event_spin(js.ev_sweep[0]));
        for (int li = 0; li < nl; ++li) c.n_eff[li] = std::min(c.n_eff[li], (int)B.h_rank[li]);
        if (use_ring) use_ring = plan_ring(c, n_xcd, ring_cap, &plan);
        if (!use_ring) {
            T = jacobi_tournament(c.n_eff.data(), nl);
            if (upload_tournament(T, B.h_items, B.d_items, c.st)) return 1;
        }
    }
    if (use_ring) return run_ring(c, js, B, plan, n_xcd, ring_two_partner, ring_staged, sweeps_used);
    return run_pair_visits(c, js, B, T, opts && opts->sweeps_hint > 0 ? opts->sweeps_hint : 0, sweeps_used);
}

static int jacobi_svd_tall(void* G, void* Vj, double* S, const htn_svd_block* desc, const htn_svd_block* desc_host,
                           int32_t n_blocks, int32_t max_m_rest, int32_t max_sweeps, double tol, int32_t* info_dev,
                           const htn_svd_opts* opts, void* stream, const std::vector<int>& tall) {
    const int nt = (int)tall.size();
    hipStream_t st = (hipStream_t)stream;
    JacScratch* jsp = nullptr;
    if (js_get(st, &jsp)) return 1;
    JacScratch& js = *jsp;
    std::vector<int> n_cols(nt);
    for (int li = 0; li < nt; ++li) n_cols[li] = desc_host[tall[li]].n;
    const JacTournament T = jacobi_tournament(n_cols.data(), nt);
    const size_t n_items = T.items.size();
    const size_t off_skip = 0, off_ids = off_skip + sizeof(int) * n_blocks;
    const size_t off_zero = (off_ids + sizeof(int) * nt + 7) / 8 * 8, off_part = off_zero + sizeof(double) * nt;
    const size_t off_ratio = off_part + sizeof(double) * nt * TALL_PARTS, off_done = off_ratio + 8 * (size_t)nt;
    const size_t off_sw = off_done + sizeof(int) * nt, off_items = (off_sw + sizeof(int) * nt + 31) / 32 * 32;
    const size_t flag_elems = (size_t)std::max(max_sweeps, 0) + 1;
    if (js.tall_dev.reserve(off_items + sizeof(JacPairItem) * std::max<size_t>(n_items, 1))) return 1;
    if (js.tall_pin.reserve(sizeof(JacPairItem) * std::max<size_t>(n_items, 1) + sizeof(int) * (n_blocks + nt))) return 1;
    if (js.tall_flags.reserve(sizeof(int) * flag_elems)) return 1;
    char* d = (char*)js.tall_dev.p;
    int* d_skip = (int*)(d + off_skip);
    int* d_ids = (int*)(d + off_ids);
    double* d_zero = (double*)(d + off_zero);
    double* d_part = (double*)(d + off_part);
    unsigned long long* d_ratio = (unsigned long long*)(d + off_ratio);
    int* d_done = (int*)(d + off_done);
    int* d_sw = (int*)(d + off_sw);
    JacPairItem* d_items = (JacPairItem*)(d + off_items);
    JacPairItem* h_items = (JacPairItem*)js.tall_pin.p;
    int* h_skip = (int*)((char*)js.tall_pin.p + sizeof(JacPairItem) * std::max<size_t>(n_items, 1));
    int* h_ids = h_skip + n_blocks;
    volatile int* h_active = (volatile int*)js.tall_flags.p;
    int* d_active = (int*)js.tall_flags.dev;
    std::vector<unsigned char> skip(n_blocks, 0);
    for (int li = 0; li < nt; ++li) skip[tall[li]] = 1;
    for (int b = 0; b < n_blocks; ++b) h_skip[b] = skip[b] ? 0 : -1;
    for (int li = 0; li < nt; ++li) h_ids[li] = tall[li];
    for (size_t k = 0; k < flag_elems; ++k) h_active[k] = 1;
    HIP_TRY(hipMemcpyAsync(d_skip, h_skip, sizeof(int) * (n_blocks + nt), hipMemcpyHostToDevice, st));
    if (upload_tournament(T, h_items, d_items, st)) return 1;
    HIP_TRY(hipMemsetAsync(d_ratio, 0, 16 * (size_t)nt, st));
    int core_used = 0;
    if (nt < n_blocks) {
        if (jacobi_svd_core(G, Vj, S, desc, desc_host, n_blocks, max_m_rest, max_sweeps, tol, info_dev, opts, stream, d_skip,
                            skip.data()))
            return 1;
        if (opts && opts->sweeps_used) core_used = *opts->sweeps_used;
    }
    int max_n = 1;
    for (int li = 0; li < nt; ++li) max_n = std::max(max_n, (int)desc_host[tall[li]].n);
    hipLaunchKernelGGL(k_jacobi_tall_init, dim3(nt, TALL_PARTS), dim3(256), 0, st, (double2*)G, (double2*)Vj, desc, d_ids, d_part);
    hipLaunchKernelGGL(k_jacobi_tall_zero, dim3(1), dim3(64), 0, st, (const double*)d_part, d_zero, nt);
    HIP_TRY(hipGetLastError());
    const double thr = std::max(tol * tol, 0.1 * tol);
    const int hint = opts && opts->sweeps_hint > 0 ? opts->sweeps_hint : 0;
    const int used = jacobi_sweep_pipeline(max_sweeps, hint, js.ev_sweep, h_active, st, [&](int sweep) {
        for (int r = 0; r < T.n_rounds(); ++r)
            if (T.round_size(r))
                hipLaunchKernelGGL(k_jacobi_tall_visit, dim3(T.round_size(r)), dim3(TALL_THREADS), 0, st, (double2*)G,
                                   (double2*)Vj, desc, d_ids, d_items + T.off[r], d_zero, d_ratio, d_done, tol);
        hipLaunchKernelGGL(k_jacobi_check, dim3(1), dim3(64), 0, st, d_ratio, d_done, d_sw, nt, thr, d_active + sweep);
    });
    if (used < 0) return 1;
    hipLaunchKernelGGL(k_jacobi_tall_finish, dim3((unsigned)((max_n + 3) / 4), (unsigned)nt), dim3(256), 0, st,
                       (const double2*)G, S, desc, d_ids, d_sw, d_done, info_dev);
    HIP_TRY(hipGetLastError());
    HIP_TRY(htn_stream_spin(st));
    if (opts && opts->sweeps_used) *opts->sweeps_used = std::max(core_used, used);
    return 0;
}

extern "C" int htn_jacobi_svd_z(void* G, void* Vj, double* S, const htn_svd_block* desc,
                                const htn_svd_block* desc_host, int32_t n_blocks, int32_t max_m_host,
                                int32_t max_sweeps, double tol, int32_t* info_dev, const htn_svd_opts* opts,
                                void* stream) {
    if (n_blocks <= 0) return 0;
    std::vector<int> tall;
    int max_m_rest = 0;
    if (desc_host) {
        for (int b = 0; b < n_blocks; ++b) {
            const htn_svd_block& D = desc_host[b];
            if (!(D.flags & HTN_SVD_QRCP) && D.m > 64 * JAC_MAXEL) tall.push_back(b);
            else max_m_rest = std::max(max_m_rest, std::max(D.m, D.pad));
        }
    } else if (max_m_host > 64 * JAC_MAXEL) {
        return fail_msg("htn_jacobi_svd_z: blocks taller than 512 rows need the host copy of the descriptors (desc_host)");
    }
    if (tall.empty())
        return jacobi_svd_core(G, Vj, S, desc, desc_host, n_blocks, max_m_host, max_sweeps, tol, info_dev, opts, stream,
                               nullptr, nullptr);
    if (max_m_rest > 64 * JAC_MAXEL) return fail_msg("htn_jacobi_svd_z: block taller than 512 rows");
    return jacobi_svd_tall(G, Vj, S, desc, desc_host, n_blocks, max_m_rest, max_sweeps, tol, info_dev, opts, stream, tall);
}

__global__ __launch_bounds__(256) void k_batched_copy(double2* __restrict__ dst, const double2* __restrict__ src,
                                                      const int32_t* __restrict__ idx,
                                                      const double* __restrict__ scl,
                                                      const htn_copy_item* __restrict__ items, double gscale) {
    const htn_copy_item I = items[blockIdx.x];
    const int total = I.rows * I.cols;
    for (int e = blockIdx.y * blockDim.x + threadIdx.x; e < total; e += blockDim.x * gridDim.y) {
        const int i = e % I.rows, j = e / I.rows;
        int gi = i, gj = j;
        if (I.idx_off >= 0) {
            if (I.gather_dim == 0) gi = idx[I.idx_off + i];
            else gj = idx[I.idx_off + j];
        }
        double2 v;
        if (I.op == HTN_OP_N) v = src[I.src_off + (int64_t)gi + (int64_t)gj * I.lds];
        else {
            v = src[I.src_off + (int64_t)gj + (int64_t)gi * I.lds];
            v.y = -v.y;
        }
        double f = gscale;
        if (I.scale_dim >= 0 && I.scl_off >= 0) {
            const double sv = scl[I.scl_off + (I.scale_dim == 0 ? gi : gj)];
            f = I.inv_norm ? (sv > 0.0 ? f / sv : 0.0) : f * sv;
        }
        dst[I.dst_off + (int64_t)i + (int64_t)j * I.ldd] = make_double2(v.x * f, v.y * f);
    }
}

extern "C" int htn_batched_copy_z(void* dst, const void* src, const int32_t* idx, const double* scl,
                                  const htn_copy_item* items, int32_t n_items, double global_scale,
                                  void* stream) {
    if (n_items <= 0) return 0;
    hipLaunchKernelGGL(k_batched_copy, dim3(n_items, 16), dim3(256), 0, (hipStream_t)stream, (double2*)dst,
                       (const double2*)src, idx, scl, items, global_scale);
    HIP_TRY(hipGetLastError());
    return 0;
}
```

include/hubbardtn_hip.h:

```cpp
#ifndef HUBBARDTN_HIP_H
#define HUBBARDTN_HIP_H

#include <stdint.h>

#ifdef __cplusplus
extern "C" {
#endif

#define HTN_ABI_VERSION 2
#define HTN_MAX_BUFS 8
#define HTN_TILE 32

#define HTN_OP_N 0
#define HTN_OP_T 1
#define HTN_OP_C 2
#define HTN_SEG_GEMM 0
#define HTN_SEG_COPY 1

typedef struct {
    int64_t c_off;
    int32_t buf_c;
    int32_t ldc;
    int32_t m, n;
    int32_t row0, col0;
    int32_t seg_begin, seg_count;
    int32_t pad[2];
    int32_t part, nparts;
    int32_t ws_slot;
    int32_t ticket;
} htn_tile;
#define HTN_BUF_WS 7
#define HTN_WS_TICKET_ELEMS 4096
#define HTN_WS_ELEMS(n_slots) (HTN_WS_TICKET_ELEMS + (int64_t)(n_slots) * HTN_TILE * HTN_TILE)

typedef struct {
    int64_t a_off, b_off;
    int32_t buf_a, buf_b;
    int32_t lda, ldb;
    int32_t k;
    int32_t op_a, op_b;
    int32_t type;
    double alpha_re, alpha_im;
} htn_seg;

const char* htn_last_error(void);
int htn_abi_version(void);

int htn_device_init(int device, char* name_host, int* cu_count_host);

int htn_grouped_gemm_z(const void* const* bufs_host, const htn_tile* tiles, int32_t n_tiles,
                       const htn_seg* segs, void* stream);

int64_t htn_dots_scratch_elems(int32_t nvec);
int htn_dots_z(const void* V, int64_t ldv, int32_t nvec, const void* w, int64_t n,
               void* out, void* scratch, void* stream);
int htn_axpys_z(void* w, const void* V, int64_t ldv, int32_t nvec, const void* coef,
                double sign, int64_t n, void* stream);
int htn_scale_inv_sqrt_z(void* dst, const void* src, const void* nrm2, int64_t n, void* stream);

typedef struct {
    const void* bufs[HTN_MAX_BUFS];
    const htn_tile* tiles;
    const htn_seg* segs;
    int32_t n_tiles;
    int32_t pad;
} htn_gemm_launch;
typedef int (*htn_exchange2_fn)(void* y_dev, int64_t n, void* user);
int64_t htn_lanczos_scratch_elems(int32_t krylovdim);
int htn_lanczos_z(const htn_gemm_launch* stages_host, int32_t n_stages, int32_t x_slot, int32_t y_slot,
                  void* V, int64_t n, int32_t krylovdim, double tol, int32_t max_restart, void* scratch,
                  int32_t zero_y, htn_exchange2_fn exchange, void* user,
                  double* eig_host, int32_t* n_matvec_host, double* residual_host,
                  double* matvec_ms_host ,
                  void* stream);
int htn_lanczos_orth_z(const htn_gemm_launch* stages_host, int32_t n_stages, int32_t x_slot, int32_t y_slot,
                       void* V, int64_t n, int32_t krylovdim, double tol, int32_t max_restart, void* scratch,
                       int32_t zero_y, htn_exchange2_fn exchange, void* user,
                       double* eig_host, int32_t* n_matvec_host, double* residual_host, double* matvec_ms_host,
                       const void* Q, int32_t n_frozen, void* stream);

#define HTN_SVD_ACCUMULATE 1
#define HTN_SVD_QRCP 2
typedef struct {
    int64_t g_off, v_off, s_off;
    int32_t m, n;
    int32_t flags, pad;
} htn_svd_block;
typedef struct {
    int32_t split_elems;
    int32_t sweeps_hint;
    double rank_cut;
    int32_t* sweeps_used;
} htn_svd_opts;
int htn_jacobi_svd_z(void* G, void* Vj, double* S, const htn_svd_block* desc, const htn_svd_block* desc_host,
                     int32_t n_blocks, int32_t max_m_host, int32_t max_sweeps, double tol, int32_t* info_dev,
                     const htn_svd_opts* opts, void* stream);

typedef struct {
    int64_t dst_off, src_off, idx_off, scl_off;
    int32_t rows, cols;
    int32_t ldd, lds;
    int32_t op;
    int32_t gather_dim;
    int32_t scale_dim;
    int32_t inv_norm;
} htn_copy_item;
int htn_batched_copy_z(void* dst, const void* src, const int32_t* idx, const double* scl,
                       const htn_copy_item* items, int32_t n_items, double global_scale,
                       void* stream);

#define HTN_QR_PANEL 16
#define HTN_QR_CHUNK 512
#define HTN_QR_MAX_M 7664
typedef struct {
    int64_t offset;
    int32_t m, n;
    int32_t ld, pad;
    int64_t r_offset;
    int32_t ldr, trans;
} htn_qr_block;
int htn_qr_blocks_z(void* A, void* Rbuf, const htn_qr_block* desc, const htn_qr_block* desc_host, int32_t n_blocks,
                    void* stream);


#define HTN_TRDOT_SLOTS 16
typedef struct {
    int64_t a_off, b_off;
    int32_t rows, cols;
    int32_t lda, ldb;
    int32_t out;
    int32_t pad[3];
    double w_re, w_im;
} htn_trdot_item;
int64_t htn_trdots_scratch_elems(int32_t n_items);
int htn_block_trdots_z(const void* A, const void* B, const htn_trdot_item* items, int32_t n_items,
                       void* out, int32_t n_out, void* scratch, void* stream);


typedef struct htn_ctx htn_ctx;
typedef struct htn_mpo htn_mpo;
typedef struct htn_mps htn_mps;

#define HTN_SYM_SU2_U1 0
#define HTN_SYM_U1_U1 1
#define HTN_SYM_SU2 2
#define HTN_MAX_SITE 4
typedef struct {
    int32_t kind;
    int32_t n_site;
    int32_t site_N[HTN_MAX_SITE];
    int32_t site_j[HTN_MAX_SITE];
} htn_symmetry;

typedef struct {
    int32_t k, dN;
    double red[HTN_MAX_SITE * HTN_MAX_SITE];
} htn_site_op;

typedef struct {
    int32_t wl, wr;
    int32_t op;
    int32_t pad;
    double coef_re, coef_im;
} htn_mpo_entry;

typedef struct {
    int32_t lN, lj, s, rN, rj;
    int32_t ld;
    int64_t off;
} htn_subblock;

typedef struct {
    int32_t N, j, count;
} htn_sector;

typedef struct {
    int32_t chi_full;
    int32_t weighting;
    double cutoff;
    int32_t krylovdim;
    int32_t maxrestart;
    double lanczos_tol;
    double jacobi_tol;
    int32_t jacobi_max_sweeps;
    int32_t svd_split_elems;
    double rank_cut;
    int32_t profile;
    int32_t pad;
} htn_sweep_opts;

typedef struct {
    int32_t bond, direction;
    int32_t n_matvec, jacobi_sweeps;
    int32_t chi_full, multiplets;
    int32_t n_tiles, n_segs;
    int64_t theta_size;
    int64_t apply_flops, apply_bytes, svd_flops;
    double energy, residual, trunc_weight;
    double t_plan, t_lanczos, t_svd, t_env, t_total;
    double matvec_ms;
} htn_bond_stats;

#define HTN_BACKEND_CPU 0
#define HTN_BACKEND_HIP 1
int htn_ctx_create(int32_t backend, int32_t device, void* stream, htn_ctx** out);
void htn_ctx_destroy(htn_ctx* ctx);
int htn_ctx_backend(const htn_ctx* ctx);
int htn_ctx_set_timing(htn_ctx* ctx, int32_t on);

#define HTN_COMM_ID_BYTES 128
int htn_comm_unique_id(void* id_host);
int htn_ctx_set_comm(htn_ctx* ctx, int32_t rank, int32_t world, const void* id_host);
int htn_ctx_set_exchange(htn_ctx* ctx, int32_t rank, int32_t world, htn_exchange2_fn fn, void* user);

int htn_mpo_create(htn_ctx* ctx, const htn_symmetry* sym, int32_t nsites, const htn_site_op* ops_host, int32_t n_ops,
                   const int32_t* level_ptr_host, const int32_t* levels_host, const int32_t* entry_ptr_host,
                   const htn_mpo_entry* entries_host, htn_mpo** out);
void htn_mpo_destroy(htn_mpo* mpo);

int htn_mps_create(htn_ctx* ctx, const htn_mpo* mpo, int32_t nsites, const int32_t* bond_ptr_host,
                   const htn_sector* sectors_host, const int32_t* sub_ptr_host, const htn_subblock* subs_host,
                   const int64_t* data_ptr_host, const void* data_host, const void* left_env_host,
                   const void* right_env_host, htn_mps** out);
void htn_mps_destroy(htn_mps* mps);

int htn_bond_update(htn_mps* mps, int32_t i, int32_t direction, int32_t placement, int32_t optimise,
                    const htn_sweep_opts* opts, htn_bond_stats* stats_host);
int htn_dmrg2_sweep(htn_mps* mps, const htn_sweep_opts* opts, htn_bond_stats* stats_host, double* energy_host);

int htn_site_update(htn_mps* mps, int32_t i, int32_t direction, int32_t optimise, const htn_sweep_opts* opts,
                    htn_bond_stats* stats_host);
int htn_dmrg1_sweep(htn_mps* mps, const htn_sweep_opts* opts, htn_bond_stats* stats_host, double* energy_host);
int32_t htn_mps_centre(const htn_mps* mps);
int64_t htn_mps_site_theta_size(htn_mps* mps, int32_t i);
int htn_heff1_apply(htn_mps* mps, int32_t i, const void* x_host, void* y_host);

int htn_mps_set_orthogonal(htn_mps* mps, const htn_mps* const* others_host, int32_t n);
int32_t htn_mps_orthogonal_count(const htn_mps* mps, int32_t* dropped_host);
int htn_mps_overlap(htn_mps* a, const htn_mps* b, double* out_host);

typedef struct {
    htn_site_op open, pass, close;
    htn_site_op onsite;
    int32_t has_onsite, pad;
} htn_corr_channel;
int htn_mps_correlator(htn_mps* mps, const htn_corr_channel* ch, void* out_host, double* norm_host);

int64_t htn_mps_theta_size(htn_mps* mps, int32_t i);
int htn_heff2_apply(htn_mps* mps, int32_t i, const void* x_host, void* y_host);
int htn_mps_get_theta(htn_mps* mps, int32_t i, void* theta_host);

int32_t htn_mps_nsites(const htn_mps* mps);
int32_t htn_mps_bond(const htn_mps* mps, int32_t b, htn_sector* sectors_host);
int64_t htn_mps_spectrum(const htn_mps* mps, int32_t b, htn_sector* sectors_host, double* values_host);
int64_t htn_mps_site_size(const htn_mps* mps, int32_t i, int32_t* kind_host);
int32_t htn_mps_get_site(const htn_mps* mps, int32_t i, htn_subblock* subs_host, void* data_host);
int64_t htn_mps_env_size(const htn_mps* mps, int32_t side, int32_t b);
int htn_mps_get_env(const htn_mps* mps, int32_t side, int32_t b, void* data_host);
typedef struct {
    int32_t aN, aj, w, bN, bj;
    int32_t rows, cols;
    int32_t pad;
    int64_t off;
} htn_env_block;
int32_t htn_mps_env_blocks(const htn_mps* mps, int32_t side, int32_t b, htn_env_block* blocks_host);
int32_t htn_mps_env_bond(const htn_mps* mps, int32_t side, int32_t b, htn_sector* sectors_host);
int htn_plan_apply_dump(htn_mps* mps, int32_t i, int32_t stage, int32_t* n_tiles, htn_tile* tiles_host, int32_t* n_segs,
                        htn_seg* segs_host, int64_t* z_size, int64_t* flops);
int32_t htn_balance_tiles(const htn_tile* tiles_host, int32_t n_tiles, int32_t n_cus, htn_tile* out_host, int32_t out_cap,
                          int32_t* n_out);
int htn_mps_cache_stats(const htn_mps* mps, int64_t* hits, int64_t* misses);

typedef struct htn_idmrg htn_idmrg;
typedef struct {
    htn_sweep_opts sweep;
    int32_t cell_sites;
    int32_t window_dN;
    double tol;
    int32_t min_steps;
    int32_t maxiter;
    int32_t sweeps_per_step;
    int32_t warm_start;
} htn_idmrg_opts;
typedef struct {
    int32_t step;
    int32_t sweeps;
    int32_t converged;
    int32_t finished;
    int32_t needs_window;
    int32_t chi_full;
    double energy;
    double energy_per_site;
    double delta;
} htn_idmrg_stats;
int htn_idmrg_create(htn_ctx* ctx, const htn_mpo* window_mpo, const htn_idmrg_opts* opts, htn_idmrg** out);
void htn_idmrg_destroy(htn_idmrg* idmrg);
int32_t htn_idmrg_boundary(const htn_idmrg* idmrg, int32_t side, htn_sector* sectors_host);
int htn_idmrg_step(htn_idmrg* idmrg, const int32_t* bond_ptr_host, const htn_sector* sectors_host,
                   const int32_t* sub_ptr_host, const htn_subblock* subs_host, const int64_t* data_ptr_host,
                   const void* data_host, htn_idmrg_stats* stats_host);
int htn_idmrg_window(htn_idmrg* idmrg, htn_mps** out);

#ifdef __cplusplus
}
#endif
#endif
```

Measured before the change: 406.1 ms.

## Defer Jacobi ring SVD host sync, prestage ring items, fuse Ritz vector kernel

Splits the ring Jacobi SVD into an enqueue and a later collect step, so the host no longer spins on the stream right after launch. The flag checks now run after the singular-value download, which already synchronises. Ring items and sync words are carved into the core scratch and uploaded in one memcpy and one memset, replacing separate uploads. In Lanczos, the Ritz vector memset, host coefficient upload and axpy become one kernel that takes its coefficients by value, and the last restart skips the trailing stream spin. This adds bookkeeping for pending state, which errors if a call is not collected before the next one.

```diff
diff --git a/hubbardtn_amd/abi.py b/hubbardtn_amd/abi.py
--- a/hubbardtn_amd/abi.py
+++ b/hubbardtn_amd/abi.py
@@ -107,7 +107,7 @@
 
 EXPORTS = ["htn_last_error", "htn_abi_version", "htn_device_init", "htn_grouped_gemm_z",
            "htn_dots_scratch_elems", "htn_dots_z", "htn_axpys_z", "htn_scale_inv_sqrt_z",
-           "htn_jacobi_svd_z", "htn_batched_copy_z", "htn_lanczos_scratch_elems", "htn_lanczos_z", "htn_lanczos_orth_z",
+           "htn_jacobi_svd_z", "htn_jacobi_collect_check", "htn_batched_copy_z", "htn_lanczos_scratch_elems", "htn_lanczos_z", "htn_lanczos_orth_z",
            "htn_trdots_scratch_elems", "htn_block_trdots_z"]
 ENGINE_EXPORTS = ["htn_ctx_create", "htn_ctx_destroy", "htn_ctx_backend", "htn_ctx_set_timing", "htn_comm_unique_id",
                   "htn_ctx_set_comm", "htn_ctx_set_exchange", "htn_mpo_create", "htn_mpo_destroy", "htn_mps_create",
@@ -156,6 +156,7 @@
     lib.htn_axpys_z.argtypes = [vp, vp, i64, i32, vp, f64, i64, vp]
     lib.htn_scale_inv_sqrt_z.argtypes = [vp, vp, vp, i64, vp]
     lib.htn_jacobi_svd_z.argtypes = [vp, vp, vp, vp, vp, i32, i32, i32, f64, vp, C.POINTER(SvdOpts), vp]
+    lib.htn_jacobi_collect_check.argtypes = [vp, vp, vp, i32, i32, C.POINTER(i32), C.POINTER(i32)]
     lib.htn_batched_copy_z.argtypes = [vp, vp, vp, vp, vp, i32, f64, vp]
     lib.htn_lanczos_scratch_elems.argtypes = [i32]
     lib.htn_lanczos_scratch_elems.restype = i64
diff --git a/hubbardtn_amd/csrc/htn_backend_hip.hip b/hubbardtn_amd/csrc/htn_backend_hip.hip
--- a/hubbardtn_amd/csrc/htn_backend_hip.hip
+++ b/hubbardtn_amd/csrc/htn_backend_hip.hip
@@ -270,6 +270,15 @@
         fork_open = false;
         return rc;
     }
+    int jacobi_svd_enqueue(void* G, void* Vj, double* S, const htn_svd_block* desc_dev, const htn_svd_block* desc_host,
+                           int n_blocks, int max_m, int max_sweeps, double tol, int32_t* info_dev,
+                           const htn_svd_opts* opts) override {
+        fork_open = true;
+        const int rc = htn_jacobi_svd_enqueue(G, Vj, S, desc_dev, desc_host, n_blocks, max_m, max_sweeps, tol, info_dev, opts, st);
+        fork_open = false;
+        return rc;
+    }
+    int jacobi_svd_collect() override { return htn_jacobi_svd_collect(st); }
     int qr_blocks(void* A, void* R, const htn_qr_block* desc_dev, const htn_qr_block* desc_host, int n_blocks) override {
         return htn_qr_blocks_z(A, R, desc_dev, desc_host, n_blocks, st);
     }
diff --git a/hubbardtn_amd/csrc/htn_common.h b/hubbardtn_amd/csrc/htn_common.h
--- a/hubbardtn_amd/csrc/htn_common.h
+++ b/hubbardtn_amd/csrc/htn_common.h
@@ -150,6 +150,11 @@
 void htn_krylov_release_stream(hipStream_t st);
 void htn_svd_release_stream(hipStream_t st);
 
+int htn_jacobi_svd_enqueue(void* G, void* Vj, double* S, const htn_svd_block* desc, const htn_svd_block* desc_host,
+                           int32_t n_blocks, int32_t max_m_host, int32_t max_sweeps, double tol, int32_t* info_dev,
+                           const htn_svd_opts* opts, void* stream);
+int htn_jacobi_svd_collect(void* stream);
+
 template <int CTRL>
 __device__ __forceinline__ double dpp_f64(double v) {
     const int lo = __builtin_amdgcn_update_dpp(0, __double2loint(v), CTRL, 0xF, 0xF, true);
diff --git a/hubbardtn_amd/csrc/htn_core.h b/hubbardtn_amd/csrc/htn_core.h
--- a/hubbardtn_amd/csrc/htn_core.h
+++ b/hubbardtn_amd/csrc/htn_core.h
@@ -295,6 +295,12 @@
     virtual int jacobi_svd(void* G, void* Vj, double* S, const htn_svd_block* desc_dev, const htn_svd_block* desc_host,
                            int n_blocks, int max_m, int max_sweeps, double tol, int32_t* info_dev,
                            const htn_svd_opts* opts) = 0;
+    virtual int jacobi_svd_enqueue(void* G, void* Vj, double* S, const htn_svd_block* desc_dev, const htn_svd_block* desc_host,
+                                   int n_blocks, int max_m, int max_sweeps, double tol, int32_t* info_dev,
+                                   const htn_svd_opts* opts) {
+        return jacobi_svd(G, Vj, S, desc_dev, desc_host, n_blocks, max_m, max_sweeps, tol, info_dev, opts);
+    }
+    virtual int jacobi_svd_collect() { return 0; }
     virtual int batched_copy(void* dst, const void* src, const int32_t* idx, const double* scl,
                              const htn_copy_item* items_dev, int n_items, double gscale) = 0;
     virtual int scale(void* x, int64_t n, double f) = 0;
diff --git a/hubbardtn_amd/csrc/htn_engine.cpp b/hubbardtn_amd/csrc/htn_engine.cpp
--- a/hubbardtn_amd/csrc/htn_engine.cpp
+++ b/hubbardtn_amd/csrc/htn_engine.cpp
@@ -923,18 +923,21 @@
             cut = o.rank_cut * h->second.second;
         so.rank_cut = std::max(cut, o.rank_cut * o.cutoff);
     }
-    if (run && be->jacobi_svd(w.G.ptr(), w.Vj.ptr(), (double*)w.S->p, (const htn_svd_block*)desc_dev->p, desc_host, n_run, sp.max_m,
-                              o.jacobi_max_sweeps, o.jacobi_tol, info_dev, &so))
+    if (run && (svd_shard ? be->jacobi_svd(w.G.ptr(), w.Vj.ptr(), (double*)w.S->p, (const htn_svd_block*)desc_dev->p, desc_host, n_run,
+                                           sp.max_m, o.jacobi_max_sweeps, o.jacobi_tol, info_dev, &so)
+                          : be->jacobi_svd_enqueue(w.G.ptr(), w.Vj.ptr(), (double*)w.S->p, (const htn_svd_block*)desc_dev->p, desc_host,
+                                                   n_run, sp.max_m, o.jacobi_max_sweeps, o.jacobi_tol, info_dev, &so)))
         return 1;
     if (svd_shard) {
         if (exchange_tramp(w.G.ptr(), std::max<int64_t>(sp.g_size, 1), ctx)) return set_error("sharded SVD: exchange of the blocks failed");
         if (exchange_tramp(w.S->p, (int64_t)(s_elems / 2), ctx)) return set_error("sharded SVD: exchange of the singular values failed");
         if (sp.any_accumulate && exchange_tramp(w.Vj.ptr(), std::max<int64_t>(sp.v_size, 1), ctx)) return 1;
     }
-    if (jac_used > 0) sweeps_hint[i + 1] = jac_used;
     w.tA = now();
     w.s_host.resize(s_elems + (i_elems + 1) / 2);
     if (be->download(w.s_host.data(), w.S->p, s_bytes)) return 1;
+    if (run && !svd_shard && be->jacobi_svd_collect()) return 1;
+    if (jac_used > 0) sweeps_hint[i + 1] = jac_used;
     w.tB = now();
     const int32_t* info_h = (const int32_t*)(w.s_host.data() + s_elems);
     for (int b = 0; b < n_run; ++b) {
diff --git a/hubbardtn_amd/csrc/htn_krylov.hip b/hubbardtn_amd/csrc/htn_krylov.hip
--- a/hubbardtn_amd/csrc/htn_krylov.hip
+++ b/hubbardtn_amd/csrc/htn_krylov.hip
@@ -399,6 +399,23 @@
     }
 }
 
+struct RitzCoef {
+    double2 c[DOT_CHUNK];
+};
+__global__ __launch_bounds__(256) void k_ritz_vector(double2* __restrict__ x, const double2* __restrict__ V, int64_t ldv, int nvec,
+                                                     const RitzCoef coef, int64_t n) {
+    for (int64_t j = (int64_t)blockIdx.x * blockDim.x + threadIdx.x; j < n; j += (int64_t)gridDim.x * blockDim.x) {
+        double sr = 0.0, si = 0.0;
+        for (int i = 0; i < nvec; ++i) {
+            const double2 c = coef.c[i];
+            const double2 v = V[(int64_t)i * ldv + j];
+            sr += c.x * v.x - c.y * v.y;
+            si += c.x * v.y + c.y * v.x;
+        }
+        x[j] = make_double2(0.0 + sr, 0.0 + si);
+    }
+}
+
 __global__ __launch_bounds__(256) void k_scale_inv_sqrt(double2* __restrict__ dst, const double2* __restrict__ src,
                                                         const double2* __restrict__ nrm2, int64_t n) {
     const double s = 1.0 / sqrt(nrm2[0].x);
@@ -512,7 +529,6 @@
     int device = -1;
     LanRecord* h_rec = nullptr;
     LanRecord* d_rec = nullptr;
-    double2* h_y = nullptr;
     hipEvent_t ev_done[LAN_SLOTS], ev_mv0[LAN_SLOTS], ev_mv1[LAN_SLOTS];
     bool have_events = false;
     unsigned long long serial = 0;
@@ -520,7 +536,6 @@
     ~LanRes() {
         if (device >= 0) (void)hipSetDevice(device);
         if (h_rec) (void)hipHostFree(h_rec);
-        if (h_y) (void)hipHostFree(h_y);
         if (have_events)
             for (int i = 0; i < LAN_SLOTS; ++i) {
                 (void)hipEventDestroy(ev_done[i]);
@@ -536,7 +551,6 @@
         HIP_TRY(hipHostMalloc((void**)&r.h_rec, sizeof(LanRecord) * LAN_SLOTS, hipHostMallocMapped | hipHostMallocCoherent));
         memset(r.h_rec, 0, sizeof(LanRecord) * LAN_SLOTS);
         HIP_TRY(hipHostGetDevicePointer((void**)&r.d_rec, r.h_rec, 0));
-        HIP_TRY(hipHostMalloc((void**)&r.h_y, sizeof(double2) * LAN_SLOTS, hipHostMallocDefault));
         for (int i = 0; i < LAN_SLOTS; ++i) {
             HIP_TRY(hipEventCreateWithFlags(&r.ev_done[i], hipEventDisableTiming));
             HIP_TRY(hipEventCreate(&r.ev_mv0[i]));
@@ -705,18 +719,17 @@
         }
         HIP_TRY(htn_stream_spin(st));
         const int k = (int)y.size();
-        for (int i = 0; i < k; ++i) R->h_y[i] = make_double2(y[i], 0.0);
-        HIP_TRY(hipMemcpyAsync(ycoef, R->h_y, sizeof(double2) * k, hipMemcpyHostToDevice, st));
+        RitzCoef yc;
+        for (int i = 0; i < DOT_CHUNK; ++i) yc.c[i] = make_double2(i < k ? y[i] : 0.0, 0.0);
         double2* xrow = V + (int64_t)(kd + 1) * n;
-        HIP_TRY(hipMemsetAsync(xrow, 0, sizeof(double2) * n, st));
-        hipLaunchKernelGGL(k_axpys, dim3(grid_for(n)), dim3(256), 0, st, xrow, V, n, k, ycoef, 1.0, n);
+        hipLaunchKernelGGL(k_ritz_vector, dim3(grid_for(n)), dim3(256), 0, st, xrow, (const double2*)V, n, k, yc, n);
         if (nf > 0) project_out(xrow);
         else
         hipLaunchKernelGGL(k_norm_partial, dim3(DOT_BLOCKS), dim3(DOT_THREADS), 0, st, xrow, n, norm_partial);
         hipLaunchKernelGGL(k_scale_by_norm, dim3(grid_for(n)), dim3(DOT_THREADS), 0, st, V, xrow, norm_partial, n,
                            (LanRecord*)nullptr, (const double2*)nullptr, (const double2*)nullptr, 0ull);
+        if (res < tol || beta < 1e-14 * std::max(amax, 1e-300) || restart == max_restart) break;
         HIP_TRY(htn_stream_spin(st));
-        if (res < tol || beta < 1e-14 * std::max(amax, 1e-300)) break;
     }
     HIP_TRY(hipGetLastError());
     if (dbg_timers)
diff --git a/hubbardtn_amd/csrc/htn_svd.hip b/hubbardtn_amd/csrc/htn_svd.hip
--- a/hubbardtn_amd/csrc/htn_svd.hip
+++ b/hubbardtn_amd/csrc/htn_svd.hip
@@ -2416,6 +2416,13 @@
 #undef RING_CASE
 }
 
+struct JacPending {
+    bool active = false;
+    int n_xcd = 1;
+    std::vector<int> n_eff;
+    const volatile int *h_rank = nullptr, *h_ring_sw = nullptr;
+    int32_t* sweeps_used = nullptr;
+};
 struct JacScratch {
     int device = -1;
     int cu_count = 0;
@@ -2433,6 +2440,7 @@
     HtnBuf tall_flags{HTN_BUF_MAPPED};
     hipStream_t aux = nullptr;
     hipEvent_t ev_fork = nullptr, ev_join = nullptr, ev_sweep[2] = {nullptr, nullptr};
+    JacPending pending;
     ~JacScratch() {
         if (device >= 0) (void)hipSetDevice(device);
         if (aux) {
@@ -2583,6 +2591,9 @@
 
 struct JacCoreBufs {
     int *d_ids, *d_slot, *d_perm;
+    RingItem *d_ring_items, *h_ring_items;
+    unsigned* d_ring_sync;
+    size_t upload_bytes, fill_bytes;
     double* d_zero;
     unsigned long long* d_ratio;
     int *d_done, *d_sw;
@@ -2593,14 +2604,22 @@
     volatile int *h_active, *h_rank, *h_ring_sw;
     int *d_active, *d_rank, *d_ring_sw;
 };
-static int carve_core_scratch(JacScratch& js, int nl, int n_blocks, int max_sweeps, size_t n_items_max, JacCoreBufs* B) {
-    const size_t off_ids = 0, off_slot = off_ids + sizeof(int) * nl, off_perm = off_slot + sizeof(int) * n_blocks;
+static int carve_core_scratch(JacScratch& js, int nl, int n_blocks, int max_sweeps, size_t n_items_max, size_t n_ring_items,
+                              size_t ring_sync_bytes, JacCoreBufs* B) {
+    const size_t off_ids = 0, off_slot = off_ids + sizeof(int) * nl;
+    const size_t off_ritems = (off_slot + sizeof(int) * n_blocks + 31) / 32 * 32;
+    const size_t off_perm = off_ritems + sizeof(RingItem) * n_ring_items;
     const size_t off_zero = off_perm + sizeof(int) * nl * 64 * JAC_MAXEL;
-    const size_t off_ratio = (off_zero + sizeof(double) * nl + 7) / 8 * 8, off_done = off_ratio + 8 * nl;
+    const size_t off_ratio = (off_zero + sizeof(double) * nl + 15) / 16 * 16, off_done = off_ratio + 8 * nl;
     const size_t off_sw = off_done + sizeof(int) * nl, off_qsync = off_sw + sizeof(int) * nl;
-    const size_t off_items = (off_qsync + sizeof(unsigned) * (QR_SYNC_WORDS * (size_t)nl + 8) + 31) / 32 * 32;
+    const size_t end_qsync = off_qsync + sizeof(unsigned) * (QR_SYNC_WORDS * (size_t)nl + 8);
+    const size_t off_rsync = (end_qsync + 15) / 16 * 16;
+    const size_t off_items = (off_rsync + ring_sync_bytes + 31) / 32 * 32;
+    const size_t h_off_ids = (sizeof(JacPairItem) * n_items_max + 31) / 32 * 32;
+    B->upload_bytes = n_ring_items ? off_perm : off_slot + sizeof(int) * n_blocks;
+    B->fill_bytes = (ring_sync_bytes ? off_rsync + ring_sync_bytes : end_qsync) - off_ratio;
     if (js.dev.reserve(off_items + sizeof(JacPairItem) * n_items_max)) return 1;
-    if (js.pinned.reserve(sizeof(JacPairItem) * n_items_max + 4 * (size_t)(nl + n_blocks) + 128)) return 1;
+    if (js.pinned.reserve(h_off_ids + off_perm + 128)) return 1;
     if (js.flags.reserve(sizeof(int) * ((size_t)(max_sweeps + 1) + 2 * (size_t)nl + 16))) return 1;
     char* d = (char*)js.dev.p;
     B->d_ids = (int*)(d + off_ids);
@@ -2612,10 +2631,13 @@
     B->d_sw = (int*)(d + off_sw);
     B->d_qsync = (unsigned*)(d + off_qsync);
     B->d_items = (JacPairItem*)(d + off_items);
+    B->d_ring_items = (RingItem*)(d + off_ritems);
+    B->d_ring_sync = (unsigned*)(d + off_rsync);
     char* h = (char*)js.pinned.p;
     B->h_items = (JacPairItem*)h;
-    B->h_ids = (int*)(h + sizeof(JacPairItem) * n_items_max);
+    B->h_ids = (int*)(h + h_off_ids);
     B->h_slot = B->h_ids + nl;
+    B->h_ring_items = (RingItem*)(h + h_off_ids + off_ritems);
     B->h_active = (volatile int*)js.flags.p;
     B->h_rank = B->h_active + (max_sweeps + 1);
     B->h_ring_sw = B->h_rank + nl;
@@ -2718,48 +2740,88 @@
     return 0;
 }
 
+struct RingSyncLayout {
+    int arrive_off, fail_off, xcc_off, conv_off;
+    size_t bytes;
+};
+static RingSyncLayout ring_sync_layout(int n_wg, int nl, int max_sweeps) {
+    RingSyncLayout L;
+    L.arrive_off = 2 * n_wg, L.fail_off = L.arrive_off + nl * max_sweeps, L.xcc_off = L.fail_off + 1;
+    L.conv_off = (L.xcc_off + n_wg + 3) & ~3;
+    L.bytes = ((size_t)L.conv_off * 4 + (size_t)nl * max_sweeps * 8 + 15) & ~(size_t)15;
+    return L;
+}
+
+static int ring_collect_flags(const volatile int* h_rank, const volatile int* h_ring_sw, const int* n_eff, int nl, int n_xcd,
+                              int* used_out, int* all_local_out) {
+    int used = 0;
+    for (int li = 0; li < nl; ++li) {
+        if (h_rank[li] < 0) return fail_msg("htn_jacobi_svd_z: a hand-off of the multi-workgroup QR timed out");
+        if (h_ring_sw[li] <= 0 && n_eff[li] >= 2)
+            return fail_msg("htn_jacobi_svd_z: a hand-off of the ring Jacobi kernel timed out");
+        used = std::max(used, (int)h_ring_sw[li] % 1000);
+    }
+    int all_local = n_xcd > 1 ? 1 : 0;
+    for (int li = 0; li < nl; ++li)
+        if (n_eff[li] >= 2 && h_ring_sw[li] < 1000) all_local = 0;
+    *used_out = used, *all_local_out = all_local;
+    return 0;
+}
+extern "C" int htn_jacobi_collect_check(const int32_t* rank, const int32_t* ring_sweeps, const int32_t* n_eff, int32_t n_large,
+                                        int32_t n_xcd, int32_t* sweeps_used, int32_t* xcd_local) {
+    int used = 0, local = 0;
+    if (ring_collect_flags(rank, ring_sweeps, n_eff, n_large, n_xcd, &used, &local)) return 1;
+    if (sweeps_used) *sweeps_used = used;
+    if (xcd_local) *xcd_local = local;
+    return 0;
+}
+static int jacobi_ring_collect(JacScratch& js) {
+    JacPending& P = js.pending;
+    if (!P.active) return 0;
+    P.active = false;
+    int used = 0, all_local = 0;
+    if (ring_collect_flags(P.h_rank, P.h_ring_sw, P.n_eff.data(), (int)P.n_eff.size(), P.n_xcd, &used, &all_local)) return 1;
+    js.xcd_local = all_local;
+    if (P.sweeps_used) *P.sweeps_used = used;
+    return 0;
+}
+
 static int run_ring(const JacCall& c, JacScratch& js, const JacCoreBufs& B, const RingPlan& plan, int n_xcd, bool two_partner,
-                    bool staged_send, int32_t* sweeps_used) {
+                    bool staged_send, int32_t* sweeps_used, bool prestaged, bool defer) {
     const int nl = c.nl(), n_wg = plan.wgs, n_items = (int)plan.items.size();
-    const int arrive_off = 2 * n_wg, fail_off = arrive_off + nl * c.max_sweeps, xcc_off = fail_off + 1;
-    const int conv_off = (xcc_off + n_wg + 3) & ~3;
-    const size_t sync_bytes = ((size_t)conv_off * 4 + (size_t)nl * c.max_sweeps * 8 + 15) & ~(size_t)15;
-    if (js.ring_sync.reserve(sync_bytes)) return 1;
+    const RingSyncLayout SL = ring_sync_layout(n_wg, nl, c.max_sweeps);
     if (js.ring_mbox.reserve(sizeof(double2) * (size_t)std::max<int64_t>(plan.mbox_elems, 1))) return 1;
-    if (js.ring_items.reserve(sizeof(RingItem) * n_items) || js.ring_items_h.reserve(sizeof(RingItem) * n_items)) return 1;
-    memcpy(js.ring_items_h.p, plan.items.data(), sizeof(RingItem) * n_items);
+    const RingItem* d_items = B.d_ring_items;
+    unsigned* d_sync = B.d_ring_sync;
+    if (!prestaged) {
+        if (js.ring_sync.reserve(SL.bytes)) return 1;
+        if (js.ring_items.reserve(sizeof(RingItem) * n_items) || js.ring_items_h.reserve(sizeof(RingItem) * n_items)) return 1;
+        memcpy(js.ring_items_h.p, plan.items.data(), sizeof(RingItem) * n_items);
+        HIP_TRY(hipMemcpyAsync(js.ring_items.p, js.ring_items_h.p, sizeof(RingItem) * n_items, hipMemcpyHostToDevice, c.st));
+        HIP_TRY(hipMemsetAsync(js.ring_sync.p, 0, SL.bytes, c.st));
+        d_items = (const RingItem*)js.ring_items.p, d_sync = (unsigned*)js.ring_sync.p;
+    }
     for (int li = 0; li < nl; ++li) B.h_ring_sw[li] = 0;
-    HIP_TRY(hipMemcpyAsync(js.ring_items.p, js.ring_items_h.p, sizeof(RingItem) * n_items, hipMemcpyHostToDevice, c.st));
-    HIP_TRY(hipMemsetAsync(js.ring_sync.p, 0, sync_bytes, c.st));
     RingArgs ra;
     ra.Vj = c.Vj, ra.G = c.G, ra.S = c.S, ra.desc = c.desc, ra.large_ids = B.d_ids;
-    ra.perm = B.d_perm, ra.zero2 = B.d_zero, ra.mbox = (double2*)js.ring_mbox.p, ra.sync = (unsigned*)js.ring_sync.p;
-    ra.arrive_off = arrive_off, ra.fail_off = fail_off, ra.conv_off = conv_off, ra.max_sweeps = c.max_sweeps, ra.tol = c.tol;
-    ra.xcc_off = xcc_off;
+    ra.perm = B.d_perm, ra.zero2 = B.d_zero, ra.mbox = (double2*)js.ring_mbox.p, ra.sync = d_sync;
+    ra.arrive_off = SL.arrive_off, ra.fail_off = SL.fail_off, ra.conv_off = SL.conv_off, ra.max_sweeps = c.max_sweeps, ra.tol = c.tol;
+    ra.xcc_off = SL.xcc_off;
     ra.two_partner = two_partner ? 1 : 0;
     ra.staged_send = staged_send ? 1 : 0;
     ra.info = c.info_dev, ra.sweeps_out = B.d_ring_sw;
     for (auto& bt : plan.batches) {
-        ra.items = (const RingItem*)js.ring_items.p + bt.first;
+        ra.items = d_items + bt.first;
         hipLaunchKernelGGL(k_jacobi_ring, dim3((unsigned)bt.second), dim3(RING_THREADS), 2 * RING_PANEL_ELEMS * sizeof(double2),
                            c.st, ra);
     }
     HIP_TRY(hipGetLastError());
     HIP_TRY(hipStreamWaitEvent(c.st, js.ev_join, 0));
+    JacPending& P = js.pending;
+    P.active = true, P.n_xcd = n_xcd, P.n_eff = c.n_eff, P.h_rank = B.h_rank, P.h_ring_sw = B.h_ring_sw, P.sweeps_used = sweeps_used;
+    if (defer) return 0;
     HIP_TRY(htn_stream_spin(c.st));
-    int used = 0;
-    for (int li = 0; li < nl; ++li) {
-        if (B.h_rank[li] < 0) return fail_msg("htn_jacobi_svd_z: a hand-off of the multi-workgroup QR timed out");
-        if (B.h_ring_sw[li] <= 0 && c.n_eff[li] >= 2)
-            return fail_msg("htn_jacobi_svd_z: a hand-off of the ring Jacobi kernel timed out");
-        used = std::max(used, (int)B.h_ring_sw[li] % 1000);
-    }
-    int all_local = n_xcd > 1 ? 1 : 0;
-    for (int li = 0; li < nl; ++li)
-        if (c.n_eff[li] >= 2 && B.h_ring_sw[li] < 1000) all_local = 0;
-    js.xcd_local = all_local;
-    if (sweeps_used) *sweeps_used = used;
-    return 0;
+    return jacobi_ring_collect(js);
 }
 
 static int run_pair_visits(const JacCall& c, JacScratch& js, const JacCoreBufs& B, const JacTournament& T, int hint,
@@ -2788,7 +2850,8 @@
 
 static int jacobi_svd_core(void* G, void* Vj, double* S, const htn_svd_block* desc, const htn_svd_block* desc_host,
                            int32_t n_blocks, int32_t max_m_host, int32_t max_sweeps, double tol, int32_t* info_dev,
-                           const htn_svd_opts* opts, void* stream, const int* skip_dev, const unsigned char* skip_host) {
+                           const htn_svd_opts* opts, void* stream, const int* skip_dev, const unsigned char* skip_host,
+                           bool defer) {
     if (n_blocks <= 0) return 0;
     if (max_m_host > 64 * JAC_MAXEL) return fail_msg("htn_jacobi_svd_z: block taller than 512 rows");
     const double rank_cut = opts && opts->rank_cut > 0.0 ? opts->rank_cut : 0.0;
@@ -2812,15 +2875,12 @@
         c.n_eff.push_back(desc_host[b].n);
     }
     JacScratch* jsp = nullptr;
-    JacCoreBufs B;
-    if (js_get(c.st, &jsp) || carve_core_scratch(*jsp, nl, n_blocks, max_sweeps, n_items_max, &B)) return 1;
+    if (js_get(c.st, &jsp)) return 1;
     JacScratch& js = *jsp;
-    for (int b = 0; b < n_blocks; ++b) B.h_slot[b] = skip_host && skip_host[b] ? nl : -1;
-    for (int li = 0; li < nl; ++li) B.h_slot[c.large[li]] = li;
-    for (int li = 0; li < nl; ++li) B.h_ids[li] = c.large[li];
-    for (int k = 0; k <= max_sweeps; ++k) B.h_active[k] = 1;
-    HIP_TRY(hipMemcpyAsync(B.d_ids, B.h_ids, sizeof(int) * (nl + n_blocks), hipMemcpyHostToDevice, c.st));
-    HIP_TRY(hipMemsetAsync(B.d_ratio, 0, 16 * (size_t)nl + sizeof(unsigned) * (QR_SYNC_WORDS * (size_t)nl + 8), c.st));
+    if (js.pending.active) {
+        js.pending.active = false;
+        return fail_msg("htn_jacobi_svd_z: the call enqueued before on this stream has not been collected");
+    }
     static const bool force_pairs = htn_env_flag("HTN_SVD_PAIRS");
     static const bool no_xcd = htn_env_flag("HTN_RING_NO_XCD");
     static const bool ring_staged = htn_env_flag("HTN_RING_STAGED_SEND");
@@ -2830,6 +2890,18 @@
     RingPlan plan;
     JacTournament T;
     bool use_ring = !force_pairs && plan_ring(c, n_xcd, ring_cap, &plan);
+    const bool prestaged = use_ring && c.cut2 <= 0.0;
+    const RingSyncLayout SL = prestaged ? ring_sync_layout(plan.wgs, nl, max_sweeps) : RingSyncLayout{0, 0, 0, 0, 0};
+    JacCoreBufs B;
+    if (carve_core_scratch(js, nl, n_blocks, max_sweeps, n_items_max, prestaged ? plan.items.size() : 0, SL.bytes, &B)) return 1;
+    if (prestaged && js.ring_mbox.reserve(sizeof(double2) * (size_t)std::max<int64_t>(plan.mbox_elems, 1))) return 1;
+    for (int b = 0; b < n_blocks; ++b) B.h_slot[b] = skip_host && skip_host[b] ? nl : -1;
+    for (int li = 0; li < nl; ++li) B.h_slot[c.large[li]] = li;
+    for (int li = 0; li < nl; ++li) B.h_ids[li] = c.large[li];
+    for (int k = 0; k <= max_sweeps; ++k) B.h_active[k] = 1;
+    if (prestaged) memcpy(B.h_ring_items, plan.items.data(), sizeof(RingItem) * plan.items.size());
+    HIP_TRY(hipMemcpyAsync(B.d_ids, B.h_ids, B.upload_bytes, hipMemcpyHostToDevice, c.st));
+    HIP_TRY(hipMemsetAsync(B.d_ratio, 0, B.fill_bytes, c.st));
     if (c.cut2 <= 0.0 && !use_ring) {
         T = jacobi_tournament(c.n_eff.data(), nl);
         if (upload_tournament(T, B.h_items, B.d_items, c.st)) return 1;
@@ -2850,7 +2922,7 @@
             if (upload_tournament(T, B.h_items, B.d_items, c.st)) return 1;
         }
     }
-    if (use_ring) return run_ring(c, js, B, plan, n_xcd, ring_two_partner, ring_staged, sweeps_used);
+    if (use_ring) return run_ring(c, js, B, plan, n_xcd, ring_two_partner, ring_staged, sweeps_used, prestaged, defer);
     return run_pair_visits(c, js, B, T, opts && opts->sweeps_hint > 0 ? opts->sweeps_hint : 0, sweeps_used);
 }
 
@@ -2899,7 +2971,7 @@
     int core_used = 0;
     if (nt < n_blocks) {
         if (jacobi_svd_core(G, Vj, S, desc, desc_host, n_blocks, max_m_rest, max_sweeps, tol, info_dev, opts, stream, d_skip,
-                            skip.data()))
+                            skip.data(), false))
             return 1;
         if (opts && opts->sweeps_used) core_used = *opts->sweeps_used;
     }
@@ -2926,10 +2998,9 @@
     return 0;
 }
 
-extern "C" int htn_jacobi_svd_z(void* G, void* Vj, double* S, const htn_svd_block* desc,
-                                const htn_svd_block* desc_host, int32_t n_blocks, int32_t max_m_host,
-                                int32_t max_sweeps, double tol, int32_t* info_dev, const htn_svd_opts* opts,
-                                void* stream) {
+static int jacobi_svd_entry(void* G, void* Vj, double* S, const htn_svd_block* desc, const htn_svd_block* desc_host,
+                            int32_t n_blocks, int32_t max_m_host, int32_t max_sweeps, double tol, int32_t* info_dev,
+                            const htn_svd_opts* opts, void* stream, bool defer) {
     if (n_blocks <= 0) return 0;
     std::vector<int> tall;
     int max_m_rest = 0;
@@ -2944,9 +3015,27 @@
     }
     if (tall.empty())
         return jacobi_svd_core(G, Vj, S, desc, desc_host, n_blocks, max_m_host, max_sweeps, tol, info_dev, opts, stream,
-                               nullptr, nullptr);
+                               nullptr, nullptr, defer);
     if (max_m_rest > 64 * JAC_MAXEL) return fail_msg("htn_jacobi_svd_z: block taller than 512 rows");
     return jacobi_svd_tall(G, Vj, S, desc, desc_host, n_blocks, max_m_rest, max_sweeps, tol, info_dev, opts, stream, tall);
+}
+
+extern "C" int htn_jacobi_svd_z(void* G, void* Vj, double* S, const htn_svd_block* desc,
+                                const htn_svd_block* desc_host, int32_t n_blocks, int32_t max_m_host,
+                                int32_t max_sweeps, double tol, int32_t* info_dev, const htn_svd_opts* opts,
+                                void* stream) {
+    return jacobi_svd_entry(G, Vj, S, desc, desc_host, n_blocks, max_m_host, max_sweeps, tol, info_dev, opts, stream, false);
+}
+
+int htn_jacobi_svd_enqueue(void* G, void* Vj, double* S, const htn_svd_block* desc, const htn_svd_block* desc_host,
+                           int32_t n_blocks, int32_t max_m_host, int32_t max_sweeps, double tol, int32_t* info_dev,
+                           const htn_svd_opts* opts, void* stream) {
+    return jacobi_svd_entry(G, Vj, S, desc, desc_host, n_blocks, max_m_host, max_sweeps, tol, info_dev, opts, stream, true);
+}
+int htn_jacobi_svd_collect(void* stream) {
+    JacScratch* js = nullptr;
+    if (js_get((hipStream_t)stream, &js)) return 1;
+    return jacobi_ring_collect(*js);
 }
 
 __global__ __launch_bounds__(256) void k_batched_copy(double2* __restrict__ dst, const double2* __restrict__ src,
diff --git a/include/hubbardtn_hip.h b/include/hubbardtn_hip.h
--- a/include/hubbardtn_hip.h
+++ b/include/hubbardtn_hip.h
@@ -95,6 +95,8 @@
 int htn_jacobi_svd_z(void* G, void* Vj, double* S, const htn_svd_block* desc, const htn_svd_block* desc_host,
                      int32_t n_blocks, int32_t max_m_host, int32_t max_sweeps, double tol, int32_t* info_dev,
                      const htn_svd_opts* opts, void* stream);
+int htn_jacobi_collect_check(const int32_t* rank, const int32_t* ring_sweeps, const int32_t* n_eff, int32_t n_large,
+                             int32_t n_xcd, int32_t* sweeps_used, int32_t* xcd_local);
 
 typedef struct {
     int64_t dst_off, src_off, idx_off, scl_off;
```

Result: faster. 401.0 ms, median of 6 (-1.2%).
